# polli-labs/linnaeus

Measured on AMD Instinct MI355X. Metric: images/sec (train fwd+bwd) mFormerV1_sm 3x224x224, higher is better.
Workload: dtype bf16; 1 GPU; mFormerV1_sm train step (forward + 4-task CE loss + backward + AdamW (one HIP launch)), bf16 operands / fp32 accumulate+residual, batch 256/GPU, 3x224x224 synthetic, DropPath 0.2, gradient checkpointing off; per_gpu_batch=256, global_batch=256, parallelism=dp1, grad_mode=direct

## Files before the change

include/lnx.h:

```cpp
#ifndef LNX_H
#define LNX_H
#include <stdint.h>

#ifdef __cplusplus
extern "C" {
#endif

#define LNX_F32 0
#define LNX_BF16 1

const char* lnx_last_error(void);
int lnx_version(void);
int lnx_device_cus(void);
int lnx_set_cu_margin(int cus);

typedef struct lnx_rowmap {
    int group, pad, off;
} lnx_rowmap;

enum { LNX_ACT_NONE = 0, LNX_ACT_GELU = 1, LNX_ACT_RELU = 2, LNX_ACT_GELU_BWD = 3, LNX_ACT_RELU_BWD = 4,
       LNX_ACT_GELU_D = 5, LNX_ACT_MUL_AUX = 6 };
enum { LNX_ADDR_PLAIN = 0, LNX_ADDR_PATCH2 = 1 };

typedef struct lnx_gemm_args {
// ... 461 lines not shown
} lnx_metrics_task;
typedef struct lnx_metrics_args {
    int dtype;
    int B, n_tasks;
    lnx_metrics_task task[LNX_SOFTCE_MAX_TASKS];
    const int64_t* subset_ids[2];
    int n_bins[2];
    int64_t* counts;
    double* sums;
} lnx_metrics_args;
int lnx_metrics_table_sizes(int n_tasks, int n_bins0, int n_bins1, int64_t* n_counts, int64_t* n_sums);
int lnx_metrics_update(const lnx_metrics_args* args, void* stream);

#define LNX_PREDICT_MAX_K 16
typedef struct lnx_predict_task {
    const void* logits;
    int64_t ld;
    int C;
    const int32_t* parent;
    int null_index;
    const int64_t* id_map;
} lnx_predict_task;
typedef struct lnx_predict_args {
    int dtype;
    int B, n_tasks;
    int K;
    int consistency;
    const int32_t* k_per_sample;
    lnx_predict_task task[LNX_SOFTCE_MAX_TASKS];
    int64_t* ids;
    float* probs;
    int32_t* count;
    int32_t* flags;
} lnx_predict_args;
int lnx_predict(const lnx_predict_args* args, void* stream);

#define LNX_RESIZE_NEAREST 0
#define LNX_RESIZE_BILINEAR 1
#define LNX_RESIZE_BICUBIC 2
#define LNX_PREPROCESS_MAX_SIDE 16384
int lnx_resize_taps(int in_size, int out_size, int filter);
int lnx_resize_coeffs(int in_size, int out_size, int filter, int32_t* k, int32_t* bounds);
typedef struct lnx_preprocess_image {
    int64_t src;
    int64_t hk, hb;
    int64_t vk, vb;
    int64_t scratch;
    int32_t h, w;
    int32_t htaps, vtaps;
    int32_t y0, rows;
} lnx_preprocess_image;
typedef struct lnx_preprocess_args {
    int n, H, W;
    int filter;
    const lnx_preprocess_image* images;
    const void* blob;
    int64_t blob_bytes;
    int64_t images_off;
    void* scratch;
    int64_t scratch_bytes;
    float mean[3], std[3];
    float* out;
} lnx_preprocess_args;
int64_t lnx_preprocess_scratch_bytes(lnx_preprocess_image* images, int n, int H, int W, int filter);
int lnx_preprocess(const lnx_preprocess_args* args, void* stream);

enum { LNX_HL_WS_RAW = 0, LNX_HL_WS_LSE, LNX_HL_WS_SS, LNX_HL_WS_COEF, LNX_HL_WS_MASKED_CW, LNX_HL_WS_MASKED_W, LNX_HL_WS_FLAGS, LNX_HL_WS_ROWS };
enum { LNX_HL_OUT_RAW_MEAN = 0, LNX_HL_OUT_MASKED_MEAN, LNX_HL_OUT_WEIGHTED, LNX_HL_OUT_SCALE, LNX_HL_OUT_TOTAL = 32, LNX_HL_OUT_INCLUSION = 33,
       LNX_HL_OUT_FLOATS = 40 };
enum { LNX_HL_NULL_TOTAL = 8, LNX_HL_NULL_INCLUDED = 9, LNX_HL_COUNTS = 10 };
typedef struct lnx_hier_loss_task {
    const void* logits;
    int64_t ld;
    int C;
    const int64_t* target;
    const float* soft_target;
    int64_t ldt;
    const float* soft;
    float smoothing;
    const float* crit_weight;
    int64_t ignore_index;
    const float* class_weight;
    int n_cw;
    int p_cw, p_w;
    float* dlogits;
    int64_t ldd;
} lnx_hier_loss_task;
typedef struct lnx_hier_loss_args {
    int dtype;
    int B, n_tasks;
    float prob;
    int mask_mul;
    const float* draws;
    const float* weights;
    float* ws;
    float* out;
    int64_t* counts;
    lnx_hier_loss_task task[LNX_SOFTCE_MAX_TASKS];
} lnx_hier_loss_args;
int lnx_hier_loss_fwd(const lnx_hier_loss_args* args, void* stream);
int lnx_hier_loss_bwd(const lnx_hier_loss_args* args, const float* go_dev, void* stream);

int lnx_convmlp_supported(int dtype, int C);
typedef struct lnx_convmlp_args {
    int dtype, M, C;
    const void* ln;
    const void* w1;
    const float* b1;
    const void* w2;
    const float* b2;
    const float* gamma;
    const float* rowscale;
    int rows_per_sample;
    const float* x;
    float* out;
    void* z;
    const void* y;
    const float* ln_w;
    const float* ln_b;
    float ln_eps;
    void* ln_out;
    float* mean;
    float* rstd;
} lnx_convmlp_args;
int lnx_convmlp_fwd(const lnx_convmlp_args* args, void* stream);

typedef struct lnx_convmlp_bwd_args {
    int dtype, M, C;
    const float* g;
    const void* ln;
    const void* z;
    const void* w1;
    const float* b1;
    const void* w2t;
    const void* w1t;
    const float* gamma;
    const float* rowscale;
    int rows_per_sample;
    void* act;
    void* dh;
    void* dz;
    void* dln;
    float* dgamma;
    const void* y;
    const float* ln_w;
    const float* mean;
    const float* rstd;
    float* d_ln_w;
    float* d_ln_b;
    float* ws;
    int64_t ws_floats;
    int dz_plain;
    int ln_defer;
} lnx_convmlp_bwd_args;
int lnx_convmlp_bwd(const lnx_convmlp_bwd_args* args, void* stream);
int64_t lnx_convmlp_bwd_ws_floats(int C, int M);


#define LNX_MAX_META 8
#define LNX_MAX_TASKS 16
typedef struct lnx_mformer_cfg {
    int dtype;
    int batch, img_h, img_w, in_chans;
    int dims[4];
    int conv_depths[2];
    int rope_depths[2];
    int rope_heads[2];
    int mlp_hidden[2];
    int n_meta;
    int meta_dims[LNX_MAX_META];
    int only_last_cls;
    int n_tasks;
    int task_classes[LNX_MAX_TASKS];
    int inference;
    int recompute;
    int fp8;
    int rope_mode;
} lnx_mformer_cfg;

typedef struct lnx_plan lnx_plan;
int lnx_plan_create(const lnx_mformer_cfg* cfg, lnx_plan** out);
void lnx_plan_destroy(lnx_plan* p);
int64_t lnx_plan_workspace_bytes(const lnx_plan* p);
int lnx_plan_num_params(const lnx_plan* p);
const char* lnx_plan_param_name(const lnx_plan* p, int i);
int64_t lnx_plan_param_numel(const lnx_plan* p, int i);
int lnx_plan_num_drop_calls(const lnx_plan* p);
int64_t lnx_plan_logits_numel(const lnx_plan* p);
int64_t lnx_plan_logits_offset(const lnx_plan* p, int task);
int lnx_plan_logits_ld(const lnx_plan* p, int task);
int lnx_plan_bind(lnx_plan* p, const float* const* params, float* const* grads, void* workspace);
int lnx_plan_forward(lnx_plan* p, const float* x, const float* meta, const float* drop_scales, const unsigned char* drop_mask,
                     float* feats, float* logits, void* stream);
int64_t lnx_plan_dropout_bytes(const lnx_plan* p);
int lnx_plan_set_dropout(lnx_plan* p, const unsigned char* masks, float drop_rate);
int64_t lnx_plan_attn_dropout_bytes(const lnx_plan* p);
int lnx_plan_set_attn_dropout(lnx_plan* p, const unsigned char* masks, float drop_rate);
int lnx_plan_backward(lnx_plan* p, const float* dlogits, const float* dfeats, int segment, void* stream);
int lnx_plan_backward_into(lnx_plan* p, const float* dlogits, const float* dfeats, float* const* grads, void* stream);
#define LNX_PROFILE_CLASSES 8
int lnx_plan_profile_begin(lnx_plan* p);
int lnx_plan_profile_end(lnx_plan* p, double* ms, double* work, int* launches);
#define LNX_PROFILE_CLASSES_EX 10
int lnx_plan_profile_begin_spans(lnx_plan* p);
int lnx_plan_profile_end_ex(lnx_plan* p, double* ms, double* work, double* bytes, int* launches);
int lnx_plan_set_wgrad_stream(lnx_plan* p, int on);
int lnx_plan_set_meta_stream(lnx_plan* p, int mode);
int lnx_plan_segment_params(const lnx_plan* p, int segment, int* idx_out, int max_out);

#ifdef __cplusplus
}
#endif
#endif
```

linnaeus_amd/_lib.py:

```python
from __future__ import annotations

import ctypes as C
import os

_HERE = os.path.dirname(os.path.abspath(__file__))
LIB_PATH = os.environ.get("LNX_LIB_PATH") or os.path.join(_HERE, "liblnx_hip.so")

F32, BF16 = 0, 1
ACT_NONE, ACT_GELU, ACT_RELU, ACT_GELU_BWD, ACT_RELU_BWD, ACT_GELU_D, ACT_MUL_AUX = 0, 1, 2, 3, 4, 5, 6
TN_WS_FLOATS = 256 * (256 * 128 + 256)
ADDR_PLAIN, ADDR_PATCH2 = 0, 1


class LnxError(RuntimeError):
    pass


class RowMap(C.Structure):
    _fields_ = [("group", C.c_int), ("pad", C.c_int), ("off", C.c_int)]


class GemmArgs(C.Structure):
    _fields_ = [
        ("dtype", C.c_int), ("M", C.c_int), ("N", C.c_int), ("K", C.c_int),
        ("A", C.c_void_p), ("lda", C.c_int64),
        ("W", C.c_void_p), ("ldw", C.c_int64),
        ("C", C.c_void_p), ("ldc", C.c_int64),
        ("out_f32", C.c_int),
        ("a_mode", C.c_int), ("Hin", C.c_int), ("Win", C.c_int), ("Cin", C.c_int),
        ("c_mode", C.c_int), ("c_map", RowMap),
        ("bias", C.c_void_p),
        ("c2", C.c_void_p), ("ldc2", C.c_int64),
        ("act", C.c_int),
        ("aux", C.c_void_p), ("ldaux", C.c_int64),
        ("gamma", C.c_void_p), ("rowscale", C.c_void_p), ("rows_per_sample", C.c_int),
        ("res", C.c_void_p), ("ldres", C.c_int64),
        ("c8", C.c_void_p), ("ldc8", C.c_int64), ("c8_scales", C.c_void_p),
    ]


class WgradArgs(C.Structure):
    _fields_ = [
        ("dtype", C.c_int), ("M", C.c_int), ("N", C.c_int), ("K", C.c_int),
        ("dY", C.c_void_p), ("lddy", C.c_int64),
        ("A", C.c_void_p), ("lda", C.c_int64),
        ("a_mode", C.c_int), ("Hin", C.c_int), ("Win", C.c_int), ("Cin", C.c_int),
        ("dW", C.c_void_p), ("lddw", C.c_int64),
        ("k_perm_c", C.c_int),
        ("db", C.c_void_p),
        ("splits", C.c_int),
        ("k_store", C.c_int),
        ("ws", C.c_void_p), ("ws_floats", C.c_int64),
        ("defer", C.c_int),
    ]


class SoftCEArgs(C.Structure):
    _fields_ = [
        ("B", C.c_int), ("C", C.c_int),
        ("logits", C.c_void_p), ("ld", C.c_int64),
        ("target", C.c_void_p),
        ("soft", C.c_void_p), ("smoothing", C.c_float),
        ("class_weight", C.c_void_p),
        ("ignore_index", C.c_int64),
        ("row_scale", C.c_void_p), ("scale", C.c_float),
        ("loss", C.c_void_p), ("loss_sum", C.c_void_p),
        ("dlogits", C.c_void_p), ("ldd", C.c_int64),
    ]


ADAMW_MAX_GROUPS = 16


class AdamWDesc(C.Structure):
    _fields_ = [("p", C.c_void_p), ("m", C.c_void_p), ("v", C.c_void_p), ("g", C.c_void_p), ("n", C.c_int64), ("group", C.c_int), ("block_start", C.c_int)]


class AdamWHyper(C.Structure):
    _fields_ = [("ngroups", C.c_int)] + [(k, C.c_float * ADAMW_MAX_GROUPS) for k in ("lr", "beta1", "beta2", "eps", "weight_decay", "bias_c1", "bias_c2", "omb1", "omb2")]


class AdEMAMixHyper(C.Structure):
    _fields_ = [("ngroups", C.c_int)] + [(k, C.c_float * ADAMW_MAX_GROUPS) for k in ("lr", "beta1", "beta2", "eps", "weight_decay", "bias_c1", "bias_c2", "omb1", "omb2",
                                                                                  "alpha_t", "beta3_t", "omb3")]


class GradNormArgs(C.Structure):
    _fields_ = [("T", C.c_int), ("alpha", C.c_float), ("norm", C.c_void_p), ("loss_sum", C.c_void_p), ("count", C.c_void_p), ("init_loss", C.c_void_p),
                ("weights", C.c_void_p), ("initial_losses", C.c_void_p), ("initted", C.c_void_p), ("metrics", C.c_void_p)]


METRICS_MAX_TASKS = 8
METRICS_CHAIN_N, METRICS_CHAIN_CORRECT, METRICS_PARTIAL_N, METRICS_PARTIAL_CORRECT, METRICS_SUBSET_OOR = range(5)
METRICS_HEAD = 8
METRICS_N, METRICS_CORRECT1, METRICS_CORRECT3, METRICS_NULL_N, METRICS_NULL_CORRECT1, METRICS_NONNULL_N, METRICS_NONNULL_CORRECT1, METRICS_LOSS_N = range(8)
METRICS_TASK_STRIDE = 8
METRICS_SUM_LOSS, METRICS_SUM_NULL_LOSS, METRICS_SUM_NONNULL_LOSS = range(3)
METRICS_SUM_STRIDE = 4


def metrics_task(t: int) -> int:
    return METRICS_HEAD + METRICS_TASK_STRIDE * t


def metrics_subset(n_tasks: int, n_bins0: int, s: int) -> int:
    return metrics_task(n_tasks) + (2 * n_tasks * n_bins0 if s else 0)


class MetricsTask(C.Structure):
    _fields_ = [("logits", C.c_void_p), ("ld", C.c_int64), ("target", C.c_void_p), ("is_null", C.c_void_p), ("loss", C.c_void_p), ("C", C.c_int)]


class MetricsArgs(C.Structure):
    _fields_ = [("dtype", C.c_int), ("B", C.c_int), ("n_tasks", C.c_int), ("task", MetricsTask * METRICS_MAX_TASKS),
                ("subset_ids", C.c_void_p * 2), ("n_bins", C.c_int * 2), ("counts", C.c_void_p), ("sums", C.c_void_p)]


PREDICT_MAX_K = 16


class PredictTask(C.Structure):
    _fields_ = [("logits", C.c_void_p), ("ld", C.c_int64), ("C", C.c_int), ("parent", C.c_void_p), ("null_index", C.c_int), ("id_map", C.c_void_p)]


class PredictArgs(C.Structure):
    _fields_ = [("dtype", C.c_int), ("B", C.c_int), ("n_tasks", C.c_int), ("K", C.c_int), ("consistency", C.c_int), ("k_per_sample", C.c_void_p),
                ("task", PredictTask * METRICS_MAX_TASKS), ("ids", C.c_void_p), ("probs", C.c_void_p), ("count", C.c_void_p), ("flags", C.c_void_p)]


RESIZE_NEAREST, RESIZE_BILINEAR, RESIZE_BICUBIC = range(3)
PREPROCESS_MAX_SIDE = 16384


class PreprocessImage(C.Structure):
    _fields_ = [("src", C.c_int64), ("hk", C.c_int64), ("hb", C.c_int64), ("vk", C.c_int64), ("vb", C.c_int64), ("scratch", C.c_int64),
                ("h", C.c_int32), ("w", C.c_int32), ("htaps", C.c_int32), ("vtaps", C.c_int32), ("y0", C.c_int32), ("rows", C.c_int32)]


class PreprocessArgs(C.Structure):
    _fields_ = [("n", C.c_int), ("H", C.c_int), ("W", C.c_int), ("filter", C.c_int), ("images", C.POINTER(PreprocessImage)), ("blob", C.c_void_p),
                ("blob_bytes", C.c_int64), ("images_off", C.c_int64), ("scratch", C.c_void_p), ("scratch_bytes", C.c_int64),
                ("mean", C.c_float * 3), ("std", C.c_float * 3), ("out", C.c_void_p)]


HL_WS_RAW, HL_WS_LSE, HL_WS_SS, HL_WS_COEF, HL_WS_MASKED_CW, HL_WS_MASKED_W, HL_WS_FLAGS, HL_WS_ROWS = range(8)
HL_OUT_RAW_MEAN, HL_OUT_MASKED_MEAN, HL_OUT_WEIGHTED, HL_OUT_SCALE = range(4)
HL_OUT_TOTAL, HL_OUT_INCLUSION, HL_OUT_FLOATS = 32, 33, 40
HL_NULL_TOTAL, HL_NULL_INCLUDED, HL_COUNTS = 8, 9, 10


class HierLossTask(C.Structure):
    _fields_ = [("logits", C.c_void_p), ("ld", C.c_int64), ("C", C.c_int), ("target", C.c_void_p), ("soft_target", C.c_void_p), ("ldt", C.c_int64),
                ("soft", C.c_void_p), ("smoothing", C.c_float), ("crit_weight", C.c_void_p), ("ignore_index", C.c_int64), ("class_weight", C.c_void_p),
                ("n_cw", C.c_int), ("p_cw", C.c_int), ("p_w", C.c_int), ("dlogits", C.c_void_p), ("ldd", C.c_int64)]


class HierLossArgs(C.Structure):
    _fields_ = [("dtype", C.c_int), ("B", C.c_int), ("n_tasks", C.c_int), ("prob", C.c_float), ("mask_mul", C.c_int), ("draws", C.c_void_p),
                ("weights", C.c_void_p), ("ws", C.c_void_p), ("out", C.c_void_p), ("counts", C.c_void_p), ("task", HierLossTask * METRICS_MAX_TASKS)]


_lib = None


def lib() -> C.CDLL:
    global _lib
    if _lib is None:
        if not os.path.exists(LIB_PATH):
            raise LnxError(
                f"{LIB_PATH} is missing: build it with `python -c 'import __graft_entry__ as g; g.build()'` "
                "(or `make -C linnaeus_amd/csrc`). linnaeus_amd has no CPU fallback."
            )
        _lib = C.CDLL(LIB_PATH)
        _lib.lnx_last_error.restype = C.c_char_p
        _lib.lnx_nt_kernel_launches.restype = C.c_int64
        _lib.lnx_convmlp_bwd_ws_floats.restype = C.c_int64
        _lib.lnx_meta_heads_bwd_part_floats.restype = C.c_int64
        if hasattr(_lib, "lnx_ademamix_step"):
            _lib.lnx_ademamix_step.argtypes = [C.c_void_p, C.c_void_p, C.c_int, C.c_int, C.POINTER(AdEMAMixHyper), C.c_void_p, C.c_float, C.c_void_p]
        if hasattr(_lib, "lnx_gradnorm_sumsq"):
            _lib.lnx_gradnorm_sumsq.argtypes = [C.c_void_p, C.c_int, C.c_int, C.c_int, C.c_int64, C.c_void_p, C.c_void_p, C.c_void_p, C.c_void_p]
        if hasattr(_lib, "lnx_metrics_update"):
            _lib.lnx_metrics_update.argtypes = [C.POINTER(MetricsArgs), C.c_void_p]
            _lib.lnx_metrics_table_sizes.argtypes = [C.c_int, C.c_int, C.c_int, C.POINTER(C.c_int64), C.POINTER(C.c_int64)]
        if hasattr(_lib, "lnx_predict"):
            _lib.lnx_predict.argtypes = [C.POINTER(PredictArgs), C.c_void_p]
            _lib.lnx_predict.restype = C.c_int
        if hasattr(_lib, "lnx_hier_loss_fwd"):
            _lib.lnx_hier_loss_fwd.argtypes = [C.POINTER(HierLossArgs), C.c_void_p]
            _lib.lnx_hier_loss_bwd.argtypes = [C.POINTER(HierLossArgs), C.c_void_p, C.c_void_p]
        if hasattr(_lib, "lnx_preprocess"):
            _lib.lnx_resize_taps.argtypes = [C.c_int, C.c_int, C.c_int]
            _lib.lnx_resize_coeffs.argtypes = [C.c_int, C.c_int, C.c_int, C.c_void_p, C.c_void_p]
            _lib.lnx_preprocess_scratch_bytes.argtypes = [C.POINTER(PreprocessImage), C.c_int, C.c_int, C.c_int, C.c_int]
            _lib.lnx_preprocess_scratch_bytes.restype = C.c_int64
            _lib.lnx_preprocess.argtypes = [C.POINTER(PreprocessArgs), C.c_void_p]
            _lib.lnx_preprocess.restype = C.c_int
        if hasattr(_lib, "lnx_layernorm_fwd_query"):
            _lib.lnx_layernorm_fwd_query.argtypes = [C.POINTER(LnArgs), C.POINTER(LnLaunch)]
            _lib.lnx_layernorm_bwd_query.argtypes = [C.POINTER(LnBwdArgs), C.POINTER(LnLaunch)]
        older = bool(os.environ.get("LNX_LIB_PATH")) and os.environ.get("LNX_LIB_OLDER") == "1"
        for name in EXPORTS:
            if not hasattr(_lib, name) and not older:
                raise LnxError(f"{LIB_PATH} does not export {name}; rebuild it")
    return _lib


def check(rc: int, what: str) -> None:
    if rc != 0:
        raise LnxError(f"{what} failed (rc={rc}): {lib().lnx_last_error().decode()}")


AUG_CLAMP, AUG_POSTERIZE, AUG_SOLARIZE, AUG_SOLARIZE_ADD, AUG_INVERT, AUG_BRIGHTNESS, AUG_CONTRAST = range(7)

NT_KERNEL_NONE, NT_KERNEL_V1, NT_KERNEL_V2, NT_KERNEL_SKINNY, NT_KERNEL_V4, NT_KERNEL_FP8, NT_KERNEL_V7, NT_KERNEL_MX8, NT_KERNEL_V9, NT_KERNEL_EXPERIMENT = 0, 1, 2, 3, 4, 6, 7, 8, 9, 15

ROPE_COS, ROPE_ROTATE = 0, 1

ATTN_KERNEL_NONE, ATTN_KERNEL_RES4, ATTN_KERNEL_RES8, ATTN_KERNEL_TILED4, ATTN_KERNEL_TILED8 = range(5)

EXPORTS = [
    "lnx_last_error", "lnx_version", "lnx_device_cus", "lnx_set_cu_margin",
    "lnx_gemm_nt", "lnx_last_nt_kernel", "lnx_nt_kernel_launches", "lnx_nt_dispatch", "lnx_gemm_tn", "lnx_gemm_tn_flush", "lnx_gemm_tn_discard", "lnx_amax", "lnx_quantize_fp8", "lnx_gemm_nt_fp8", "lnx_quantize_mxfp8", "lnx_gemm_nt_mxfp8", "lnx_dropout_mul", "lnx_dropout_residual", "lnx_plan_dropout_bytes", "lnx_plan_set_dropout", "lnx_plan_attn_dropout_bytes", "lnx_plan_set_attn_dropout",
    "lnx_layernorm_fwd", "lnx_layernorm_bwd", "lnx_layernorm_bwd_flush", "lnx_layernorm_bwd_discard", "lnx_layernorm_fwd_query", "lnx_layernorm_bwd_query",
    "lnx_dwconv7_fwd", "lnx_dwconv7_wgrad",
    "lnx_gemm_nt_group_ok", "lnx_gemm_nt_group", "lnx_rope_cos_table", "lnx_rope_cos_table_hd", "lnx_rope_cossin_table_hd", "lnx_rope_cos_tables", "lnx_attn_bwd_ws_floats", "lnx_attn_bwd_ws_floats_hd", "lnx_attn_fwd", "lnx_attn_bwd", "lnx_attn_bwd_flush", "lnx_attn_bwd_discard", "lnx_attn_dispatch", "lnx_last_attn_kernel",
    "lnx_im2col_stem", "lnx_scale_cast", "lnx_layerscale_bwd", "lnx_layerscale_apply_wgrad", "lnx_fill_rows", "lnx_colsum_rows",
    "lnx_agg2_fwd", "lnx_agg2_bwd", "lnx_pack_meta", "lnx_meta_heads_supported", "lnx_meta_heads_fwd", "lnx_meta_heads_bwd", "lnx_meta_heads_bwd_part_floats", "lnx_prep_weights", "lnx_prep_blocks", "lnx_softce", "lnx_softce_multi", "lnx_stem_fwd", "lnx_stem_fwd_ok", "lnx_adamw_blocks", "lnx_grad_sumsq", "lnx_adamw_step", "lnx_ademamix_step", "lnx_gradnorm_sumsq", "lnx_gradnorm_update",
    "lnx_metrics_table_sizes", "lnx_metrics_update", "lnx_predict", "lnx_resize_taps", "lnx_resize_coeffs", "lnx_preprocess_scratch_bytes", "lnx_preprocess", "lnx_hier_loss_fwd", "lnx_hier_loss_bwd",
    "lnx_mix_rows", "lnx_mix_meta",
    "lnx_aug_pointwise", "lnx_aug_saturation", "lnx_aug_rowstat", "lnx_aug_rescale", "lnx_aug_affine", "lnx_aug_stencil", "lnx_erase_rects", "lnx_u8hwc_to_f32chw",
    "lnx_convmlp_supported", "lnx_convmlp_fwd", "lnx_convmlp_bwd", "lnx_convmlp_bwd_ws_floats",
    "lnx_plan_create", "lnx_plan_destroy", "lnx_plan_workspace_bytes", "lnx_plan_num_params", "lnx_plan_param_name",
    "lnx_plan_param_numel", "lnx_plan_num_drop_calls", "lnx_plan_logits_numel", "lnx_plan_logits_offset", "lnx_plan_logits_ld",
    "lnx_plan_bind", "lnx_plan_forward", "lnx_plan_backward", "lnx_plan_backward_into", "lnx_plan_segment_params", "lnx_plan_profile_begin", "lnx_plan_profile_end", "lnx_plan_profile_begin_spans", "lnx_plan_profile_end_ex", "lnx_plan_set_wgrad_stream", "lnx_plan_set_meta_stream",
]


class MetaHeadArgs(C.Structure):
    _fields_ = [
        ("B", C.c_int), ("C", C.c_int), ("dim", C.c_int), ("off", C.c_int),
        ("meta", C.c_void_p), ("meta_width", C.c_int), ("eps", C.c_float),
        ("w0", C.c_void_p), ("ldw0", C.c_int), ("b0", C.c_void_p), ("ln0_w", C.c_void_p), ("ln0_b", C.c_void_p),
        ("w1", C.c_void_p), ("ldw1", C.c_int), ("b1", C.c_void_p), ("ln1_w", C.c_void_p), ("ln1_b", C.c_void_p),
        ("w2", C.c_void_p), ("ldw2", C.c_int), ("b2", C.c_void_p), ("ln2_w", C.c_void_p), ("ln2_b", C.c_void_p),
        ("t0", C.c_void_p), ("h0", C.c_void_p), ("x", C.c_void_p), ("h1", C.c_void_p), ("n1", C.c_void_p), ("h2", C.c_void_p),
        ("m0", C.c_void_p), ("r0", C.c_void_p), ("m1", C.c_void_p), ("r1", C.c_void_p), ("m2", C.c_void_p), ("r2", C.c_void_p),
        ("tok", C.c_void_p), ("tok_row_stride", C.c_int64), ("tok_row_offset", C.c_int64),
    ]


class MetaHeadBwdArgs(C.Structure):
    _fields_ = [
        ("B", C.c_int), ("C", C.c_int), ("dim", C.c_int),
        ("g", C.c_void_p), ("g_row_stride", C.c_int64), ("g_row_offset", C.c_int64),
        ("w1t", C.c_void_p), ("ldw1t", C.c_int), ("w2t", C.c_void_p), ("ldw2t", C.c_int),
        ("ln0_w", C.c_void_p), ("ln1_w", C.c_void_p), ("ln2_w", C.c_void_p),
        ("t0", C.c_void_p), ("h0", C.c_void_p), ("x", C.c_void_p), ("h1", C.c_void_p), ("n1", C.c_void_p), ("h2", C.c_void_p),
        ("m0", C.c_void_p), ("r0", C.c_void_p), ("m1", C.c_void_p), ("r1", C.c_void_p), ("m2", C.c_void_p), ("r2", C.c_void_p),
        ("dp2", C.c_void_p), ("dp1", C.c_void_p), ("dp0", C.c_void_p), ("part", C.c_void_p),
        ("d_w0", C.c_void_p), ("d_b0", C.c_void_p), ("d_ln0_w", C.c_void_p), ("d_ln0_b", C.c_void_p),
        ("d_w1", C.c_void_p), ("d_b1", C.c_void_p), ("d_ln1_w", C.c_void_p), ("d_ln1_b", C.c_void_p),
        ("d_w2", C.c_void_p), ("d_b2", C.c_void_p), ("d_ln2_w", C.c_void_p), ("d_ln2_b", C.c_void_p),
    ]


class LnArgs(C.Structure):
    _fields_ = [
        ("M", C.c_int), ("C", C.c_int), ("eps", C.c_float),
        ("x", C.c_void_p), ("x_dtype", C.c_int), ("ldx", C.c_int64), ("x_map", RowMap),
        ("w", C.c_void_p), ("b", C.c_void_p),
        ("y", C.c_void_p), ("y_dtype", C.c_int), ("ldy", C.c_int64), ("y_map", RowMap),
        ("add", C.c_void_p), ("ldadd", C.c_int64),
        ("mean", C.c_void_p), ("rstd", C.c_void_p),
        ("y8", C.c_void_p), ("ldy8", C.c_int64), ("y8_scales", C.c_void_p),
    ]


class LnBwdArgs(C.Structure):
    _fields_ = [
        ("M", C.c_int), ("C", C.c_int),
        ("dy", C.c_void_p), ("dy_dtype", C.c_int), ("lddy", C.c_int64), ("dy_map", RowMap),
        ("x", C.c_void_p), ("x_dtype", C.c_int), ("ldx", C.c_int64), ("x_map", RowMap),
        ("w", C.c_void_p), ("mean", C.c_void_p), ("rstd", C.c_void_p),
        ("gin", C.c_void_p), ("ldgin", C.c_int64),
        ("dx", C.c_void_p), ("dx_dtype", C.c_int), ("lddx", C.c_int64),
        ("dw", C.c_void_p), ("db", C.c_void_p), ("relu_mask", C.c_int),
        ("ws", C.c_void_p), ("ws_floats", C.c_int64),
        ("dx2", C.c_void_p), ("dx2_dtype", C.c_int), ("lddx2", C.c_int64), ("dx2_rowscale", C.c_void_p), ("dx2_rows_per_sample", C.c_int),
        ("dx2_8", C.c_void_p), ("dx2_8_scales", C.c_void_p), ("lddx2_8", C.c_int64),
        ("defer", C.c_int),
    ]


LN_COLS_NONE, LN_COLS_ATOMICS, LN_COLS_WORKSPACE = range(3)


class LnLaunch(C.Structure):
    _fields_ = [("G", C.c_int), ("V", C.c_int), ("pair", C.c_int), ("full", C.c_int), ("mx", C.c_int), ("grid", C.c_int), ("cols", C.c_int), ("slices", C.c_int)]


class RopeTable(C.Structure):
    _fields_ = [
        ("freqs", C.c_void_p), ("cos_out", C.c_void_p), ("dsin_out", C.c_void_p),
        ("heads", C.c_int), ("H", C.c_int), ("W", C.c_int), ("head_dim", C.c_int),
        ("rope_mode", C.c_int), ("sin_out", C.c_void_p),
    ]


class DwconvArgs(C.Structure):
    _fields_ = [
        ("B", C.c_int), ("H", C.c_int), ("W", C.c_int), ("C", C.c_int),
        ("x", C.c_void_p), ("x_dtype", C.c_int), ("w49", C.c_void_p), ("bias", C.c_void_p),
        ("flip", C.c_int), ("res", C.c_void_p), ("y", C.c_void_p), ("y_dtype", C.c_int),
    ]


class DwconvWgradArgs(C.Structure):
    _fields_ = [
        ("B", C.c_int), ("H", C.c_int), ("W", C.c_int), ("C", C.c_int),
        ("x", C.c_void_p), ("x_dtype", C.c_int), ("dy", C.c_void_p), ("dy_dtype", C.c_int),
        ("dw", C.c_void_p), ("db", C.c_void_p),
    ]


class AttnArgs(C.Structure):
    _fields_ = [
        ("dtype", C.c_int), ("B", C.c_int), ("N", C.c_int), ("E", C.c_int), ("heads", C.c_int),
        ("qkv", C.c_void_p), ("cos_tab", C.c_void_p), ("o", C.c_void_p), ("lse", C.c_void_p),
        ("drop_mask", C.c_void_p), ("drop_inv_keep", C.c_float), ("head_dim", C.c_int),
        ("rope_mode", C.c_int), ("sin_tab", C.c_void_p),
    ]


class AttnBwdArgs(C.Structure):
    _fields_ = [
        ("dtype", C.c_int), ("B", C.c_int), ("N", C.c_int), ("E", C.c_int), ("heads", C.c_int),
        ("qkv", C.c_void_p), ("cos_tab", C.c_void_p), ("o", C.c_void_p), ("lse", C.c_void_p),
        ("d_o", C.c_void_p), ("dqkv", C.c_void_p), ("freq_ws", C.c_void_p), ("delta", C.c_void_p),
        ("drop_mask", C.c_void_p), ("drop_inv_keep", C.c_float),
        ("dsin_tab", C.c_void_p), ("dfreqs", C.c_void_p), ("defer_freqs", C.c_int), ("head_dim", C.c_int),
        ("rope_mode", C.c_int), ("sin_tab", C.c_void_p), ("grid_w", C.c_int),
    ]


class PrepDesc(C.Structure):
    _fields_ = [
        ("src", C.c_void_p), ("dst", C.c_void_p), ("dst_t", C.c_void_p),
        ("rows", C.c_int), ("cols", C.c_int), ("ld", C.c_int), ("ld_t", C.c_int),
        ("P", C.c_int), ("mode", C.c_int), ("block_start", C.c_int),
    ]


PREP_CAST, PREP_CONV_PERM, PREP_DW49 = 0, 1, 2


class ConvMlpArgs(C.Structure):
    _fields_ = [
        ("dtype", C.c_int), ("M", C.c_int), ("C", C.c_int),
        ("ln", C.c_void_p), ("w1", C.c_void_p), ("b1", C.c_void_p), ("w2", C.c_void_p), ("b2", C.c_void_p),
        ("gamma", C.c_void_p), ("rowscale", C.c_void_p), ("rows_per_sample", C.c_int),
        ("x", C.c_void_p), ("out", C.c_void_p), ("z", C.c_void_p),
        ("y", C.c_void_p), ("ln_w", C.c_void_p), ("ln_b", C.c_void_p), ("ln_eps", C.c_float), ("ln_out", C.c_void_p),
        ("mean", C.c_void_p), ("rstd", C.c_void_p),
    ]


class ConvMlpBwdArgs(C.Structure):
    _fields_ = [
        ("dtype", C.c_int), ("M", C.c_int), ("C", C.c_int),
        ("g", C.c_void_p), ("ln", C.c_void_p), ("z", C.c_void_p), ("w1", C.c_void_p), ("b1", C.c_void_p),
        ("w2t", C.c_void_p), ("w1t", C.c_void_p), ("gamma", C.c_void_p), ("rowscale", C.c_void_p), ("rows_per_sample", C.c_int),
        ("act", C.c_void_p), ("dh", C.c_void_p), ("dz", C.c_void_p), ("dln", C.c_void_p), ("dgamma", C.c_void_p),
        ("y", C.c_void_p), ("ln_w", C.c_void_p), ("mean", C.c_void_p), ("rstd", C.c_void_p), ("d_ln_w", C.c_void_p), ("d_ln_b", C.c_void_p),
        ("ws", C.c_void_p), ("ws_floats", C.c_int64),
        ("dz_plain", C.c_int), ("ln_defer", C.c_int),
    ]


class StemArgs(C.Structure):
    _fields_ = [("x", C.c_void_p), ("w", C.c_void_p), ("bias", C.c_void_p), ("ln_w", C.c_void_p), ("ln_b", C.c_void_p), ("patches", C.c_void_p),
                ("pre", C.c_void_p), ("y", C.c_void_p), ("mean", C.c_void_p), ("rstd", C.c_void_p), ("B", C.c_int), ("Cin", C.c_int), ("H", C.c_int),
                ("W", C.c_int), ("Cout", C.c_int), ("eps", C.c_float)]


class MixArgs(C.Structure):
    _fields_ = [
        ("x", C.c_void_p), ("perm", C.c_void_p), ("valid", C.c_void_p), ("out", C.c_void_p),
        ("B", C.c_int), ("row", C.c_int64), ("H", C.c_int), ("W", C.c_int), ("lam", C.c_float),
        ("h0", C.c_int), ("h1", C.c_int), ("w0", C.c_int), ("w1", C.c_int), ("mode", C.c_int),
    ]
```

linnaeus_amd/csrc/api.cpp:

```cpp
#include <hip/hip_runtime.h>
#include <stdarg.h>
#include <stdio.h>
#include <stdlib.h>
#include <string.h>

#include <atomic>
#include <mutex>

#include "../../include/lnx.h"

static thread_local char g_err[1024] = "";

void lnx_set_error(const char* fmt, ...) {
    va_list ap;
    va_start(ap, fmt);
    vsnprintf(g_err, sizeof(g_err), fmt, ap);
    va_end(ap);
}

extern "C" const char* lnx_last_error(void) { return g_err; }
extern "C" int lnx_version(void) { return 107; }
extern "C" int lnx_device_cus(void) {
    int dev = 0;
    if (hipGetDevice(&dev) != hipSuccess) return -1;
    hipDeviceProp_t prop;
    if (hipGetDeviceProperties(&prop, dev) != hipSuccess) return -1;
    return prop.multiProcessorCount;
}

static std::atomic<int> g_cu_margin{-1};
int persistent_cus(int cus) {
    int m = g_cu_margin.load(std::memory_order_relaxed);
    if (m < 0) {
        const char* e = getenv("LNX_CU_MARGIN");
        m = e ? atoi(e) : 0;
        if (m < 0) m = 0;
        g_cu_margin.store(m, std::memory_order_relaxed);
    }
    const int room = cus - m;
    return room < 8 ? 8 : room;
}
void set_cu_margin(int m) { g_cu_margin.store(m < 0 ? 0 : m, std::memory_order_relaxed); }
bool tile_sched_static() {
    const char* e = getenv("LNX_TILE_SCHED");
    return e && strcmp(e, "static") == 0;
}
int tile_slot_of(hipStream_t st) {
    static std::mutex mu;
    static hipStream_t known[64];
    static int n = 0;
    std::lock_guard<std::mutex> lock(mu);
    for (int i = 0; i < n; ++i)
        if (known[i] == st) return i;
    if (n < 64) {
        known[n] = st;
        return n++;
    }
    return -1;
}
int device_cus() {
    static std::atomic<int> cached{0};
    int c = cached.load(std::memory_order_relaxed);
    if (c == 0) {
        c = lnx_device_cus();
        if (c > 0) cached.store(c, std::memory_order_relaxed);
    }
    return c > 0 ? c : 0;
}
extern "C" int lnx_set_cu_margin(int cus) {
    if (cus < 0 || cus > 1024) {
        lnx_set_error("lnx_set_cu_margin: %d (0..1024 compute units)", cus);
        return 1;
    }
    set_cu_margin(cus);
    return 0;
}
```

linnaeus_amd/csrc/convmlp.hip:

```cpp
#include <stdlib.h>

#include "common.hpp"
#include "../../include/lnx.h"

namespace {

struct CmP {
    const unsigned char* ln;
    const unsigned char* w1;
    const unsigned char* w2;
    const unsigned char* w2t;
    const unsigned char* w1t;
    const unsigned char* zin;
    const float* b1;
    const float* b2;
    const float* gamma;
    const float* rowscale;
    const float* x;
    const float* g;
    float* out;
    unsigned char* z;
    unsigned char* act;
    unsigned char* dh;
    unsigned char* dz;
    unsigned char* dln;
    float* dgamma;
    int M, C, rps;
    const unsigned char* y;
    const float* lnw;
    const float* lnb;
    float eps;
    unsigned char* ln_out;
    float* mean;
    float* rstd;
    float* part;
    int64_t part_floats;
    int ln_defer;
    int tile_slot;
    int dz_plain;
    float* dlnw;
    float* dlnb;
};

__device__ __forceinline__ void mfma16(f32x4_t& acc, const uint4& a, const uint4& b) {
    acc = __builtin_amdgcn_mfma_f32_16x16x32_bf16(__builtin_bit_cast(bf16x8_t, a), __builtin_bit_cast(bf16x8_t, b), acc, 0, 0, 0);
}

__device__ __forceinline__ int key4(int a) { return (4 - (a & 3)) & 3; }

#define CM_DS_READ128(dst, addr, OFF) asm volatile("ds_read_b128 %0, %1 offset:" #OFF : "=v"(dst) : "v"(addr) : "memory")

template <int NK> struct Geo {
    static constexpr int C = 32 * NK;
    static constexpr int PART = NK * 4096;
    static constexpr int CT = C / 16;
};

template <int NK, int NW>
__device__ __forceinline__ void dma_nmajor(unsigned char* lds_part, const unsigned char* W, int n0, int wave, int lane) {
    constexpr int C = Geo<NK>::C;
    constexpr int NINS = 4 * NK;
    static_assert(NINS % NW == 0, "DMA pieces must divide evenly over the waves");
#pragma unroll
    for (int t = 0; t < NINS / NW; ++t) {
        const int i = wave + NW * t;
        const int ks = i >> 2, rb = i & 3;
        const int row = 16 * rb + (lane >> 2), u = lane & 3;
        const unsigned char* src = W + ((int64_t)(n0 + row) * C + ks * 32 + ((u ^ key4(row >> 3)) << 3)) * 2;
        __builtin_amdgcn_global_load_lds((const __attribute__((address_space(1))) void*)src,
                                         (__attribute__((address_space(3))) void*)(lds_part + i * 1024), 16, 0, 0);
    }
}

template <int NK, int NW>
__device__ __forceinline__ void dma_cmajor(unsigned char* lds_part, const unsigned char* W, int n0, int wave, int lane) {
    constexpr int C = Geo<NK>::C;
    constexpr int RB = C / 16;
    constexpr int NINS = 2 * RB;
#pragma unroll
    for (int t = 0; t < NINS / NW; ++t) {
        const int i = wave + NW * t;
        const int ks2 = i / RB, rb = i % RB;
        const int row = 16 * rb + (lane >> 2), u = lane & 3;
        const unsigned char* src = W + ((int64_t)row * (4 * C) + n0 + ks2 * 32 + ((u ^ key4(row >> 2)) << 3)) * 2;
        __builtin_amdgcn_global_load_lds((const __attribute__((address_space(1))) void*)src,
                                         (__attribute__((address_space(3))) void*)(lds_part + i * 1024), 16, 0, 0);
    }
}

template <int NK, int MT>
__device__ __forceinline__ void prod_nmajor(f32x4_t (&h)[4][MT], uint32_t part_addr, int s, int g, const uint4 (&xf)[MT][NK]) {
    const uint32_t unit = (uint32_t)((g ^ key4(s >> 2)) << 4);
    const uint32_t base = part_addr + (uint32_t)((8 * (s >> 2) + (s & 3)) * 64) + unit;
#pragma unroll
    for (int nt = 0; nt < 4; ++nt)
#pragma unroll
        for (int mt = 0; mt < MT; ++mt) h[nt][mt] = f32x4_t{0.f, 0.f, 0.f, 0.f};
#pragma unroll
    for (int ks = 0; ks < NK; ++ks) {
        uint4 wf[4];
        const uint32_t a = base + ks * 4096;
        CM_DS_READ128(wf[0], a, 0);
        CM_DS_READ128(wf[1], a, 256);
        CM_DS_READ128(wf[2], a, 2048);
        CM_DS_READ128(wf[3], a, 2304);
        asm volatile("s_waitcnt lgkmcnt(0)" ::: "memory");
        __builtin_amdgcn_sched_barrier(0);
#pragma unroll
        for (int nt = 0; nt < 4; ++nt)
#pragma unroll
            for (int mt = 0; mt < MT; ++mt) mfma16(h[nt][mt], wf[nt], xf[mt][ks]);
    }
}

template <int NK, int MT, int KB>
__device__ __forceinline__ void prod_nmajor_b(f32x4_t (&h)[4][MT], uint32_t part_addr, int s, int g, const uint4 (&xf)[MT][NK]) {
    const uint32_t unit = (uint32_t)((g ^ key4(s >> 2)) << 4);
    const uint32_t base = part_addr + (uint32_t)((8 * (s >> 2) + (s & 3)) * 64) + unit;
#pragma unroll
    for (int nt = 0; nt < 4; ++nt)
#pragma unroll
        for (int mt = 0; mt < MT; ++mt) h[nt][mt] = f32x4_t{0.f, 0.f, 0.f, 0.f};
#pragma unroll
    for (int k0 = 0; k0 < NK; k0 += KB) {
        uint4 wf[KB][4];
#pragma unroll
        for (int kb = 0; kb < KB; ++kb) {
            if (k0 + kb < NK) {
                const uint32_t a = base + (k0 + kb) * 4096;
                CM_DS_READ128(wf[kb][0], a, 0);
                CM_DS_READ128(wf[kb][1], a, 256);
                CM_DS_READ128(wf[kb][2], a, 2048);
                CM_DS_READ128(wf[kb][3], a, 2304);
            }
        }
        asm volatile("s_waitcnt lgkmcnt(0)" ::: "memory");
        __builtin_amdgcn_sched_barrier(0);
#pragma unroll
        for (int kb = 0; kb < KB; ++kb) {
            if (k0 + kb < NK) {
#pragma unroll
                for (int nt = 0; nt < 4; ++nt)
#pragma unroll
                    for (int mt = 0; mt < MT; ++mt) mfma16(h[nt][mt], wf[kb][nt], xf[mt][k0 + kb]);
            }
        }
    }
}

template <int NK, int MT>
__device__ __forceinline__ void prod_cmajor(f32x4_t (&o)[Geo<NK>::CT][MT], uint32_t part_addr, int s, int g, const uint4 (&pf)[MT][2]) {
    constexpr int C = Geo<NK>::C;
    constexpr int CT = Geo<NK>::CT;
    const uint32_t base = part_addr + (uint32_t)(s * 64) + (uint32_t)((g ^ key4(s >> 2)) << 4);
    constexpr int GB = CT % 6 == 0 ? 6 : (CT % 4 == 0 ? 4 : CT);
#pragma unroll
    for (int ks2 = 0; ks2 < 2; ++ks2) {
#pragma unroll
        for (int c0 = 0; c0 < CT; c0 += GB) {
            uint4 wf[GB];
#pragma unroll
            for (int b = 0; b < GB; ++b) {
                const uint32_t a = base + (uint32_t)(ks2 * C * 64 + (c0 + b) * 1024);
                CM_DS_READ128(wf[b], a, 0);
            }
            asm volatile("s_waitcnt lgkmcnt(0)" ::: "memory");
            __builtin_amdgcn_sched_barrier(0);
#pragma unroll
            for (int b = 0; b < GB; ++b)
#pragma unroll
                for (int mt = 0; mt < MT; ++mt) mfma16(o[c0 + b][mt], wf[b], pf[mt][ks2]);
        }
    }
}

template <int NK, int MT>
__device__ __forceinline__ void prod_nmajor_pipe(f32x4_t (&h)[4][MT], uint32_t part_addr, int s, int g, const uint4 (&xf)[MT][NK]) {
// ... 573 lines not shown
    float* gms = b2s + C;
    float* lws = gms + C;
    float* lbs = lws + C;
    const int lane = threadIdx.x & 63;
    const int wave = __builtin_amdgcn_readfirstlane(threadIdx.x >> 6);
    const int s = lane & 15, g = lane >> 4;
    const uint32_t lds0 = (uint32_t)(uintptr_t)(__attribute__((address_space(3))) unsigned char*)smem;

    for (int i = threadIdx.x; i < 4 * C; i += 512) b1s[i] = p.b1[i];
    for (int i = threadIdx.x; i < C; i += 512) {
        b2s[i] = p.b2[i];
        gms[i] = p.gamma[i];
        if constexpr (LNF) {
            lws[i] = p.lnw[i];
            lbs[i] = p.lnb[i];
        }
    }
    const bool dyn = p.tile_slot >= 0;
    const TileShare sh = tile_share((p.M + 31) / 32);
    unsigned* const ctr = &g_tile_ctr[dyn ? p.tile_slot : 0][sh.part][0];
    int drawn = dyn ? sched_draw_counted(ctr) : 0;
    dma_all_nmajor<NK>(w1img, p.w1, wave, lane);
    dma_all_cmajor<NK>(w2img, p.w2, wave, lane);
    asm volatile("s_waitcnt vmcnt(0)" ::: "memory");
    __syncthreads();

    const int ntile = (p.M + 31) / 32;
    auto load_x = [&](uint4 (&dst)[MT][NK], int tile) __attribute__((always_inline)) {
#pragma unroll
        for (int mt = 0; mt < MT; ++mt) {
            const int m = min(tile * 32 + mt * 16 + s, p.M - 1);
#pragma unroll
            for (int ks = 0; ks < NK; ++ks) dst[mt][ks] = ld16((LNF ? p.y : p.ln) + ((int64_t)m * C + ks * 32 + 8 * g) * 2);
        }
    };
    const int xbase = sh.base, xcnt = sh.cnt, xwaves = 8 * sh.workers;
    const int last_draw = xcnt + xwaves - 1;
    int pos = dyn ? __builtin_amdgcn_readfirstlane(drawn) : sh.index * 8 + wave;
    bool reset_ctr = dyn && pos == last_draw;
    uint4 xf[MT][NK];
    if (pos < xcnt) load_x(xf, xbase + pos);
    const float* rsp = p.rowscale ? p.rowscale : p.gamma;
    const float rsf = p.rowscale ? 1.0f : 0.0f;

    int next = 0;
    for (; pos < xcnt; pos = next) {
        const int tile = xbase + pos;
        const int m_base = tile * 32;
        if constexpr (LNF) {
#pragma unroll
            for (int mt = 0; mt < MT; ++mt) {
                float mu, rs;
                ln_row_frags<NK>(xf[mt], lws, lbs, g, p.eps, mu, rs);
                const int m = min(m_base + mt * 16 + s, p.M - 1);
                if constexpr (SAVE != 0) {
#pragma unroll
                    for (int ks = 0; ks < NK; ++ks) st16(p.ln_out + ((int64_t)m * C + ks * 32 + 8 * g) * 2, xf[mt][ks]);
                    if (g == 0) {
                        p.mean[m] = mu;
                        p.rstd[m] = rs;
                    }
                }
            }
        }
        if constexpr (LNF) __builtin_amdgcn_sched_barrier(0);
        if (dyn) drawn = sched_draw_counted(ctr);
        float4 xrv[MT][CT];
        float rsv[MT];
        f32x4_t o[CT][MT];
#pragma unroll
        for (int ct = 0; ct < CT; ++ct)
#pragma unroll
            for (int mt = 0; mt < MT; ++mt) o[ct][mt] = f32x4_t{0.f, 0.f, 0.f, 0.f};
        auto chunk = [&](const int j, auto lastc) __attribute__((always_inline)) {
            constexpr bool LAST = decltype(lastc)::value;
            if constexpr (LAST) {
                __builtin_amdgcn_sched_barrier(0);
                if (dyn) {
                    next = __builtin_amdgcn_readfirstlane(drawn);
                    reset_ctr = reset_ctr || next == last_draw;
                } else {
                    next = pos + xwaves;
                }
#pragma unroll
                for (int mt = 0; mt < MT; ++mt) {
                    const int m = min(m_base + mt * 16 + s, p.M - 1);
#pragma unroll
                    for (int ct = 0; ct < CT; ++ct) xrv[mt][ct] = *reinterpret_cast<const float4*>(p.x + (int64_t)m * C + ct * 16 + 4 * g);
                    rsv[mt] = rsp[p.rowscale ? m / p.rps : 0];
                }
            }
            f32x4_t h[4][MT];
            prod_nmajor_b<NK, MT, NK>(h, lds0 + j * PART, s, g, xf);
            if constexpr (LAST) {
                __builtin_amdgcn_sched_barrier(0);
                load_x(xf, next < xcnt ? xbase + next : tile);
            }
            f32x4_t bv[4];
            const uint32_t ba = lds0 + 2 * NCH * PART + (uint32_t)((64 * j + 8 * g) * 4);
            CM_DS_READ128(bv[0], ba, 0);
            CM_DS_READ128(bv[1], ba, 16);
            CM_DS_READ128(bv[2], ba, 128);
            CM_DS_READ128(bv[3], ba, 144);
            asm volatile("s_waitcnt lgkmcnt(0)" ::: "memory");
            __builtin_amdgcn_sched_barrier(0);
            constexpr int GK = NK == 3 ? 1 : 2;
#pragma unroll
            for (int mt = 0; mt < MT; ++mt)
#pragma unroll
                for (int n2 = 0; n2 < 4; n2 += GK) {
                    f32x4_t hv[GK];
#pragma unroll
                    for (int k = 0; k < GK; ++k) hv[k] = h[n2 + k][mt];
                    gelu4_bias_n<GK>(hv, &bv[n2]);
#pragma unroll
                    for (int k = 0; k < GK; ++k) h[n2 + k][mt] = hv[k];
                }
            uint4 pf[MT][2];
#pragma unroll
            for (int mt = 0; mt < MT; ++mt) {
                pf[mt][0] = pack8(h[0][mt], h[1][mt]);
                pf[mt][1] = pack8(h[2][mt], h[3][mt]);
            }
            prod_cmajor<NK, MT>(o, lds0 + NCH * PART + j * PART, s, g, pf);
        };
#pragma unroll 1
        for (int j = 0; j < NCH - 1; ++j) chunk(j, BoolC<false>{});
        chunk(NCH - 1, BoolC<true>{});
#pragma unroll
        for (int mt = 0; mt < MT; ++mt) {
            const int m = min(m_base + mt * 16 + s, p.M - 1);
            const float rs = fmaf(rsv[mt] - 1.0f, rsf, 1.0f);
#pragma unroll
            for (int ct = 0; ct < CT; ++ct) {
                const int c = ct * 16 + 4 * g;
                const float4 b2 = *reinterpret_cast<const float4*>(b2s + c);
                const float4 gm = *reinterpret_cast<const float4*>(gms + c);
                const float4 xr = xrv[mt][ct];
                const float z0 = o[ct][mt][0] + b2.x, z1 = o[ct][mt][1] + b2.y, z2 = o[ct][mt][2] + b2.z, z3 = o[ct][mt][3] + b2.w;
                if constexpr (SAVE == 1) {
                    uint2 zz;
                    bf16_t* zh = reinterpret_cast<bf16_t*>(&zz);
                    zh[0] = (bf16_t)z0; zh[1] = (bf16_t)z1; zh[2] = (bf16_t)z2; zh[3] = (bf16_t)z3;
                    *reinterpret_cast<uint2*>(p.z + ((int64_t)m * C + c) * 2) = zz;
                }
                *reinterpret_cast<float4*>(p.out + (int64_t)m * C + c) =
                    make_float4(xr.x + rs * gm.x * z0, xr.y + rs * gm.y * z1, xr.z + rs * gm.z * z2, xr.w + rs * gm.w * z3);
            }
        }
    }
    if (reset_ctr && lane == 0) sched_reset(ctr);
}

template <int NK, int MT, bool ST, bool LNB, bool DG>
__global__ __launch_bounds__(512) void convmlp_bwd_res_kernel(const CmP p) {
    constexpr int C = Geo<NK>::C;
    constexpr int CT = Geo<NK>::CT;
    constexpr int PART = Geo<NK>::PART;
    constexpr int NCH = 4 * C / 64;
    extern __shared__ __attribute__((aligned(16))) unsigned char smem[];
    unsigned char* w1img = smem;
    unsigned char* w2timg = smem + NCH * PART;
    float* b1s = reinterpret_cast<float*>(smem + 2 * NCH * PART);
    float* dgs = b1s + 4 * C;
    float* lws = dgs + C;
    float* dls = lws + C;
    float* gms = dls + 2 * C;
    const int lane = threadIdx.x & 63;
    const int wave = __builtin_amdgcn_readfirstlane(threadIdx.x >> 6);
    const int s = lane & 15, g = lane >> 4;
    const uint32_t lds0 = (uint32_t)(uintptr_t)(__attribute__((address_space(3))) unsigned char*)smem;

    for (int i = threadIdx.x; i < 4 * C; i += 512) b1s[i] = p.b1[i];
    for (int i = threadIdx.x; i < C; i += 512) {
        dgs[i] = 0.f;
        gms[i] = p.gamma[i];
        if constexpr (LNB) {
            lws[i] = p.lnw[i];
            dls[i] = dls[C + i] = 0.f;
        }
    }
    const bool dyn = p.tile_slot >= 0;
    const TileShare sh = tile_share((p.M + 16 * MT - 1) / (16 * MT));
    unsigned* const ctr = &g_tile_ctr[dyn ? p.tile_slot : 0][sh.part][0];
    int drawn = dyn ? sched_draw_counted(ctr) : 0;
    dma_all_nmajor<NK>(w1img, p.w1, wave, lane);
    dma_all_nmajor<NK>(w2timg, p.w2t, wave, lane);
    asm volatile("s_waitcnt vmcnt(0)" ::: "memory");
    __syncthreads();

    float dgp[NK][8];
#pragma unroll
    for (int ks = 0; ks < NK; ++ks)
#pragma unroll
        for (int j = 0; j < 8; ++j) dgp[ks][j] = 0.f;

    const int ntile = (p.M + 16 * MT - 1) / (16 * MT);
    const float* rsp = p.rowscale ? p.rowscale : p.gamma;
    const float rsf = p.rowscale ? 1.0f : 0.0f;
    struct TileIn {
        uint4 x[MT][NK], z[MT][NK];
        float4 g0[MT][NK], g1[MT][NK];
        float rs[MT];
        LnRow<NK> lr[MT];
    };
    auto fetch_tile = [&](TileIn& t, int tile) __attribute__((always_inline)) {
#pragma unroll
        for (int mt = 0; mt < MT; ++mt) {
            const int m = min(tile * (16 * MT) + mt * 16 + s, p.M - 1);
#pragma unroll
            for (int ks = 0; ks < NK; ++ks) {
                const int c = ks * 32 + 8 * g;
                t.x[mt][ks] = ld16(p.ln + ((int64_t)m * C + c) * 2);
                t.g0[mt][ks] = *reinterpret_cast<const float4*>(p.g + (int64_t)m * C + c);
                t.g1[mt][ks] = *reinterpret_cast<const float4*>(p.g + (int64_t)m * C + c + 4);
                if constexpr (DG) t.z[mt][ks] = ld16(p.zin + ((int64_t)m * C + c) * 2);
            }
            t.rs[mt] = rsp[p.rowscale ? m / p.rps : 0];
            if constexpr (LNB) ln_bwd_fetch<NK>(t.lr[mt], p, m, g);
        }
    };
    const int xbase = sh.base, xcnt = sh.cnt, xwaves = 8 * sh.workers;
    const int last_draw = xcnt + xwaves - 1;
    int pos = dyn ? __builtin_amdgcn_readfirstlane(drawn) : sh.index * 8 + wave;
    bool reset_ctr = dyn && pos == last_draw;
    TileIn cur;
    if (pos < xcnt) fetch_tile(cur, xbase + pos);
    int next = 0;
    for (; pos < xcnt; pos = next) {
        const int tile = xbase + pos;
        const int m_base = tile * (16 * MT);
        uint4 xf[MT][NK], zf[MT][NK];
        LnRow<NK> lrow[MT];
#pragma unroll
        for (int mt = 0; mt < MT; ++mt) {
            int m = m_base + mt * 16 + s;
            const bool mv = m < p.M;
            if (!mv) m = p.M - 1;
            const float rs = fmaf(cur.rs[mt] - 1.0f, rsf, 1.0f);
            lrow[mt] = cur.lr[mt];
#pragma unroll
            for (int ks = 0; ks < NK; ++ks) {
                const int c = ks * 32 + 8 * g;
                xf[mt][ks] = cur.x[mt][ks];
                const float4 g0 = cur.g0[mt][ks], g1 = cur.g1[mt][ks];
                const float4 a0 = *reinterpret_cast<const float4*>(gms + c), a1 = *reinterpret_cast<const float4*>(gms + c + 4);
                Vec16<bf16_t> zin, dzv, dzs;
                if constexpr (DG) zin.raw = cur.z[mt][ks];
                const float gv[8] = {g0.x, g0.y, g0.z, g0.w, g1.x, g1.y, g1.z, g1.w};
                const float av[8] = {a0.x, a0.y, a0.z, a0.w, a1.x, a1.y, a1.z, a1.w};
#pragma unroll
                for (int j = 0; j < 8; ++j) {
                    const float sg = rs * gv[j];
                    dzv.set(j, sg * av[j]);
                    dzs.set(j, p.dz_plain ? sg : sg * av[j]);
                    if constexpr (DG) dgp[ks][j] = fmaf(mv ? sg : 0.f, zin.get(j), dgp[ks][j]);
                }
                zf[mt][ks] = dzv.raw;
                st16(p.dz + ((int64_t)m * C + c) * 2, dzs.raw);
            }
        }
        if (dyn) drawn = sched_draw_counted(ctr);
        f32x4_t dl[CT][MT];
#pragma unroll
        for (int ct = 0; ct < CT; ++ct)
#pragma unroll
            for (int mt = 0; mt < MT; ++mt) dl[ct][mt] = f32x4_t{0.f, 0.f, 0.f, 0.f};
#pragma unroll 1
        for (int j = 0; j < NCH; ++j) {
            f32x4_t h[4][MT], da[4][MT];
            prod_nmajor_b<NK, MT, NK>(h, lds0 + j * PART, s, g, xf);
            prod_nmajor_b<NK, MT, NK>(da, lds0 + NCH * PART + j * PART, s, g, zf);
            f32x4_t bv[4];
            const uint32_t ba = lds0 + 2 * NCH * PART + (uint32_t)((64 * j + 8 * g) * 4);
            CM_DS_READ128(bv[0], ba, 0);
            CM_DS_READ128(bv[1], ba, 16);
            CM_DS_READ128(bv[2], ba, 128);
            CM_DS_READ128(bv[3], ba, 144);
            asm volatile("s_waitcnt lgkmcnt(0)" ::: "memory");
            __builtin_amdgcn_sched_barrier(0);
#pragma unroll
            for (int mt = 0; mt < MT; ++mt)
#pragma unroll
                for (int n2 = 0; n2 < 4; n2 += 2) {
                    f32x4_t hv[2] = {h[n2][mt], h[n2 + 1][mt]}, dv[2] = {da[n2][mt], da[n2 + 1][mt]};
                    gelu4_bias_grad_n<2>(hv, &bv[n2], dv);
                    h[n2][mt] = hv[0];
                    h[n2 + 1][mt] = hv[1];
                    da[n2][mt] = dv[0];
                    da[n2 + 1][mt] = dv[1];
                }
            uint4 pd[MT][2];
#pragma unroll
            for (int mt = 0; mt < MT; ++mt) {
                const uint4 pa0 = pack8(h[0][mt], h[1][mt]), pa1 = pack8(h[2][mt], h[3][mt]);
                pd[mt][0] = pack8(da[0][mt], da[1][mt]);
                pd[mt][1] = pack8(da[2][mt], da[3][mt]);
                const int m = min(m_base + mt * 16 + s, p.M - 1);
                if constexpr (ST) {
                    const int64_t off = ((int64_t)m * (4 * C) + 64 * j + 8 * g) * 2;
                    st16(p.act + off, pa0);
                    st16(p.act + off + 64, pa1);
                    st16(p.dh + off, pd[mt][0]);
                    st16(p.dh + off + 64, pd[mt][1]);
                }
            }
            prod_tr_nmajor<NK, MT>(dl, lds0 + j * PART, s, g, pd);
        }
        __builtin_amdgcn_sched_barrier(0);
        if (dyn) {
            next = __builtin_amdgcn_readfirstlane(drawn);
            reset_ctr = reset_ctr || next == last_draw;
        } else {
            next = pos + xwaves;
        }
        fetch_tile(cur, next < xcnt ? xbase + next : tile);
        if constexpr (LNB) {
            ln_bwd_rows<NK, MT, 0>(p, dl, lrow[0], m_base + s, s, g, lws, dls);
            if constexpr (MT == 2) ln_bwd_rows<NK, MT, 1>(p, dl, lrow[MT - 1], m_base + 16 + s, s, g, lws, dls);
        } else {
#pragma unroll
            for (int mt = 0; mt < MT; ++mt) {
                const int m = min(m_base + mt * 16 + s, p.M - 1);
#pragma unroll
                for (int ct = 0; ct < CT; ++ct) {
                    const int c = ct * 16 + 4 * g;
                    uint2 v;
                    bf16_t* vh = reinterpret_cast<bf16_t*>(&v);
                    vh[0] = (bf16_t)dl[ct][mt][0]; vh[1] = (bf16_t)dl[ct][mt][1]; vh[2] = (bf16_t)dl[ct][mt][2]; vh[3] = (bf16_t)dl[ct][mt][3];
                    *reinterpret_cast<uint2*>(p.dln + ((int64_t)m * C + c) * 2) = v;
                }
            }
        }
    }
    if constexpr (DG) {
#pragma unroll
        for (int ks = 0; ks < NK; ++ks)
#pragma unroll
            for (int j = 0; j < 8; ++j) {
                float t = dgp[ks][j];
                t += __shfl_xor(t, 1, 64);
                t += __shfl_xor(t, 2, 64);
                t += __shfl_xor(t, 4, 64);
                t += __shfl_xor(t, 8, 64);
                if (s == 0) atomicAdd(&dgs[ks * 32 + 8 * g + j], t);
            }
    }
    __syncthreads();
    if constexpr (DG)
        for (int i = threadIdx.x; i < C; i += 512) atomicAdd(p.dgamma + i, dgs[i]);
    if constexpr (LNB)
        for (int i = threadIdx.x; i < 2 * C; i += 512) p.part[(int64_t)blockIdx.x * (2 * C) + i] = dls[i];
    if (reset_ctr && lane == 0) sched_reset(ctr);
}

__global__ __launch_bounds__(256) void ln_partials_reduce_kernel(const float* __restrict__ part, int nwg, int C, float* __restrict__ dw, float* __restrict__ db) {
    const int e = blockIdx.x * 256 + threadIdx.x;
    if (e >= 2 * C) return;
    const int per = (nwg + gridDim.y - 1) / gridDim.y;
    const int w0 = blockIdx.y * per, w1 = min(nwg, w0 + per);
    float t0 = 0.f, t1 = 0.f, t2 = 0.f, t3 = 0.f;
    int w = w0;
    for (; w + 4 <= w1; w += 4) {
        t0 += part[(int64_t)w * 2 * C + e];
        t1 += part[(int64_t)(w + 1) * 2 * C + e];
        t2 += part[(int64_t)(w + 2) * 2 * C + e];
        t3 += part[(int64_t)(w + 3) * 2 * C + e];
    }
    for (; w < w1; ++w) t0 += part[(int64_t)w * 2 * C + e];
    const float t = (t0 + t1) + (t2 + t3);
    if (w0 < w1) atomicAdd((e < C ? dw : db) + (e < C ? e : e - C), t);
}

static const bool nw8 = !(getenv("LNX_CM_NW") && atoi(getenv("LNX_CM_NW")) == 4);

static int bwd_grid(int C, int M) {
    if (C <= 96) {
        const int rows = C == 32 ? 32 : 16;
        const int grid = cdiv(cdiv(M, rows), 8);
        return grid > 256 ? 256 : grid;
    }
    return cdiv(M, 16 * (nw8 ? 8 : 4));
}

static int res_room() {
    const int cus = device_cus();
    const int room = persistent_cus(cus > 0 ? cus : 256);
    return room > 256 ? 256 : room;
}

template <int NK, bool LNF, int SAVE>
int launch_fwd_res_t(const CmP& p, hipStream_t st) {
    const size_t lds = 2 * (4 * Geo<NK>::C / 64) * Geo<NK>::PART + 8 * Geo<NK>::C * sizeof(float);
    static bool attr = false;
    if (!attr) {
        (void)hipFuncSetAttribute(reinterpret_cast<const void*>(&convmlp_fwd_res_kernel<NK, LNF, SAVE>), hipFuncAttributeMaxDynamicSharedMemorySize, (int)lds);
        attr = true;
    }
    int grid = cdiv(cdiv(p.M, 32), 8);
    const int room = res_room();
    if (grid > room) grid = room;
    CmP q = p;
    q.tile_slot = tile_sched_static() ? -1 : tile_slot_of(st);
    hipLaunchKernelGGL((convmlp_fwd_res_kernel<NK, LNF, SAVE>), dim3(grid), dim3(512), lds, st, q);
    return 0;
}
template <int NK>
int launch_fwd_res(const CmP& p, hipStream_t st) {
    if (p.y) return p.z ? launch_fwd_res_t<NK, true, 1>(p, st) : (p.ln_out ? launch_fwd_res_t<NK, true, 2>(p, st) : launch_fwd_res_t<NK, true, 0>(p, st));
    return p.z ? launch_fwd_res_t<NK, false, 1>(p, st) : launch_fwd_res_t<NK, false, 0>(p, st);
}
inline int reduce_ln_partials(const CmP& p, int nwg, hipStream_t st) {
    if (p.ln_defer) {
        ln_postpone_reduce(p.part, nwg, p.C, p.dlnw, p.dlnb, nwg >= 64 ? 64 : 1, st);
        return 0;
    }
    hipLaunchKernelGGL(ln_partials_reduce_kernel, dim3(cdiv(2 * p.C, 256), nwg >= 64 ? 64 : 1), dim3(256), 0, st, p.part, nwg, p.C, p.dlnw, p.dlnb);
    return 0;
}
template <int NK, int MT, bool ST, bool LNB, bool DG>
int launch_bwd_res_t(const CmP& p, hipStream_t st) {
    const size_t lds = 2 * (4 * Geo<NK>::C / 64) * Geo<NK>::PART + 9 * Geo<NK>::C * sizeof(float);
    static bool attr = false;
    if (!attr) {
        (void)hipFuncSetAttribute(reinterpret_cast<const void*>(&convmlp_bwd_res_kernel<NK, MT, ST, LNB, DG>), hipFuncAttributeMaxDynamicSharedMemorySize, (int)lds);
        attr = true;
    }
    int grid = bwd_grid(p.C, p.M);
    if (LNB && (int64_t)grid * 2 * p.C > p.part_floats) return -1;
    const int room = res_room();
    if (grid > room) grid = room;
    CmP q = p;
    q.tile_slot = tile_sched_static() ? -1 : tile_slot_of(st);
    hipLaunchKernelGGL((convmlp_bwd_res_kernel<NK, MT, ST, LNB, DG>), dim3(grid), dim3(512), lds, st, q);
    return LNB ? reduce_ln_partials(p, grid, st) : 0;
}
template <int NK, int MT>
int launch_bwd_res(const CmP& p, hipStream_t st) {
    if (p.zin == nullptr) {
        if (p.y) return p.act ? launch_bwd_res_t<NK, MT, true, true, false>(p, st) : launch_bwd_res_t<NK, MT, false, true, false>(p, st);
        return p.act ? launch_bwd_res_t<NK, MT, true, false, false>(p, st) : launch_bwd_res_t<NK, MT, false, false, false>(p, st);
    }
    if (p.y) return p.act ? launch_bwd_res_t<NK, MT, true, true, true>(p, st) : launch_bwd_res_t<NK, MT, false, true, true>(p, st);
    return p.act ? launch_bwd_res_t<NK, MT, true, false, true>(p, st) : launch_bwd_res_t<NK, MT, false, false, true>(p, st);
}

template <int NK, int MT, int NW, bool LNF>
int launch_fwd_t(const CmP& p, hipStream_t st) {
    const size_t lds = 3 * 2 * Geo<NK>::PART + 4 * Geo<NK>::C * sizeof(float);
    static bool attr = false;
    if (!attr) {
        (void)hipFuncSetAttribute(reinterpret_cast<const void*>(&convmlp_fwd_kernel<NK, MT, NW, LNF>), hipFuncAttributeMaxDynamicSharedMemorySize, (int)lds);
        attr = true;
    }
    hipLaunchKernelGGL((convmlp_fwd_kernel<NK, MT, NW, LNF>), dim3(cdiv(p.M, 16 * NW * MT)), dim3(64 * NW), lds, st, p);
    return 0;
}
template <int NK, int MT, int NW>
int launch_fwd(const CmP& p, hipStream_t st) {
    return p.y ? launch_fwd_t<NK, MT, NW, true>(p, st) : launch_fwd_t<NK, MT, NW, false>(p, st);
}

template <int NK, int MT, int NW, bool ST, bool LNB, bool DG>
int launch_bwd_t(const CmP& p, hipStream_t st) {
    const size_t lds = 2 * 3 * Geo<NK>::PART + 8 * Geo<NK>::C * sizeof(float);
    static bool attr = false;
    if (!attr) {
        (void)hipFuncSetAttribute(reinterpret_cast<const void*>(&convmlp_bwd_kernel<NK, MT, NW, ST, LNB, DG>), hipFuncAttributeMaxDynamicSharedMemorySize, (int)lds);
        attr = true;
    }
    static_assert(MT == 1, "bwd_grid() assumes 16-row wave tiles in the streamed-weight backward");
    const int grid = bwd_grid(p.C, p.M);
    if (LNB && (int64_t)grid * 2 * p.C > p.part_floats) return -1;
    hipLaunchKernelGGL((convmlp_bwd_kernel<NK, MT, NW, ST, LNB, DG>), dim3(grid), dim3(64 * NW), lds, st, p);
    return LNB ? reduce_ln_partials(p, grid, st) : 0;
}
template <int NK, int MT, int NW>
int launch_bwd(const CmP& p, hipStream_t st) {
    if (p.zin == nullptr) {
        if (p.y) return p.act ? launch_bwd_t<NK, MT, NW, true, true, false>(p, st) : launch_bwd_t<NK, MT, NW, false, true, false>(p, st);
        return p.act ? launch_bwd_t<NK, MT, NW, true, false, false>(p, st) : launch_bwd_t<NK, MT, NW, false, false, false>(p, st);
    }
    if (p.y) return p.act ? launch_bwd_t<NK, MT, NW, true, true, true>(p, st) : launch_bwd_t<NK, MT, NW, false, true, true>(p, st);
    return p.act ? launch_bwd_t<NK, MT, NW, true, false, true>(p, st) : launch_bwd_t<NK, MT, NW, false, false, true>(p, st);
}

}

extern "C" int64_t lnx_convmlp_bwd_ws_floats(int C, int M) {
    if (!lnx_convmlp_supported(LNX_BF16, C) || M <= 0) return 0;
    return (int64_t)bwd_grid(C, M) * 2 * C;
}

extern "C" int lnx_convmlp_supported(int dtype, int C) { return dtype == LNX_BF16 && (C == 32 || C == 64 || C == 96 || C == 128 || C == 192); }

extern "C" int lnx_convmlp_fwd(const lnx_convmlp_args* a, void* stream) {
    LNX_CHECK(a && (a->ln || a->y) && a->w1 && a->w2 && a->b1 && a->b2 && a->gamma && a->x && a->out, "lnx_convmlp_fwd: null operand");
    if (a->y) {
        LNX_CHECK(a->ln_w && a->ln_b && a->ln == nullptr, "lnx_convmlp_fwd: the fused LayerNorm form takes y, ln_w, ln_b and no ln");
        LNX_CHECK((a->mean == nullptr) == (a->ln_out == nullptr) && (a->rstd == nullptr) == (a->ln_out == nullptr) && (a->z == nullptr || a->ln_out != nullptr),
                  "lnx_convmlp_fwd: with y, the outputs ln_out, mean and rstd are written together (what a backward needs) or not at all; z only with them");
    }
    LNX_CHECK(lnx_convmlp_supported(a->dtype, a->C), "lnx_convmlp_fwd: unsupported dtype %d / C %d (bf16, C in {32,64,96,128,192})", a->dtype, a->C);
    LNX_CHECK(a->M > 0, "lnx_convmlp_fwd: empty");
    if (a->rowscale) LNX_CHECK(a->rows_per_sample > 0, "lnx_convmlp_fwd: rowscale needs rows_per_sample");
    CmP p{};
    p.ln = (const unsigned char*)a->ln; p.w1 = (const unsigned char*)a->w1; p.w2 = (const unsigned char*)a->w2;
    p.b1 = a->b1; p.b2 = a->b2; p.gamma = a->gamma; p.rowscale = a->rowscale; p.x = a->x; p.out = a->out; p.z = (unsigned char*)a->z;
    p.M = a->M; p.C = a->C; p.rps = a->rows_per_sample > 0 ? a->rows_per_sample : 1;
    p.y = (const unsigned char*)a->y; p.lnw = a->ln_w; p.lnb = a->ln_b; p.eps = a->ln_eps; p.ln_out = (unsigned char*)a->ln_out; p.mean = a->mean; p.rstd = a->rstd;
    hipStream_t st = (hipStream_t)stream;
    switch (a->C) {
        case 32: launch_fwd_res<1>(p, st); break;
        case 64: launch_fwd_res<2>(p, st); break;
        case 96: launch_fwd_res<3>(p, st); break;
        case 128: if (nw8) launch_fwd<4, 1, 8>(p, st); else launch_fwd<4, 1, 4>(p, st); break;
        case 192: if (nw8) launch_fwd<6, 1, 8>(p, st); else launch_fwd<6, 1, 4>(p, st); break;
    }
    LNX_LAUNCH_CHECK();
    return 0;
}

extern "C" int lnx_convmlp_bwd(const lnx_convmlp_bwd_args* a, void* stream) {
    LNX_CHECK(a && a->g && a->ln && a->w1 && a->w2t && a->w1t && a->b1 && a->gamma && a->dz && a->dln && (a->dgamma || !a->z),
              "lnx_convmlp_bwd: null operand (z may be NULL: dgamma is then not produced here; with z, dgamma is required)");
    LNX_CHECK((a->act == nullptr) == (a->dh == nullptr), "lnx_convmlp_bwd: act and dh must both be given or both be NULL");
    LNX_CHECK(lnx_convmlp_supported(a->dtype, a->C), "lnx_convmlp_bwd: unsupported dtype %d / C %d", a->dtype, a->C);
    LNX_CHECK(a->M > 0, "lnx_convmlp_bwd: empty");
    if (a->rowscale) LNX_CHECK(a->rows_per_sample > 0, "lnx_convmlp_bwd: rowscale needs rows_per_sample");
    if (a->y) LNX_CHECK(a->ln_w && a->mean && a->rstd && a->d_ln_w && a->d_ln_b && a->ws, "lnx_convmlp_bwd: the fused LayerNorm form needs ln_w, mean, rstd, d_ln_w, d_ln_b and ws");
    CmP p{};
    p.y = (const unsigned char*)a->y; p.lnw = a->ln_w; p.mean = const_cast<float*>(a->mean); p.rstd = const_cast<float*>(a->rstd);
    p.part = a->ws; p.part_floats = a->ws_floats; p.dlnw = a->d_ln_w; p.dlnb = a->d_ln_b; p.ln_defer = a->ln_defer;
    p.g = a->g; p.ln = (const unsigned char*)a->ln; p.zin = (const unsigned char*)a->z; p.w1 = (const unsigned char*)a->w1;
    p.w2t = (const unsigned char*)a->w2t; p.w1t = (const unsigned char*)a->w1t; p.b1 = a->b1; p.gamma = a->gamma; p.rowscale = a->rowscale;
    p.act = (unsigned char*)a->act; p.dh = (unsigned char*)a->dh; p.dz = (unsigned char*)a->dz; p.dln = (unsigned char*)a->dln; p.dgamma = a->dgamma;
    p.M = a->M; p.C = a->C; p.rps = a->rows_per_sample > 0 ? a->rows_per_sample : 1;
    p.dz_plain = a->dz_plain != 0;
    hipStream_t st = (hipStream_t)stream;
    int rc = 0;
    switch (a->C) {
        case 32: rc = launch_bwd_res<1, 2>(p, st); break;
        case 64: rc = launch_bwd_res<2, 1>(p, st); break;
        case 96: rc = launch_bwd_res<3, 1>(p, st); break;
        case 128: rc = nw8 ? launch_bwd<4, 1, 8>(p, st) : launch_bwd<4, 1, 4>(p, st); break;
        case 192: rc = nw8 ? launch_bwd<6, 1, 8>(p, st) : launch_bwd<6, 1, 4>(p, st); break;
    }
    LNX_CHECK(rc == 0, "lnx_convmlp_bwd: ws too small for the LayerNorm partial sums (M=%d C=%d ws_floats=%lld)", a->M, a->C, (long long)a->ws_floats);
    LNX_LAUNCH_CHECK();
    return 0;
}
```

linnaeus_amd/csrc/plan.cpp:

```cpp
#include <hip/hip_runtime.h>
#include <stdlib.h>
#include <string.h>

#include <mutex>
#include <atomic>
#include <string>
#include <vector>

#include "../../include/lnx.h"

void lnx_set_error(const char* fmt, ...);

#define RUN(expr)                  \
    do {                           \
        const int rc_ = (expr);    \
        if (rc_ != 0) return rc_;  \
    } while (0)
#define FAIL(...)                   \
    do {                            \
        lnx_set_error(__VA_ARGS__); \
        return 1;                   \
    } while (0)
#define HIPRUN(expr)                                                         \
    do {                                                                     \
        const hipError_t e_ = (expr);                                        \
        if (e_ != hipSuccess) FAIL("%s: %s", #expr, hipGetErrorString(e_)); \
    } while (0)

namespace {

constexpr int LN_DEFER_SLOTS = 16;
constexpr int FREQ_DEFER_SLOTS = 8;

inline int64_t align_up(int64_t v, int64_t a) { return (v + a - 1) / a * a; }

struct OpW {
    int param = -1;
    int N = 0, K = 0;
    int ld = 0;
    int ld_t = 0;
    int mode = LNX_PREP_CAST, P = 0;
    bool f32 = false;
    int64_t off = 0, off_t = 0;
    int64_t off8 = 0, off8s = 0;
    int64_t off8t = 0, off8ts = 0;
};

struct ConvBlk {
    bool fused = false;
    bool fused_ln = false;
    bool keep_z = true;
    int gamma, dww, dwb, lnw, lnb, b1, b2;
    OpW w1, w2;
    int64_t w49;
    int64_t xin, y, ln, mean, rstd, hpre, act, z;
};
struct RopeBlk {
    int n1w, n1b, n2w, n2b, freqs, qkvb, projb, fc1b, fc2b;
    OpW qkv, proj, fc1, fc2;
    int64_t xin, n1, mean1, rstd1, qkvbuf, cos, dsin, o, lse, xmid, n2, mean2, rstd2, hpre, act;
    int64_t dm_proj = 0, dm_hid = 0, dm_fc2 = 0;
    int64_t dm_attn = 0;
};
struct MetaHead {
    int b0, lnw0, lnb0, nf1w, nf1b, nf2w, nf2b, b1, b2;
    OpW w0, w1, w2;
    int dim, off;
    int64_t t0, h0, x, m0, r0, h1, n1, m1, r1, h2, m2, r2;
    int64_t dp2 = 0, dp1 = 0, dp0 = 0, part = 0;
};
struct Down {
    int lnw, lnb, cb;
    OpW w;
    int64_t ln, mean, rstd;
};

}

constexpr int TN_WS_SLOTS = 4;

struct lnx_plan {
    lnx_mformer_cfg c;
    int esz;
    int E;
    int H[4], W[4], HW[4];
    int N2, N3;
    std::vector<std::string> names;
    std::vector<int64_t> numel;
    std::vector<const float*> P;
    std::vector<float*> G;
    bool bound = false, has_grads = false, fwd_done = false;
    unsigned char* ws = nullptr;
    int64_t ws_bytes = 0;

    int stem_b, stem_lnw, stem_lnb, cls[2], norm_w[2], norm_b[2], fin_w, fin_b, agg_w, agg_b, cl_b1, cl_b2, cl_lnw, cl_lnb;
    OpW stem_w, cl_w1, cl_w2;
    std::vector<int> head_b;
    std::vector<OpW> head_w;
    std::vector<int> logit_ld;
    std::vector<int64_t> logit_off;
    int64_t logits_numel = 0;
    Down down[3];
    std::vector<ConvBlk> conv[2];
    std::vector<RopeBlk> rope[2];
    std::vector<MetaHead> meta[2];
    std::vector<OpW*> all_w;
    std::vector<int> drop_conv[2], drop_attn[2], drop_mlp[2];
    int n_drop = 0;

    int64_t o_descs = 0, n_descs = 0, prep_blocks = 0;
    int64_t n_descs_t = 0, n_descs_f = 0, prep_blocks_f = 0;
    int64_t o_patches, o_stem_pre, o_stem_mean, o_stem_rstd;
    int64_t o_stage_out[4];
    int64_t o_tok[2];
    int64_t o_t1, o_t1_mean, o_t1_rstd;
    int64_t o_cl_hpre, o_cl_act, o_cl_u, o_cl_mean, o_cl_rstd, o_c1n;
    int64_t o_c2n, o_n2_mean, o_n2_rstd, o_agg, o_fin_mean, o_fin_rstd, o_feats, o_featsT;
    int64_t o_g[4];
    int64_t o_sA, o_sB = 0, o_sC, o_sD;
    int64_t o_lnws = 0, lnws_floats = 0, o_lnws_side = 0, lnws_side_floats = 0;
    int64_t lnws_defer_floats = 0;
    int64_t o_lnws_defer = 0;
    int ln_pending = 0;
    int64_t gcos_floats = 0;
    int freq_pending = 0;
    bool freq_defer = true;
    bool ln_defer = true;
    int64_t o_tnws = 0;
    int64_t o_lsws = 0, lsws_floats = 0;
    int64_t o_gcos , o_delta, o_dt1, o_tail[6], o_mtmp[4], o_dlT;
    int64_t o_a8 = 0, o_a8s = 0, o_h8 = 0, o_h8s = 0;
    const float* last_drop = nullptr;
    const unsigned char* last_mask = nullptr;
    std::vector<unsigned char> mask_host;
    const float* last_meta = nullptr;
    int resident[4] = {-1, -1, -1, -1};
    const unsigned char* dmask = nullptr;
    float inv_keep = 1.0f;
    int64_t dmask_bytes = 0;
    const unsigned char* amask = nullptr;
    float a_inv_keep = 1.0f;
    int64_t amask_bytes = 0;
    hipStream_t side = nullptr;
    hipEvent_t ev_fork = nullptr, ev_meta = nullptr, ev_bfork[2] = {nullptr, nullptr}, ev_bjoin[2] = {nullptr, nullptr};
    hipStream_t wgs = nullptr;
    bool wgs_on = true;
    bool meta_forked[2] = {false, false};
    int meta_mode = 1;
    bool meta_chain = true;
    bool chain_ok[2] = {false, false};
    bool dy8_ready = false;
    hipEvent_t ev_wf[4] = {nullptr, nullptr, nullptr, nullptr}, ev_wj[4] = {nullptr, nullptr, nullptr, nullptr};
    bool profile = false;
    bool profile_spans = false;
    struct Span { hipEvent_t e0, e1; int cls; double work, bytes; };
    std::vector<Span> spans;
    std::vector<hipEvent_t> ev_pool;
    size_t ev_used = 0;

    template <typename U> U* at(int64_t off) const { return reinterpret_cast<U*>(ws + off); }
    const float* drop_ptr(int call) const {
        if (last_drop == nullptr || call < 0 || !mask_host[call]) return nullptr;
        return last_drop + (int64_t)call * c.batch;
    }
};

namespace {

int find_param(const lnx_plan* p, const std::string& n) {
    for (size_t i = 0; i < p->names.size(); ++i)
        if (p->names[i] == n) return (int)i;
    return -1;
}

void add_param(lnx_plan* p, const std::string& n, int64_t numel) {
    p->names.push_back(n);
    p->numel.push_back(numel);
}

void build_inventory(lnx_plan* p) {
    const lnx_mformer_cfg& c = p->c;
    const int* D = c.dims;
    char b[128];
    add_param(p, "cls_token_1", D[2]);
    add_param(p, "cls_token_2", D[3]);
    add_param(p, "stem.0.weight", (int64_t)D[0] * c.in_chans * 16);
    add_param(p, "stem.0.bias", D[0]);
    add_param(p, "stem.1.weight", D[0]);
    add_param(p, "stem.1.bias", D[0]);
    for (int i = 0; i < 3; ++i) {
        snprintf(b, sizeof b, "downsample_layers.%d.", i);
        const std::string pre(b);
        add_param(p, pre + "norm.weight", D[i]);
        add_param(p, pre + "norm.bias", D[i]);
        add_param(p, pre + "conv.weight", (int64_t)D[i + 1] * D[i] * 4);
        add_param(p, pre + "conv.bias", D[i + 1]);
    }
    for (int s = 0; s < 2; ++s)
        for (int i = 0; i < c.conv_depths[s]; ++i) {
            snprintf(b, sizeof b, "stages.%d.%d.", s, i);
            const std::string pre(b);
            const int64_t C = D[s];
            add_param(p, pre + "gamma", C);
            add_param(p, pre + "dwconv.weight", C * 49);
// ... 164 lines not shown
            ConvBlk& k = p->conv[s][i];
            const int C = D[s];
            k.gamma = find_param(p, pre + "gamma");
            k.dww = find_param(p, pre + "dwconv.weight");
            k.dwb = find_param(p, pre + "dwconv.bias");
            k.lnw = find_param(p, pre + "norm.weight");
            k.lnb = find_param(p, pre + "norm.bias");
            k.b1 = find_param(p, pre + "pwconv1.bias");
            k.b2 = find_param(p, pre + "pwconv2.bias");
            k.w1 = make_w(p, pre + "pwconv1.weight", 4 * C, C, true);
            k.w2 = make_w(p, pre + "pwconv2.weight", C, 4 * C, true);
            p->drop_conv[s].push_back(call++);
        }
    }
    for (int s = 0; s < 2; ++s) {
        p->rope[s].resize(c.rope_depths[s]);
        for (int i = 0; i < c.rope_depths[s]; ++i) {
            snprintf(b, sizeof b, "stages.%d.%d.", s + 2, i);
            const std::string pre(b);
            RopeBlk& k = p->rope[s][i];
            const int C = D[2 + s], hid = c.mlp_hidden[s];
            k.n1w = find_param(p, pre + "norm1.weight");
            k.n1b = find_param(p, pre + "norm1.bias");
            k.n2w = find_param(p, pre + "norm2.weight");
            k.n2b = find_param(p, pre + "norm2.bias");
            k.freqs = find_param(p, pre + "attn.freqs");
            k.qkvb = find_param(p, pre + "attn.qkv.bias");
            k.projb = find_param(p, pre + "attn.proj.bias");
            k.fc1b = find_param(p, pre + "mlp.fc1.bias");
            k.fc2b = find_param(p, pre + "mlp.fc2.bias");
            k.qkv = make_w(p, pre + "attn.qkv.weight", 3 * C, C, true);
            k.proj = make_w(p, pre + "attn.proj.weight", C, C, true);
            k.fc1 = make_w(p, pre + "mlp.fc1.weight", hid, C, true);
            k.fc2 = make_w(p, pre + "mlp.fc2.weight", C, hid, true);
            p->drop_attn[s].push_back(call++);
            p->drop_mlp[s].push_back(call++);
        }
    }
    p->n_drop = call;
    for (int s = 0; s < 2; ++s) {
        snprintf(b, sizeof b, "norm_%d.", s + 1);
        p->norm_w[s] = find_param(p, std::string(b) + "weight");
        p->norm_b[s] = find_param(p, std::string(b) + "bias");
        p->meta[s].resize(c.n_meta);
        int off = 0;
        for (int m = 0; m < c.n_meta; ++m) {
            snprintf(b, sizeof b, "meta.%d.head_%d.", m, s + 1);
            const std::string pre(b);
            MetaHead& k = p->meta[s][m];
            const int C = D[2 + s];
            k.dim = c.meta_dims[m];
            k.off = off;
            off += k.dim;
            k.w0 = make_w(p, pre + "0.weight", C, k.dim, false, LNX_PREP_CAST, 0, true);
            k.b0 = find_param(p, pre + "0.bias");
            k.lnw0 = find_param(p, pre + "2.weight");
            k.lnb0 = find_param(p, pre + "2.bias");
            k.nf1w = find_param(p, pre + "3.norm_fn1.weight");
            k.nf1b = find_param(p, pre + "3.norm_fn1.bias");
            k.nf2w = find_param(p, pre + "3.norm_fn2.weight");
            k.nf2b = find_param(p, pre + "3.norm_fn2.bias");
            k.w1 = make_w(p, pre + "3.w1.weight", C, C, true, LNX_PREP_CAST, 0, true);
            k.b1 = find_param(p, pre + "3.w1.bias");
            k.w2 = make_w(p, pre + "3.w2.weight", C, C, true, LNX_PREP_CAST, 0, true);
            k.b2 = find_param(p, pre + "3.w2.bias");
        }
    }
    if (!c.only_last_cls) {
        p->cl_w1 = make_w(p, "cl_1_fc.0.fc1.weight", D[2], D[2], true);
        p->cl_w2 = make_w(p, "cl_1_fc.0.fc2.weight", D[3], D[2], true);
        p->cl_b1 = find_param(p, "cl_1_fc.0.fc1.bias");
        p->cl_b2 = find_param(p, "cl_1_fc.0.fc2.bias");
        p->cl_lnw = find_param(p, "cl_1_fc.1.weight");
        p->cl_lnb = find_param(p, "cl_1_fc.1.bias");
        p->agg_w = find_param(p, "aggregate.weight");
        p->agg_b = find_param(p, "aggregate.bias");
    }
    p->fin_w = find_param(p, "final_norm.weight");
    p->fin_b = find_param(p, "final_norm.bias");
    p->head_w.resize(c.n_tasks);
    p->head_b.resize(c.n_tasks);
    p->logit_ld.resize(c.n_tasks);
    p->logit_off.resize(c.n_tasks);
    for (int t = 0; t < c.n_tasks; ++t) {
        snprintf(b, sizeof b, "head.%d.", t);
        p->head_w[t] = make_w(p, std::string(b) + "weight", c.task_classes[t], D[3], true);
        p->head_b[t] = find_param(p, std::string(b) + "bias");
        p->logit_ld[t] = (int)align_up(c.task_classes[t], 8);
        p->head_w[t].ld_t = p->logit_ld[t];
        p->logit_off[t] = p->logits_numel;
        p->logits_numel += (int64_t)B * p->logit_ld[t];
    }

    auto reg = [&](OpW& w) { p->all_w.push_back(&w); };
    reg(p->stem_w);
    for (int i = 0; i < 3; ++i) reg(p->down[i].w);
    for (int s = 0; s < 2; ++s)
        for (auto& k : p->conv[s]) {
            reg(k.w1);
            reg(k.w2);
        }
    for (int s = 0; s < 2; ++s)
        for (auto& k : p->rope[s]) {
            reg(k.qkv);
            reg(k.proj);
            reg(k.fc1);
            reg(k.fc2);
        }
    for (int s = 0; s < 2; ++s)
        for (auto& k : p->meta[s]) {
            reg(k.w0);
            reg(k.w1);
            reg(k.w2);
        }
    if (!c.only_last_cls) {
        reg(p->cl_w1);
        reg(p->cl_w2);
    }
    for (auto& w : p->head_w) reg(w);

    Carver cv;
    int ndw = 0;
    for (int s = 0; s < 2; ++s) ndw += c.conv_depths[s];
    p->n_descs = (int64_t)p->all_w.size() + ndw;
    p->o_descs = cv.take(p->n_descs * sizeof(lnx_prep_desc));
    for (OpW* w : p->all_w) {
        const int wes = w->f32 ? 4 : 2;
        w->off = cv.take((int64_t)w->N * w->ld * wes);
        if (w->ld_t) w->off_t = cv.take((int64_t)w->K * w->ld_t * wes);
    }
    for (int s = 0; s < 2; ++s)
        for (auto& k : p->conv[s]) k.w49 = cv.take((int64_t)49 * D[s] * 4);
    if (c.fp8)
        for (int s = 0; s < 2; ++s)
            for (auto& k : p->rope[s]) {
                for (OpW* w : {&k.qkv, &k.fc1, &k.fc2}) {
                    w->off8 = cv.take((int64_t)w->N * w->K);
                    w->off8s = cv.take((int64_t)(w->K / 128) * w->N * 4);
                }
                if (!c.inference && !(getenv("LNX_FP8_DGRAD") && atoi(getenv("LNX_FP8_DGRAD")) == 0))
                    for (OpW* w : {&k.proj, &k.fc1, &k.fc2}) {
                        w->off8t = cv.take((int64_t)w->K * w->N);
                        w->off8ts = cv.take((int64_t)(w->N / 128) * w->K * 4);
                    }
            }
    const int64_t arena_end = cv.cur;
    (void)arena_end;

    const int64_t M0 = (int64_t)B * p->HW[0];
    p->o_patches = cv.take(M0 * 64 * esz);
    p->o_stem_pre = cv.take(M0 * D[0] * esz);
    p->o_stem_mean = cv.take(M0 * 4);
    p->o_stem_rstd = cv.take(M0 * 4);
    int64_t maxMC = 0, maxM4C = 0;
    bool any_fused = false;
    const bool inf = c.inference != 0;
    const bool ck = !inf && c.recompute != 0;
    for (int s = 0; s < 2; ++s) {
        const int64_t M = (int64_t)B * p->HW[s], C = D[s];
        if (M * C > maxMC) maxMC = M * C;
        if (M * 4 * C > maxM4C) maxM4C = M * 4 * C;
        int64_t pp[2] = {0, 0};
        if (inf) {
            pp[0] = cv.take(M * C * 4);
            pp[1] = cv.take(M * C * 4);
        }
        const size_t nb = p->conv[s].size();
        for (size_t i = 0; i < nb; ++i) {
            ConvBlk& k = p->conv[s][i];
            const bool share = (inf || ck) && i > 0;
            const ConvBlk& f = p->conv[s][0];
            k.xin = inf ? pp[i & 1] : cv.take(M * C * 4);
            k.y = share ? f.y : cv.take(M * C * esz);
            k.ln = share ? f.ln : cv.take(M * C * esz);
            k.mean = share ? f.mean : cv.take(M * 4);
            k.rstd = share ? f.rstd : cv.take(M * 4);
            k.fused = lnx_convmlp_supported(c.dtype, (int)C) != 0 && getenv("LNX_NO_FUSED_MLP") == nullptr &&
                      (getenv("LNX_FUSED_MLP_MAXC") == nullptr || C <= atoi(getenv("LNX_FUSED_MLP_MAXC")));
            any_fused = any_fused || k.fused;
            {
                const int64_t lnws = (int64_t)2048 * 2 * (D[3] > D[0] ? D[3] : D[0]);
                k.fused_ln = k.fused && getenv("LNX_NO_FUSED_LN") == nullptr && lnx_convmlp_bwd_ws_floats((int)C, (int)M) <= lnws;
            }
            if (!k.fused) {
                k.hpre = share ? f.hpre : cv.take(M * 4 * C * esz);
                k.act = share ? f.act : cv.take(M * 4 * C * esz);
            }
            k.keep_z = !k.fused || getenv("LNX_CONV_Z") != nullptr;
            k.z = !k.keep_z ? 0 : (share ? f.z : cv.take(M * C * esz));
        }
        p->o_stage_out[s] = inf ? pp[nb & 1] : cv.take(M * C * 4);
        p->down[s].ln = cv.take(M * C * esz);
        p->down[s].mean = cv.take(M * 4);
        p->down[s].rstd = cv.take(M * 4);
        p->o_g[s] = inf ? 0 : cv.take(M * C * 4);
    }
    for (int s = 0; s < 2; ++s) {
        const int N = s == 0 ? p->N2 : p->N3;
        const int64_t M = (int64_t)B * N, C = D[2 + s], hid = c.mlp_hidden[s];
        const int heads = c.rope_heads[s];
        if (M * C > maxMC) maxMC = M * C;
        const int64_t wide = hid > 3 * C ? hid : 3 * C;
        if (M * wide > maxM4C) maxM4C = M * wide;
        p->o_tok[s] = cv.take(M * C * 4);
        int64_t pp[2] = {0, 0};
        if (inf) {
            pp[0] = cv.take(M * C * 4);
            pp[1] = cv.take(M * C * 4);
        }
        for (size_t i = 0; i < p->rope[s].size(); ++i) {
            RopeBlk& k = p->rope[s][i];
            const bool share = (inf || ck) && i > 0;
            const RopeBlk& f = p->rope[s][0];
            if (i == 0) k.xin = p->o_tok[s];
            k.n1 = share ? f.n1 : cv.take(M * C * esz);
            k.mean1 = share ? f.mean1 : cv.take(M * 4);
            k.rstd1 = share ? f.rstd1 : cv.take(M * 4);
            k.qkvbuf = share ? f.qkvbuf : cv.take(M * 3 * C * esz);
            k.cos = cv.take((int64_t)p->HW[2 + s] * C / 2 * 4);
            if (c.rope_mode == LNX_ROPE_ROTATE) k.dsin = cv.take((int64_t)p->HW[2 + s] * C / 2 * 4);
            else k.dsin = inf ? 0 : cv.take((int64_t)2 * p->HW[2 + s] * C / 2 * 4);
            k.o = share ? f.o : cv.take(M * C * esz);
            k.lse = share ? f.lse : cv.take((int64_t)B * heads * N * 4);
            k.xmid = share ? f.xmid : cv.take(M * C * 4);
            k.n2 = share ? f.n2 : cv.take(M * C * esz);
            k.mean2 = share ? f.mean2 : cv.take(M * 4);
            k.rstd2 = share ? f.rstd2 : cv.take(M * 4);
            k.hpre = share ? f.hpre : cv.take(M * hid * esz);
            k.act = share ? f.act : cv.take(M * hid * esz);
            const int64_t outb = inf ? pp[i & 1] : cv.take(M * C * 4);
            if (i + 1 < p->rope[s].size()) p->rope[s][i + 1].xin = outb;
            else p->o_stage_out[2 + s] = outb;
        }
        p->o_g[2 + s] = inf ? 0 : cv.take(M * C * 4);
        for (auto& k : p->meta[s]) {
            k.t0 = cv.take((int64_t)B * 16 * 4);
            k.h0 = cv.take((int64_t)B * C * 4);
            k.x = cv.take((int64_t)B * C * 4);
            k.m0 = cv.take(B * 4);
            k.r0 = cv.take(B * 4);
            k.h1 = cv.take((int64_t)B * C * 4);
            k.n1 = cv.take((int64_t)B * C * 4);
            k.m1 = cv.take(B * 4);
            k.r1 = cv.take(B * 4);
            k.h2 = cv.take((int64_t)B * C * 4);
            k.m2 = cv.take(B * 4);
            k.r2 = cv.take(B * 4);
            if (!inf && p->chain_ok[s]) {
                k.dp2 = cv.take((int64_t)B * C * 4);
                k.dp1 = cv.take((int64_t)B * C * 4);
                k.dp0 = cv.take((int64_t)B * C * 4);
                k.part = cv.take(lnx_meta_heads_bwd_part_floats(B, (int)C) * 4);
            }
        }
    }
    {
        const int64_t M2 = (int64_t)B * p->N2;
        p->o_t1 = cv.take(M2 * D[2] * esz);
        p->o_t1_mean = cv.take(M2 * 4);
        p->o_t1_rstd = cv.take(M2 * 4);
        p->o_dt1 = inf ? 0 : cv.take(M2 * D[2] * esz);
        p->down[2].ln = cv.take((int64_t)B * p->HW[2] * D[2] * esz);
        p->down[2].mean = cv.take((int64_t)B * p->HW[2] * 4);
        p->down[2].rstd = cv.take((int64_t)B * p->HW[2] * 4);
        p->o_cl_hpre = cv.take((int64_t)B * D[2] * esz);
        p->o_cl_act = cv.take((int64_t)B * D[2] * esz);
        p->o_cl_u = cv.take((int64_t)B * D[3] * 4);
        p->o_cl_mean = cv.take(B * 4);
        p->o_cl_rstd = cv.take(B * 4);
        p->o_c1n = cv.take((int64_t)B * D[3] * 4);
        p->o_c2n = cv.take((int64_t)B * D[3] * 4);
        p->o_n2_mean = cv.take(B * 4);
        p->o_n2_rstd = cv.take(B * 4);
        p->o_agg = cv.take((int64_t)B * D[3] * 4);
        p->o_fin_mean = cv.take(B * 4);
        p->o_fin_rstd = cv.take(B * 4);
        p->o_feats = cv.take((int64_t)B * D[3] * 4);
        p->o_featsT = cv.take((int64_t)B * D[3] * esz);
        for (int i = 0; i < 6; ++i) p->o_tail[i] = cv.take((int64_t)B * D[3] * 4);
        for (int i = 0; i < 4; ++i) p->o_mtmp[i] = cv.take((int64_t)B * (D[3] > D[2] ? D[3] : D[2]) * 4);
        p->o_dlT = cv.take((p->logits_numel > 8 ? p->logits_numel : 8) * esz);
    }
    if (c.fp8) {
        int64_t mc = 0, mh = 0;
        for (int s = 0; s < 2; ++s) {
            const int64_t M = (int64_t)B * (s == 0 ? p->N2 : p->N3);
            if (M * D[2 + s] > mc) mc = M * D[2 + s];
            if (M * c.mlp_hidden[s] > mh) mh = M * c.mlp_hidden[s];
        }
        p->o_a8 = cv.take(mc);
        p->o_a8s = cv.take(mc / 32);
        p->o_h8 = cv.take(mh);
        p->o_h8s = cv.take(mh / 32);
    }
    p->lnws_floats = (int64_t)2048 * 2 * (D[3] > D[0] ? D[3] : D[0]);
    p->lnws_side_floats = (int64_t)256 * 2 * D[3];
    if (!inf) {
        p->o_lnws = cv.take(p->lnws_floats * 4);
        {
            const int64_t rows[5] = {(int64_t)B * p->HW[0], (int64_t)B * p->HW[1], (int64_t)B * p->N2, (int64_t)B * p->N3, (int64_t)B};
            const int64_t wide[5] = {D[0], D[1], D[2], D[3], D[3]};
            int64_t need = 0;
            for (int i = 0; i < 5; ++i) {
                int64_t wgs = (rows[i] + 7) / 8;
                if (wgs > 2048) wgs = 2048;
                if (wgs * 2 * wide[i] > need) need = wgs * 2 * wide[i];
            }
            p->lnws_defer_floats = need;
            p->o_lnws_defer = cv.take(need * 4 * LN_DEFER_SLOTS);
        }
        p->o_lnws_side = cv.take(p->lnws_side_floats * 4);
        p->o_tnws = cv.take((int64_t)LNX_TN_WS_FLOATS * 4 * TN_WS_SLOTS);
        {
            const int64_t cmax = D[0] > D[1] ? D[0] : D[1];
            p->lsws_floats = cmax * 4 * cmax + cmax;
            p->o_lsws = cv.take(p->lsws_floats * 4);
        }
        p->o_sA = cv.take(maxM4C * esz);
        if (any_fused) p->o_sB = cv.take(maxM4C * esz);
        p->o_sC = cv.take(maxMC * esz);
        p->o_sD = cv.take(maxMC * esz);
    }
    if (!inf) {
        int64_t gmax = 0, dmax = 0;
        for (int s = 0; s < 2; ++s) {
            const int N = s == 0 ? p->N2 : p->N3;
            const int64_t gsz = lnx_attn_bwd_ws_floats_hd(B, N, c.rope_heads[s], D[2 + s] / c.rope_heads[s]) * 4;
            const int64_t dsz = (int64_t)B * c.rope_heads[s] * N * 4;
            if (gsz > gmax) gmax = gsz;
            if (dsz > dmax) dmax = dsz;
        }
        p->gcos_floats = gmax / 4;
        p->o_gcos = cv.take(gmax * FREQ_DEFER_SLOTS);
        p->o_delta = cv.take(dmax);
    }
    for (int s = 0; s < 2; ++s) {
        const int64_t M = (int64_t)B * (s == 0 ? p->N2 : p->N3), C = D[2 + s], hid = c.mlp_hidden[s];
        for (auto& k : p->rope[s]) {
            k.dm_proj = p->dmask_bytes;
            k.dm_hid = k.dm_proj + M * C;
            k.dm_fc2 = k.dm_hid + M * hid;
            p->dmask_bytes = k.dm_fc2 + M * C;
            const int64_t N = s == 0 ? p->N2 : p->N3;
            k.dm_attn = p->amask_bytes;
            p->amask_bytes += (int64_t)B * c.rope_heads[s] * N * ((N + 63) / 64 * 64);
        }
    }
    p->ws_bytes = cv.cur;
    *out = p;
    return 0;
}

extern "C" int64_t lnx_plan_dropout_bytes(const lnx_plan* p) { return p ? p->dmask_bytes : 0; }
extern "C" int64_t lnx_plan_attn_dropout_bytes(const lnx_plan* p) { return p ? p->amask_bytes : 0; }

extern "C" int lnx_plan_set_attn_dropout(lnx_plan* p, const unsigned char* masks, float drop_rate) {
    if (!p) FAIL("lnx_plan_set_attn_dropout: null plan");
    if (masks == nullptr || drop_rate == 0.0f) {
        p->amask = nullptr;
        p->a_inv_keep = 1.0f;
        return 0;
    }
    if (!(drop_rate > 0.0f && drop_rate < 1.0f)) FAIL("lnx_plan_set_attn_dropout: drop_rate %g must be in [0, 1)", (double)drop_rate);
    if (p->c.inference) FAIL("lnx_plan_set_attn_dropout: dropout is a training-time operation; this is an inference plan");
    if ((((uintptr_t)masks) & 3) != 0) FAIL("lnx_plan_set_attn_dropout: the mask buffer must be 4-byte aligned");
    p->amask = masks;
    p->a_inv_keep = 1.0f / (1.0f - drop_rate);
    return 0;
}

extern "C" int lnx_plan_set_dropout(lnx_plan* p, const unsigned char* masks, float drop_rate) {
    if (!p) FAIL("lnx_plan_set_dropout: null plan");
    if (masks == nullptr || drop_rate == 0.0f) {
        p->dmask = nullptr;
        p->inv_keep = 1.0f;
        return 0;
    }
    if (!(drop_rate > 0.0f && drop_rate < 1.0f)) FAIL("lnx_plan_set_dropout: drop_rate %g must be in [0, 1)", (double)drop_rate);
    if (p->c.inference) FAIL("lnx_plan_set_dropout: dropout is a training-time operation; this is an inference plan");
    if (p->c.fp8) FAIL("lnx_plan_set_dropout: dropout is not available on fp8 plans");
    if ((((uintptr_t)masks) & 7) != 0) FAIL("lnx_plan_set_dropout: the mask buffer must be 8-byte aligned");
    p->dmask = masks;
    p->inv_keep = 1.0f / (1.0f - drop_rate);
    return 0;
}

static hipStream_t shared_stream(int which) {
    static std::mutex mu;
    static hipStream_t tab[2][64] = {};
    int dev = 0;
    if (hipGetDevice(&dev) != hipSuccess || dev < 0 || dev >= 64) return nullptr;
    std::lock_guard<std::mutex> lock(mu);
    if (!tab[which][dev] && hipStreamCreateWithFlags(&tab[which][dev], hipStreamNonBlocking) != hipSuccess) tab[which][dev] = nullptr;
    return tab[which][dev];
}

extern "C" void lnx_plan_destroy(lnx_plan* p) {
    if (!p) return;
    (void)lnx_gemm_tn_discard();
    (void)lnx_layernorm_bwd_discard();
    if (p->side) {
        (void)hipStreamSynchronize(p->side);
        (void)hipEventDestroy(p->ev_fork);
        (void)hipEventDestroy(p->ev_meta);
        for (int i = 0; i < 2; ++i) {
            (void)hipEventDestroy(p->ev_bfork[i]);
            (void)hipEventDestroy(p->ev_bjoin[i]);
        }
    }
    if (p->wgs) {
        (void)hipStreamSynchronize(p->wgs);
        for (int i = 0; i < 4; ++i) {
            (void)hipEventDestroy(p->ev_wf[i]);
            (void)hipEventDestroy(p->ev_wj[i]);
        }
    }
    for (hipEvent_t e : p->ev_pool) (void)hipEventDestroy(e);
    delete p;
}
extern "C" int64_t lnx_plan_workspace_bytes(const lnx_plan* p) { return p ? p->ws_bytes : 0; }
extern "C" int lnx_plan_num_params(const lnx_plan* p) { return p ? (int)p->names.size() : 0; }
extern "C" const char* lnx_plan_param_name(const lnx_plan* p, int i) {
    return (p && i >= 0 && i < (int)p->names.size()) ? p->names[i].c_str() : nullptr;
}
extern "C" int64_t lnx_plan_param_numel(const lnx_plan* p, int i) { return (p && i >= 0 && i < (int)p->numel.size()) ? p->numel[i] : -1; }
extern "C" int lnx_plan_num_drop_calls(const lnx_plan* p) { return p ? p->n_drop : 0; }
extern "C" int64_t lnx_plan_logits_numel(const lnx_plan* p) { return p ? p->logits_numel : 0; }
extern "C" int64_t lnx_plan_logits_offset(const lnx_plan* p, int t) { return (p && t >= 0 && t < p->c.n_tasks) ? p->logit_off[t] : -1; }
extern "C" int lnx_plan_logits_ld(const lnx_plan* p, int t) { return (p && t >= 0 && t < p->c.n_tasks) ? p->logit_ld[t] : -1; }

extern "C" int lnx_plan_bind(lnx_plan* p, const float* const* params, float* const* grads, void* workspace) {
    if (!p || !params || !workspace) FAIL("lnx_plan_bind: null argument");
    {
        static std::atomic<int> bound_dev{-1};
        int dev = -1;
        HIPRUN(hipGetDevice(&dev));
        int expect = -1;
        if (!bound_dev.compare_exchange_strong(expect, dev) && expect != dev)
            FAIL("lnx_plan_bind: this process already runs plans on device %d, now device %d is current: the library is one-process-per-GPU", expect, dev);
    }
    const int n = (int)p->names.size();
    p->P.assign(params, params + n);
    for (int i = 0; i < n; ++i)
        if (p->P[i] == nullptr || (((uintptr_t)p->P[i]) & 3) != 0) FAIL("lnx_plan_bind: parameter %s is null or misaligned", p->names[i].c_str());
    p->has_grads = grads != nullptr;
    if (grads) {
        p->G.assign(grads, grads + n);
        for (int i = 0; i < n; ++i)
            if (p->G[i] == nullptr) FAIL("lnx_plan_bind: gradient of %s is null", p->names[i].c_str());
    } else {
        p->G.assign(n, nullptr);
    }
    p->ws = reinterpret_cast<unsigned char*>(workspace);
    if ((((uintptr_t)p->ws) & 255) != 0) FAIL("lnx_plan_bind: workspace must be 256-byte aligned");
    int64_t arena_end = 0;
    for (OpW* w : p->all_w) {
        const int wes = w->f32 ? 4 : 2;
        const int64_t e1 = w->off + (int64_t)w->N * w->ld * wes;
        const int64_t e2 = w->ld_t ? w->off_t + (int64_t)w->K * w->ld_t * wes : 0;
        if (e1 > arena_end) arena_end = e1;
        if (e2 > arena_end) arena_end = e2;
    }
    HIPRUN(hipMemset(p->ws, 0, (size_t)arena_end));
    std::vector<lnx_prep_desc> d;
    int blk = 0;
    auto push_w = [&](OpW* w) {
        lnx_prep_desc e;
        memset(&e, 0, sizeof e);
        e.src = p->P[w->param];
        e.dst = p->ws + w->off;
        e.dst_t = w->ld_t ? p->ws + w->off_t : nullptr;
        e.rows = w->N;
// ... 624 lines not shown
        RUN(ln_fwd(c, B, C, 1e-5f, c.at<float>(p->o_stage_out[3]), LNX_F32, C, clsrow, p->norm_w[1], p->norm_b[1], c.at<float>(p->o_c2n), LNX_F32, C, IDM, nullptr,
                   0, c.at<float>(p->o_n2_mean), c.at<float>(p->o_n2_rstd)));
        const float* fin_in = c.at<float>(p->o_c2n);
        if (!cf.only_last_cls) {
            RUN(lnx_agg2_fwd(c.at<float>(p->o_c1n), c.at<float>(p->o_c2n), p->P[p->agg_w], p->P[p->agg_b], c.at<float>(p->o_agg), B, C, stream));
            fin_in = c.at<float>(p->o_agg);
        }
        RUN(ln_fwd(c, B, C, 1e-5f, fin_in, LNX_F32, C, IDM, p->fin_w, p->fin_b, c.at<float>(p->o_feats), LNX_F32, C, IDM, nullptr, 0, c.at<float>(p->o_fin_mean),
                   c.at<float>(p->o_fin_rstd)));
        if (feats) HIPRUN(hipMemcpyAsync(feats, c.at<float>(p->o_feats), (size_t)B * C * 4, hipMemcpyDeviceToDevice, (hipStream_t)stream));
        if (cf.n_tasks > 0) {
            RUN(lnx_scale_cast(c.at<float>(p->o_feats), C, IDM, nullptr, 0, c.at<void>(p->o_featsT), cf.dtype, C, B, C, stream));
            lnx_gemm_args hg[LNX_MAX_TASKS];
            for (int t = 0; t < cf.n_tasks; ++t) {
                hg[t] = gemm_base(c, B, cf.task_classes[t], C, c.at<void>(p->o_featsT), C, c.wptr(p->head_w[t]), p->head_w[t].ld, logits + p->logit_off[t],
                                  p->logit_ld[t], true);
                hg[t].bias = p->P[p->head_b[t]];
            }
            RUN(heads_nt(c, hg, cf.n_tasks, false));
        }
    }
    p->fwd_done = true;
    return 0;
}

namespace {

static inline bool wg_on(const lnx_plan* p) { return p->wgs != nullptr && p->wgs_on; }
Ctx wg_ctx(const Ctx& c) { return Ctx{c.p, wg_on(c.p) ? (void*)c.p->wgs : c.st, c.dt}; }
int wg_fork(const Ctx& c, int j) {
    if (!wg_on(c.p)) return 0;
    HIPRUN(hipEventRecord(c.p->ev_wf[j], (hipStream_t)c.st));
    HIPRUN(hipStreamWaitEvent(c.p->wgs, c.p->ev_wf[j], 0));
    return 0;
}
int wg_done(const Ctx& c, int j) {
    if (!wg_on(c.p)) return 0;
    HIPRUN(hipEventRecord(c.p->ev_wj[j], c.p->wgs));
    return 0;
}
int wg_join(const Ctx& c, int j) {
    if (!wg_on(c.p)) return 0;
    HIPRUN(hipStreamWaitEvent((hipStream_t)c.st, c.p->ev_wj[j], 0));
    return 0;
}

int rope_block_bwd(const Ctx& c, int s, int i, float* g, bool have_dy) {
    lnx_plan* p = c.p;
    RopeBlk& k = p->rope[s][i];
    const int B = p->c.batch, C = p->c.dims[2 + s], heads = p->c.rope_heads[s], hid = p->c.mlp_hidden[s];
    const int N = s == 0 ? p->N2 : p->N3, M = B * N, E = p->E;
    void* sA = c.at<void>(p->o_sA);
    void* sC = c.at<void>(p->o_sC);
    void* sD = c.at<void>(p->o_sD);
    Timed span(c, 8, 2.0 * rope_block_flops(B, N, C, hid));
    const Ctx cw = wg_ctx(c);
    auto wfork = [&](int j) { return wg_fork(c, j); };
    auto wdone = [&](int j) { return wg_done(c, j); };
    auto wjoin = [&](int j) { return wg_join(c, j); };
    if (!have_dy) RUN(lnx_scale_cast(g, C, IDM, p->drop_ptr(p->drop_mlp[s][i]), N, sC, c.dt, C, M, C, c.st));
    if (p->dmask) RUN(lnx_dropout_mul(sC, c.dt, p->dmask + k.dm_fc2, p->inv_keep, M, C, c.st));
    RUN(wfork(0));
    RUN(wgrad(cw, M, C, hid, sC, C, c.at<void>(k.act), hid, k.fc2.param, k.fc2b, hid, 0, 0));
    RUN(wdone(0));
    lnx_gemm_args a = gemm_base(c, M, hid, C, sC, C, c.wtptr(k.fc2), k.fc2.ld_t, sA, hid, false);
    a.act = fp8_rows(p, M, C) ? LNX_ACT_GELU_BWD : LNX_ACT_MUL_AUX; a.aux = c.at<void>(k.hpre); a.ldaux = hid;
    const bool qpass = getenv("LNX_FP8_DGRAD_QPASS") != nullptr;
    const bool mx_dgrad = c.dt == LNX_BF16 && fp8_rows(p, M, C) && k.fc2.off8ts != 0 && k.proj.off8ts != 0 && !p->dmask && C % 128 == 0 && !qpass;
    RUN(linear_dgrad(c, a, k.fc2, !(have_dy && p->dy8_ready), p->o_a8, p->o_a8s, p->o_h8, p->o_h8s));
    p->dy8_ready = false;
    if (p->dmask) RUN(lnx_dropout_mul(sA, c.dt, p->dmask + k.dm_hid, p->inv_keep, M, hid, c.st));
    RUN(wfork(1));
    RUN(wgrad(cw, M, hid, C, sA, hid, c.at<void>(k.n2), C, k.fc1.param, k.fc1b, C, 0, 1));
    RUN(wdone(1));
    a = gemm_base(c, M, C, hid, sA, hid, c.wtptr(k.fc1), k.fc1.ld_t, sD, C, false);
    RUN(linear_dgrad(c, a, k.fc1, false, p->o_h8, p->o_h8s));
    RUN(wjoin(0));
    Dx2 d2;
    d2.p = sC; d2.rowscale = p->drop_ptr(p->drop_attn[s][i]); d2.rps = N;
    if (mx_dgrad) {
        d2.p8 = c.at<void>(p->o_a8); d2.p8s = c.at<void>(p->o_a8s);
    }
    RUN(ln_bwd(c, M, C, sD, c.dt, C, IDM, c.at<float>(k.xmid), LNX_F32, C, IDM, k.n2w, k.n2b, c.at<float>(k.mean2), c.at<float>(k.rstd2), g, g, LNX_F32, C, false, d2));
    if (p->dmask) RUN(lnx_dropout_mul(sC, c.dt, p->dmask + k.dm_proj, p->inv_keep, M, C, c.st));
    RUN(wfork(2));
    RUN(wgrad(cw, M, C, C, sC, C, c.at<void>(k.o), C, k.proj.param, k.projb, C, 0, 2));
    RUN(wdone(2));
    a = gemm_base(c, M, C, C, sC, C, c.wtptr(k.proj), k.proj.ld_t, sD, C, false);
    RUN(linear_dgrad(c, a, k.proj, !mx_dgrad, p->o_a8, p->o_a8s));
    RUN(wjoin(1));
    lnx_attn_bwd_args ab;
    memset(&ab, 0, sizeof ab);
    ab.dtype = c.dt; ab.B = B; ab.N = N; ab.E = E; ab.heads = heads; ab.head_dim = C / heads;
    ab.qkv = c.at<void>(k.qkvbuf); ab.cos_tab = c.at<float>(k.cos); ab.o = c.at<void>(k.o); ab.lse = c.at<float>(k.lse);
    ab.d_o = sD; ab.dqkv = sA; ab.freq_ws = c.at<float>(p->o_gcos); ab.delta = c.at<float>(p->o_delta);
    if (p->freq_defer && E < N) {
        if (p->freq_pending == FREQ_DEFER_SLOTS) {
            RUN(lnx_attn_bwd_flush(c.st));
            p->freq_pending = 0;
        }
        ab.freq_ws = c.at<float>(p->o_gcos) + (int64_t)p->freq_pending * p->gcos_floats;
        ab.defer_freqs = 1;
        ++p->freq_pending;
    }
    ab.dsin_tab = c.at<float>(k.dsin); ab.dfreqs = p->G[k.freqs];
    if (p->c.rope_mode == LNX_ROPE_ROTATE) {
        ab.rope_mode = LNX_ROPE_ROTATE; ab.sin_tab = c.at<float>(k.dsin); ab.dsin_tab = nullptr; ab.grid_w = p->W[2 + s];
    }
    if (p->amask) {
        ab.drop_mask = p->amask + k.dm_attn; ab.drop_inv_keep = p->a_inv_keep;
    }
    {
        Timed t(c, 3, 14.0 * B * (double)N * N * C);
        RUN(lnx_attn_bwd(&ab, c.st));
    }
    RUN(wfork(3));
    RUN(wgrad(cw, M, 3 * C, C, sA, 3 * C, c.at<void>(k.n1), C, k.qkv.param, k.qkvb, C, 0, 3));
    RUN(lnx_gemm_tn_flush(cw.st));
    RUN(wdone(3));
    RUN(wjoin(2));
    a = gemm_base(c, M, C, 3 * C, sA, 3 * C, c.wtptr(k.qkv), k.qkv.ld_t, sC, C, false);
    RUN(gemm_nt_t(c, &a));
    Dx2 d1;
    if (i > 0) {
        d1.p = sC; d1.rowscale = p->drop_ptr(p->drop_mlp[s][i - 1]); d1.rps = N;
        if (mx_dgrad) {
            d1.p8 = c.at<void>(p->o_a8); d1.p8s = c.at<void>(p->o_a8s);
            p->dy8_ready = true;
        }
    }
    RUN(ln_bwd(c, M, C, sC, c.dt, C, IDM, c.at<float>(k.xin), LNX_F32, C, IDM, k.n1w, k.n1b, c.at<float>(k.mean1), c.at<float>(k.rstd1), g, g, LNX_F32, C, false, d1));
    RUN(wjoin(3));
    return 0;
}

int conv_block_bwd(const Ctx& c, int s, int i, float* g) {
    lnx_plan* p = c.p;
    ConvBlk& k = p->conv[s][i];
    const int B = p->c.batch, H = p->H[s], W = p->W[s], C = p->c.dims[s];
    const int M = B * H * W;
    void* sA = c.at<void>(p->o_sA);
    void* sC = c.at<void>(p->o_sC);
    void* sD = c.at<void>(p->o_sD);
    Timed span(c, 9, 4.0 * M * C * (8.0 * C + 49.0));
    bool forked = false, joined = false;
    if (k.fused) {
        void* sB = c.at<void>(p->o_sB);
        lnx_convmlp_bwd_args f;
        memset(&f, 0, sizeof f);
        f.dtype = c.dt; f.M = M; f.C = C;
        f.g = g; f.ln = c.at<void>(k.ln); f.z = k.keep_z ? c.at<void>(k.z) : nullptr; f.w1 = c.wptr(k.w1); f.b1 = p->P[k.b1];
        f.w2t = c.wtptr(k.w2); f.w1t = c.wtptr(k.w1); f.gamma = p->P[k.gamma];
        f.rowscale = p->drop_ptr(p->drop_conv[s][i]); f.rows_per_sample = H * W;
        f.act = sB; f.dh = sA; f.dz = sC; f.dln = sD; f.dgamma = p->G[k.gamma];
        f.dz_plain = k.keep_z ? 0 : 1;
        if (k.fused_ln) {
            f.y = c.at<void>(k.y); f.ln_w = p->P[k.lnw]; f.mean = c.at<float>(k.mean); f.rstd = c.at<float>(k.rstd);
            f.d_ln_w = p->G[k.lnw]; f.d_ln_b = p->G[k.lnb];
            f.ws = c.at<float>(p->o_lnws); f.ws_floats = p->lnws_floats;
            if (p->ln_defer && p->o_lnws_defer != 0 && lnx_convmlp_bwd_ws_floats(C, M) <= p->lnws_defer_floats) {
                if (p->ln_pending == LN_DEFER_SLOTS) {
                    RUN(lnx_layernorm_bwd_flush(c.st));
                    p->ln_pending = 0;
                }
                f.ws = c.at<float>(p->o_lnws_defer) + (int64_t)p->ln_pending * p->lnws_defer_floats;
                f.ws_floats = p->lnws_defer_floats;
                f.ln_defer = 1;
                ++p->ln_pending;
            }
        }
        {
            Timed t(c, 7, 2.0 * M * C * 4 * C * 3);
            RUN(lnx_convmlp_bwd(&f, c.st));
        }
        const Ctx cw = wg_ctx(c);
        RUN(wg_fork(c, 0));
        forked = true;
        if (k.keep_z) {
            RUN(wgrad(cw, M, C, 4 * C, sC, C, sB, 4 * C, k.w2.param, k.b2, 4 * C, 0, 0));
            RUN(wgrad(cw, M, 4 * C, C, sA, 4 * C, c.at<void>(k.ln), C, k.w1.param, k.b1, C, 0, 1));
            RUN(lnx_gemm_tn_flush(cw.st));
        } else {
            float* S = c.at<float>(p->o_lsws);
            float* T = S + (int64_t)C * 4 * C;
            HIPRUN(hipMemsetAsync(S, 0, ((size_t)C * 4 * C + C) * 4, (hipStream_t)cw.st));
            RUN(wgrad_into(cw, M, C, 4 * C, sC, C, sB, 4 * C, S, T, 4 * C, 0));
            RUN(wgrad(cw, M, 4 * C, C, sA, 4 * C, c.at<void>(k.ln), C, k.w1.param, k.b1, C, 0, 1));
            RUN(lnx_gemm_tn_flush(cw.st));
            RUN(lnx_layerscale_apply_wgrad(S, T, 4 * C, p->P[k.w2.param], p->P[k.b2], 4 * C, p->P[k.gamma], p->G[k.w2.param], p->G[k.b2], 4 * C, p->G[k.gamma], C, 4 * C, cw.st));
        }
        RUN(wg_done(c, 0));
        if (!k.fused_ln) {
            RUN(wg_join(c, 0));
            joined = true;
        }
    } else {
        RUN(lnx_layerscale_bwd(g, c.at<void>(k.z), c.dt, p->P[k.gamma], p->drop_ptr(p->drop_conv[s][i]), H * W, sC, p->G[k.gamma], M, C, c.st));
        RUN(wgrad(c, M, C, 4 * C, sC, C, c.at<void>(k.act), 4 * C, k.w2.param, k.b2, 4 * C));
        lnx_gemm_args a = gemm_base(c, M, 4 * C, C, sC, C, c.wtptr(k.w2), k.w2.ld_t, sA, 4 * C, false);
        static const bool keep_h = getenv("LNX_CONV_HPRE") != nullptr;
        a.act = keep_h ? LNX_ACT_GELU_BWD : LNX_ACT_MUL_AUX; a.aux = c.at<void>(k.hpre); a.ldaux = 4 * C;
        RUN(gemm_nt_t(c, &a));
        RUN(wgrad(c, M, 4 * C, C, sA, 4 * C, c.at<void>(k.ln), C, k.w1.param, k.b1, C));
        a = gemm_base(c, M, C, 4 * C, sA, 4 * C, c.wtptr(k.w1), k.w1.ld_t, sD, C, false);
        RUN(gemm_nt_t(c, &a));
    }
    void* dy = sD;
    if (!k.fused_ln) {
        RUN(ln_bwd(c, M, C, sD, c.dt, C, IDM, c.at<void>(k.y), c.dt, C, IDM, k.lnw, k.lnb, c.at<float>(k.mean), c.at<float>(k.rstd), nullptr, sC, c.dt, C, false));
        dy = sC;
    }
    lnx_dwconv_wgrad_args w;
    memset(&w, 0, sizeof w);
    w.B = B; w.H = H; w.W = W; w.C = C;
    w.x = c.at<float>(k.xin); w.x_dtype = LNX_F32; w.dy = dy; w.dy_dtype = c.dt;
    w.dw = p->G[k.dww]; w.db = p->G[k.dwb];
    {
        Timed t(c, 5, (double)M * C * (4 + p->esz));
        RUN(lnx_dwconv7_wgrad(&w, c.st));
    }
    lnx_dwconv_args d;
    memset(&d, 0, sizeof d);
    d.B = B; d.H = H; d.W = W; d.C = C;
    d.x = dy; d.x_dtype = c.dt; d.w49 = c.at<float>(k.w49); d.bias = nullptr; d.flip = 1; d.res = g; d.y = g; d.y_dtype = LNX_F32;
    {
        Timed t(c, 4, (double)M * C * (8 + p->esz));
        RUN(lnx_dwconv7_fwd(&d, c.st));
    }
    if (forked && !joined) RUN(wg_join(c, 0));
    return 0;
}

int downsample_bwd(const Ctx& c, int i, const float* gout, int64_t ldg, lnx_rowmap gmap, const void* x, int xdt, int64_t ldx, lnx_rowmap xm, void* dx, int dxdt,
                   int64_t lddx) {
    lnx_plan* p = c.p;
    Down& d = p->down[i];
    const int B = p->c.batch, Hin = p->H[i], Win = p->W[i], Cin = p->c.dims[i], Cout = p->c.dims[i + 1];
    const int Min = B * Hin * Win, Mout = Min / 4;
    void* sA = c.at<void>(p->o_sA);
    void* sC = c.at<void>(p->o_sC);
    RUN(lnx_scale_cast(gout, ldg, gmap, nullptr, 0, sC, c.dt, Cout, Mout, Cout, c.st));
    lnx_wgrad_args w;
    memset(&w, 0, sizeof w);
    w.dtype = c.dt; w.M = Mout; w.N = Cout; w.K = 4 * Cin;
    w.dY = sC; w.lddy = Cout; w.A = c.at<void>(d.ln); w.a_mode = LNX_ADDR_PATCH2; w.Hin = Hin; w.Win = Win; w.Cin = Cin;
    w.dW = p->G[d.w.param]; w.lddw = 4 * Cin; w.k_perm_c = Cin; w.db = p->G[d.cb];
    w.ws = c.at<float>(p->o_tnws); w.ws_floats = LNX_TN_WS_FLOATS;
    {
        Timed t(c, 1, 2.0 * Mout * Cout * 4 * Cin);
        RUN(lnx_gemm_tn(&w, c.st));
    }
    lnx_gemm_args a = gemm_base(c, Mout, 4 * Cin, Cout, sC, Cout, c.wtptr(d.w), d.w.ld_t, sA, 0, false);
    a.c_mode = LNX_ADDR_PATCH2; a.Hin = Hin; a.Win = Win; a.Cin = Cin;
    RUN(gemm_nt_t(c, &a));
    RUN(ln_bwd(c, Min, Cin, sA, c.dt, Cin, IDM, x, xdt, ldx, xm, d.lnw, d.lnb, c.at<float>(d.mean), c.at<float>(d.rstd), nullptr, dx, dxdt, lddx, false));
    return 0;
}

int meta_head_bwd(const Ctx& cc, int s, int m, const float* g, int N) {
    const Ctx c{cc.p, cc.st, LNX_F32};
    lnx_plan* p = c.p;
    MetaHead& k = p->meta[s][m];
    const int B = p->c.batch, C = p->c.dims[2 + s];
    float* dtok = c.at<float>(p->o_mtmp[0]);
    void* t1 = c.at<void>(p->o_mtmp[1]);
    void* t2 = c.at<void>(p->o_mtmp[2]);
    float* dxf = c.at<float>(p->o_mtmp[3]);
    const lnx_rowmap rm = {1, N - 1, 1 + m};
    RUN(lnx_scale_cast(g, C, rm, nullptr, 0, dtok, LNX_F32, C, B, C, c.st));
    RUN(ln_bwd(c, B, C, dtok, LNX_F32, C, IDM, c.at<void>(k.h2), c.dt, C, IDM, k.nf2w, k.nf2b, c.at<float>(k.m2), c.at<float>(k.r2), nullptr, t1, c.dt, C, true));
    RUN(wgrad(c, B, C, C, t1, C, c.at<void>(k.n1), C, k.w2.param, k.b2, C));
    lnx_gemm_args a = gemm_base(c, B, C, C, t1, C, c.wtptr(k.w2), k.w2.ld_t, t2, C, false);
    RUN(gemm_nt_t(c, &a));
    RUN(ln_bwd(c, B, C, t2, c.dt, C, IDM, c.at<void>(k.h1), c.dt, C, IDM, k.nf1w, k.nf1b, c.at<float>(k.m1), c.at<float>(k.r1), nullptr, t1, c.dt, C, true));
    RUN(wgrad(c, B, C, C, t1, C, c.at<void>(k.x), C, k.w1.param, k.b1, C));
    a = gemm_base(c, B, C, C, t1, C, c.wtptr(k.w1), k.w1.ld_t, dxf, C, true);
    a.res = dtok; a.ldres = C;
    RUN(gemm_nt_t(c, &a));
    RUN(ln_bwd(c, B, C, dxf, LNX_F32, C, IDM, c.at<void>(k.h0), c.dt, C, IDM, k.lnw0, k.lnb0, c.at<float>(k.m0), c.at<float>(k.r0), nullptr, t1, c.dt, C, true));
    RUN(wgrad(c, B, C, 16, t1, C, c.at<void>(k.t0), 16, k.w0.param, k.b0, k.dim, k.dim));
    return 0;
}

int tokens_bwd(const Ctx& c, int s, const float* g) {
    lnx_plan* p = c.p;
    const int B = p->c.batch, C = p->c.dims[2 + s], N = s == 0 ? p->N2 : p->N3;
    const lnx_rowmap clsmap = {1, N - 1, 0};
    RUN(lnx_colsum_rows(g, C, clsmap, p->G[p->cls[s]], B, C, c.st));
    hipStream_t const mst = meta_stream(p);
    p->meta_forked[s] = mst != nullptr;
    if (mst) {
        HIPRUN(hipEventRecord(p->ev_bfork[s], (hipStream_t)c.st));
        HIPRUN(hipStreamWaitEvent(mst, p->ev_bfork[s], 0));
        const Ctx cs{p, (void*)mst, c.dt};
        if (p->chain_ok[s]) RUN(meta_chain_bwd(cs, s, g));
        else
            for (int m = 0; m < p->c.n_meta; ++m) RUN(meta_head_bwd(cs, s, m, g, N));
        HIPRUN(hipEventRecord(p->ev_bjoin[s], mst));
    } else if (p->chain_ok[s]) {
        RUN(meta_chain_bwd(c, s, g));
    } else {
        for (int m = 0; m < p->c.n_meta; ++m) RUN(meta_head_bwd(c, s, m, g, N));
    }
    return 0;
}

int conv_block_restore(const Ctx& c, int s, int i) {
    lnx_plan* p = c.p;
    if (!p->c.recompute || p->resident[s] == i) return 0;
    const int nb = p->c.conv_depths[s];
    float* xout = i + 1 < nb ? c.at<float>(p->conv[s][i + 1].xin) : c.at<float>(p->o_stage_out[s]);
    return conv_block_fwd(c, s, i, nullptr, xout);
}
int rope_block_restore(const Ctx& c, int s, int i) {
    lnx_plan* p = c.p;
    if (!p->c.recompute || p->resident[2 + s] == i) return 0;
    const int nb = p->c.rope_depths[s];
    float* xout = i + 1 < nb ? c.at<float>(p->rope[s][i + 1].xin) : c.at<float>(p->o_stage_out[2 + s]);
    p->dy8_ready = false;
    return rope_block_fwd(c, s, i, xout);
}

int ln_flush(const Ctx& c) {
    lnx_plan* p = c.p;
    if (p->ln_pending > 0) {
        RUN(lnx_layernorm_bwd_flush(c.st));
        p->ln_pending = 0;
    }
    if (p->freq_pending > 0) {
        RUN(lnx_attn_bwd_flush(c.st));
        p->freq_pending = 0;
// ... 270 lines not shown
```

linnaeus_amd/ops.py:

```python
from __future__ import annotations

import ctypes as C
from typing import Optional, Tuple

import torch

from . import _lib as L
from ._lib import F32, BF16

_TORCH_DT = {F32: torch.float32, BF16: torch.bfloat16}


def code_of(t: torch.Tensor) -> int:
    if t.dtype == torch.float32:
        return F32
    if t.dtype == torch.bfloat16:
        return BF16
    raise L.LnxError(f"unsupported tensor dtype {t.dtype}")


def torch_dtype(code: int) -> torch.dtype:
    return _TORCH_DT[code]


# ... 206 lines not shown
    B, H, W, Cc = x.shape
    a = L.DwconvArgs()
    a.B, a.H, a.W, a.C = B, H, W, Cc
    a.x, a.x_dtype, a.w49, a.bias = _p(x), code_of(x), _p(w49), _p(bias)
    a.flip, a.res, a.y, a.y_dtype = int(flip), _p(res), _p(y), code_of(y)
    L.check(L.lib().lnx_dwconv7_fwd(C.byref(a), _stream()), "lnx_dwconv7_fwd")
    return y


def dwconv7_wgrad(x, dy, dw, db):
    B, H, W, Cc = x.shape
    a = L.DwconvWgradArgs()
    a.B, a.H, a.W, a.C = B, H, W, Cc
    a.x, a.x_dtype, a.dy, a.dy_dtype, a.dw, a.db = _p(x), code_of(x), _p(dy), code_of(dy), _p(dw), _p(db)
    L.check(L.lib().lnx_dwconv7_wgrad(C.byref(a), _stream()), "lnx_dwconv7_wgrad")


def rope_cos_table(freqs, H, W, out=None, dsin=None):
    heads, half = freqs.shape[1], freqs.shape[2]
    if out is None:
        out = torch.empty(H * W, heads, half, device=freqs.device, dtype=torch.float32)
    L.check(L.lib().lnx_rope_cos_table_hd(_p(freqs), heads, 2 * half, H, W, _p(out), _p(dsin) if dsin is not None else None, _stream()),
            "lnx_rope_cos_table_hd")
    return out


def rope_cossin_table(freqs, H, W):
    heads, half = freqs.shape[1], freqs.shape[2]
    cos = torch.empty(H * W, heads, half, device=freqs.device, dtype=torch.float32)
    sin = torch.empty_like(cos)
    L.check(L.lib().lnx_rope_cossin_table_hd(_p(freqs), heads, 2 * half, H, W, _p(cos), _p(sin), None, _stream()), "lnx_rope_cossin_table_hd")
    return cos, sin


def rope_cos_tables(entries):
    arr = (L.RopeTable * len(entries))()
    for t, (freqs, H, W, out, dsin, *rest) in zip(arr, entries):
        t.freqs, t.cos_out, t.dsin_out = _p(freqs), _p(out), _p(dsin) if dsin is not None else None
        t.heads, t.H, t.W, t.head_dim = freqs.shape[1], H, W, 2 * freqs.shape[2]
        if rest and rest[0] is not None:
            t.rope_mode, t.sin_out = L.ROPE_ROTATE, _p(rest[0])
    L.check(L.lib().lnx_rope_cos_tables(arr, len(entries), _stream()), "lnx_rope_cos_tables")


def attn_bwd_ws_floats(B, N, heads, head_dim=64):
    fn = L.lib().lnx_attn_bwd_ws_floats_hd
    fn.restype = C.c_int64
    return int(fn(B, N, heads, head_dim))


def _head_dim(qkv, heads, head_dim):
    if head_dim is not None:
        return int(head_dim)
    return qkv.shape[-1] // (3 * heads) if qkv.dim() >= 2 and qkv.shape[-1] % (3 * heads) == 0 else 64


def attn_fwd(qkv, cos_tab, o, lse, B, N, E, heads, *, drop_mask=None, drop_rate=0.0, head_dim=None, sin_tab=None):
    a = L.AttnArgs()
    if sin_tab is not None:
        a.rope_mode, a.sin_tab = L.ROPE_ROTATE, _p(sin_tab)
    a.dtype, a.B, a.N, a.E, a.heads = code_of(qkv), B, N, E, heads
    a.head_dim = _head_dim(qkv, heads, head_dim)
    a.qkv, a.cos_tab, a.o, a.lse = _p(qkv), _p(cos_tab), _p(o), _p(lse)
    if drop_mask is not None:
        a.drop_mask, a.drop_inv_keep = _p(drop_mask), 1.0 / (1.0 - drop_rate)
    L.check(L.lib().lnx_attn_fwd(C.byref(a), _stream()), "lnx_attn_fwd")


def attn_bwd(qkv, cos_tab, o, lse, d_o, dqkv, delta, B, N, E, heads, *, dsin=None, dfreqs=None, drop_mask=None, drop_rate=0.0, defer_freqs=False,
             head_dim=None, sin_tab=None, grid_w=0):
    a = L.AttnBwdArgs()
    if sin_tab is not None:
        a.rope_mode, a.sin_tab, a.grid_w, a.dfreqs = L.ROPE_ROTATE, _p(sin_tab), int(grid_w), _p(dfreqs) if dfreqs is not None else None
    a.dtype, a.B, a.N, a.E, a.heads = code_of(qkv), B, N, E, heads
    a.head_dim = _head_dim(qkv, heads, head_dim)
    a.qkv, a.cos_tab, a.o, a.lse = _p(qkv), _p(cos_tab), _p(o), _p(lse)
    ws = torch.empty(max(attn_bwd_ws_floats(B, N, heads, a.head_dim), 1), device=qkv.device, dtype=torch.float32)
    a.d_o, a.dqkv, a.freq_ws, a.delta = _p(d_o), _p(dqkv), _p(ws), _p(delta)
    if dsin is not None:
        a.dsin_tab, a.dfreqs = _p(dsin), _p(dfreqs)
    if drop_mask is not None:
        a.drop_mask, a.drop_inv_keep = _p(drop_mask), 1.0 / (1.0 - drop_rate)
    a.defer_freqs = int(bool(defer_freqs))
    L.check(L.lib().lnx_attn_bwd(C.byref(a), _stream()), "lnx_attn_bwd")
    return ws


def attn_bwd_flush():
    L.check(L.lib().lnx_attn_bwd_flush(_stream()), "lnx_attn_bwd_flush")


def im2col_stem(x, patches):
    B, Cin, H, W = x.shape
    L.check(L.lib().lnx_im2col_stem(_p(x), B, Cin, H, W, _p(patches), code_of(patches), patches.stride(0), _stream()), "lnx_im2col_stem")


def stem_fwd(x, w, bias, ln_w, ln_b, y, *, patches=None, pre=None, mean=None, rstd=None, eps=1e-6):
    a = L.StemArgs()
    a.x, a.w, a.bias, a.ln_w, a.ln_b = _p(x), _p(w), _p(bias), _p(ln_w), _p(ln_b)
    a.patches, a.pre, a.y, a.mean, a.rstd = _p(patches), _p(pre), _p(y), _p(mean), _p(rstd)
    a.B, a.Cin, a.H, a.W = x.shape
    a.Cout, a.eps = w.shape[0], eps
    L.check(L.lib().lnx_stem_fwd(C.byref(a), _stream()), "lnx_stem_fwd")


def scale_cast(inp, out, M, Cc, *, ldin=None, in_map=None, rowscale=None, rows_per_sample=0, ldout=None):
    L.check(L.lib().lnx_scale_cast(_p(inp), C.c_int64(ldin if ldin is not None else inp.stride(-2)), _map(in_map), _p(rowscale), rows_per_sample,
                                   _p(out), code_of(out), C.c_int64(ldout if ldout is not None else out.stride(-2)), M, Cc, _stream()), "lnx_scale_cast")


def layerscale_bwd(g, z, gamma, rowscale, rows_per_sample, dz, dgamma, M, Cc):
    L.check(L.lib().lnx_layerscale_bwd(_p(g), _p(z), code_of(z), _p(gamma), _p(rowscale), rows_per_sample, _p(dz), _p(dgamma), M, Cc, _stream()),
            "lnx_layerscale_bwd")


def fill_rows(vec, out, ldout, row_map, M, Cc):
    L.check(L.lib().lnx_fill_rows(_p(vec), _p(out), C.c_int64(ldout), _map(row_map), M, Cc, _stream()), "lnx_fill_rows")


def colsum_rows(inp, ldin, row_map, out, M, Cc):
    L.check(L.lib().lnx_colsum_rows(_p(inp), C.c_int64(ldin), _map(row_map), _p(out), M, Cc, _stream()), "lnx_colsum_rows")


def agg2_fwd(a, b, w2, bias1, out, M, Cc):
    L.check(L.lib().lnx_agg2_fwd(_p(a), _p(b), _p(w2), _p(bias1), _p(out), M, Cc, _stream()), "lnx_agg2_fwd")


def agg2_bwd(dout, a, b, w2, da, db, dw2, dbias1, M, Cc):
    L.check(L.lib().lnx_agg2_bwd(_p(dout), _p(a), _p(b), _p(w2), _p(da), _p(db), _p(dw2), _p(dbias1), M, Cc, _stream()), "lnx_agg2_bwd")


def pack_meta(meta, off, dim, out):
    L.check(L.lib().lnx_pack_meta(_p(meta), meta.shape[1], off, dim, _p(out), code_of(out), meta.shape[0], _stream()), "lnx_pack_meta")


def convmlp_fwd(ln, w1, b1, w2, b2, gamma, x, out, *, rowscale=None, rows_per_sample=0, z=None, y=None, ln_w=None, ln_b=None, ln_eps=1e-6,
                ln_out=None, mean=None, rstd=None):
    a = L.ConvMlpArgs()
    src = ln if y is None else y
    a.dtype, a.M, a.C = code_of(src), src.shape[0], src.shape[1]
    a.ln, a.w1, a.b1, a.w2, a.b2, a.gamma = _p(ln), _p(w1), _p(b1), _p(w2), _p(b2), _p(gamma)
    a.rowscale, a.rows_per_sample, a.x, a.out, a.z = _p(rowscale), rows_per_sample, _p(x), _p(out), _p(z)
    a.y, a.ln_w, a.ln_b, a.ln_eps, a.ln_out, a.mean, a.rstd = _p(y), _p(ln_w), _p(ln_b), ln_eps, _p(ln_out), _p(mean), _p(rstd)
    L.check(L.lib().lnx_convmlp_fwd(C.byref(a), _stream()), "lnx_convmlp_fwd")
    return out


def layerscale_apply_wgrad(s, t, w, b, gamma, dw, db, dgamma):
    L.check(L.lib().lnx_layerscale_apply_wgrad(_p(s), _p(t), C.c_int64(s.stride(0)), _p(w), _p(b), C.c_int64(w.stride(0)), _p(gamma), _p(dw), _p(db),
                                               C.c_int64(dw.stride(0)), _p(dgamma), w.shape[0], w.shape[1], _stream()), "lnx_layerscale_apply_wgrad")


def convmlp_bwd(g, ln, z, w1, b1, w2t, w1t, gamma, act, dh, dz, dln, dgamma, *, rowscale=None, rows_per_sample=0, y=None, ln_w=None, mean=None,
                rstd=None, d_ln_w=None, d_ln_b=None, ws=None, dz_plain=False):
    a = L.ConvMlpBwdArgs()
    a.dtype, a.M, a.C = code_of(ln), ln.shape[0], ln.shape[1]
    a.g, a.ln, a.z, a.w1, a.b1, a.w2t, a.w1t, a.gamma = _p(g), _p(ln), _p(z), _p(w1), _p(b1), _p(w2t), _p(w1t), _p(gamma)
    a.rowscale, a.rows_per_sample = _p(rowscale), rows_per_sample
    a.act, a.dh, a.dz, a.dln, a.dgamma = _p(act), _p(dh), _p(dz), _p(dln), _p(dgamma)
    a.y, a.ln_w, a.mean, a.rstd, a.d_ln_w, a.d_ln_b = _p(y), _p(ln_w), _p(mean), _p(rstd), _p(d_ln_w), _p(d_ln_b)
    a.ws, a.ws_floats = _p(ws), (ws.numel() if ws is not None else 0)
    a.dz_plain = int(dz_plain)
    L.check(L.lib().lnx_convmlp_bwd(C.byref(a), _stream()), "lnx_convmlp_bwd")


def _meta_head_buffers(B, C_, dev):
    f = lambda *shape: torch.empty(*shape, device=dev, dtype=torch.float32)
    return {"t0": f(B, 16), "h0": f(B, C_), "x": f(B, C_), "h1": f(B, C_), "n1": f(B, C_), "h2": f(B, C_),
            "m0": f(B), "r0": f(B), "m1": f(B), "r1": f(B), "m2": f(B), "r2": f(B)}


def meta_heads_fwd(meta, heads, tok, eps=1e-5):
    B = meta.shape[0]
    arr = (L.MetaHeadArgs * len(heads))()
    keep, saved = [], []
    for i, h in enumerate(heads):
        C_ = h["w1"].shape[0]
        w0p = torch.zeros(C_, 16, device=meta.device)
        w0p[:, :h["dim"]] = h["w0"]
        bufs = _meta_head_buffers(B, C_, meta.device)
        t = tok[i] if isinstance(tok, (list, tuple)) else tok
        a = arr[i]
        a.B, a.C, a.dim, a.off, a.meta, a.meta_width, a.eps = B, C_, h["dim"], h["off"], _p(meta), meta.shape[1], eps
        a.w0, a.ldw0, a.b0, a.ln0_w, a.ln0_b = _p(w0p), 16, _p(h["b0"]), _p(h["ln0_w"]), _p(h["ln0_b"])
        a.w1, a.ldw1, a.b1, a.ln1_w, a.ln1_b = _p(h["w1"]), C_, _p(h["b1"]), _p(h["ln1_w"]), _p(h["ln1_b"])
        a.w2, a.ldw2, a.b2, a.ln2_w, a.ln2_b = _p(h["w2"]), C_, _p(h["b2"]), _p(h["ln2_w"]), _p(h["ln2_b"])
        for k_, v in bufs.items():
            setattr(a, k_, _p(v))
        a.tok, a.tok_row_stride, a.tok_row_offset = _p(t), t.shape[1] * C_, h["slot"] * C_
        keep.append(w0p)
        saved.append(bufs)
    L.check(L.lib().lnx_meta_heads_fwd(arr, len(heads), _stream()), "lnx_meta_heads_fwd")
    return saved


def meta_heads_bwd(g, heads, saved, grads):
    arr = (L.MetaHeadBwdArgs * len(heads))()
    keep = []
    for i, (h, sv, gr) in enumerate(zip(heads, saved, grads)):
        C_ = h["w1"].shape[0]
        gi = g[i] if isinstance(g, (list, tuple)) else g
        B = gi.shape[0]
        w1t, w2t = h["w1"].t().contiguous(), h["w2"].t().contiguous()
        dp = [torch.empty(B, C_, device=gi.device) for _ in range(3)]
        part = torch.empty(L.lib().lnx_meta_heads_bwd_part_floats(B, C_), device=gi.device)
        a = arr[i]
        a.B, a.C, a.dim = B, C_, h["dim"]
        a.g, a.g_row_stride, a.g_row_offset = _p(gi), gi.shape[1] * C_, h["slot"] * C_
        a.w1t, a.ldw1t, a.w2t, a.ldw2t = _p(w1t), C_, _p(w2t), C_
        a.ln0_w, a.ln1_w, a.ln2_w = _p(h["ln0_w"]), _p(h["ln1_w"]), _p(h["ln2_w"])
        for k_, v in sv.items():
            setattr(a, k_, _p(v))
        a.dp2, a.dp1, a.dp0, a.part = _p(dp[0]), _p(dp[1]), _p(dp[2]), _p(part)
        for k_ in ("w0", "b0", "ln0_w", "ln0_b", "w1", "b1", "ln1_w", "ln1_b", "w2", "b2", "ln2_w", "ln2_b"):
            setattr(a, "d_" + k_, _p(gr[k_]))
        keep += [w1t, w2t, part] + dp
    L.check(L.lib().lnx_meta_heads_bwd(arr, len(heads), _stream()), "lnx_meta_heads_bwd")
    torch.cuda.current_stream().synchronize()


def metrics_table_sizes(n_tasks: int, n_bins0: int = 0, n_bins1: int = 0) -> Tuple[int, int]:
    nc, ns = C.c_int64(), C.c_int64()
    L.check(L.lib().lnx_metrics_table_sizes(n_tasks, n_bins0, n_bins1, C.byref(nc), C.byref(ns)), "lnx_metrics_table_sizes")
    return nc.value, ns.value


def metrics_update(logits, targets, counts, sums, *, num_classes=None, is_null=None, losses=None, subset_ids=(), n_bins=()):
    T = len(logits)
    if not 1 <= T <= L.METRICS_MAX_TASKS or len(targets) != T:
        raise L.LnxError(f"metrics_update: {T} tasks (1..{L.METRICS_MAX_TASKS}), {len(targets)} targets")
    a = L.MetricsArgs()
    a.dtype, a.B, a.n_tasks = code_of(logits[0]), logits[0].shape[0], T
    for t in range(T):
        x, tg = logits[t], targets[t]
        nul = is_null[t] if is_null is not None else None
        ls = losses[t] if losses is not None else None
        if x.dim() != 2 or x.shape[0] != a.B or code_of(x) != a.dtype or (x.shape[1] > 1 and x.stride(1) != 1):
            raise L.LnxError(f"metrics_update: task {t} logits must be [B, C] rows of one dtype with unit column stride, got {tuple(x.shape)} {x.dtype} strides {x.stride()}")
        if tg.dtype != torch.int64 or tg.shape != (a.B,) or not tg.is_contiguous():
            raise L.LnxError(f"metrics_update: task {t} target must be contiguous int64 [B]")
        if nul is not None and (nul.dtype not in (torch.uint8, torch.bool) or nul.shape != (a.B,) or not nul.is_contiguous()):
            raise L.LnxError(f"metrics_update: task {t} is_null must be contiguous uint8 / bool [B]")
        if ls is not None and (ls.dtype != torch.float32 or ls.shape != (a.B,) or not ls.is_contiguous()):
            raise L.LnxError(f"metrics_update: task {t} loss must be contiguous fp32 [B]")
        k = a.task[t]
        k.logits, k.ld, k.C = _p(x), (x.stride(0) if a.B > 1 else x.shape[1]), (num_classes[t] if num_classes is not None else x.shape[1])
        k.target, k.is_null, k.loss = _p(tg), _p(nul), _p(ls)
    for s, (ids, nb) in enumerate(zip(subset_ids, n_bins)):
        if ids is None:
            continue
        if ids.dtype != torch.int64 or ids.shape != (a.B,) or not ids.is_contiguous():
            raise L.LnxError(f"metrics_update: subset ids {s} must be contiguous int64 [B]")
        a.subset_ids[s], a.n_bins[s] = ids.data_ptr(), nb
    nc, ns = metrics_table_sizes(T, a.n_bins[0], a.n_bins[1])
    if counts.dtype != torch.int64 or sums.dtype != torch.float64 or counts.numel() < nc or sums.numel() < ns or not (counts.is_contiguous() and sums.is_contiguous()):
        raise L.LnxError(f"metrics_update: tables must be contiguous int64 [>= {nc}] / float64 [>= {ns}]")
    a.counts, a.sums = _p(counts), _p(sums)
    L.check(L.lib().lnx_metrics_update(C.byref(a), _stream()), "lnx_metrics_update")


def predict_topk(logits, parents, *, K, null_index=0, id_maps=None, k_per_sample=None, consistency=True, num_classes=None, out=None):
    T = len(logits)
    if not 1 <= T <= L.METRICS_MAX_TASKS or len(parents) != T:
        raise L.LnxError(f"predict_topk: {T} tasks (1..{L.METRICS_MAX_TASKS}), {len(parents)} parent tables")
    nulls = list(null_index) if isinstance(null_index, (list, tuple)) else [null_index] * T
    if len(nulls) != T or (id_maps is not None and len(id_maps) != T):
        raise L.LnxError(f"predict_topk: {T} tasks need {T} null indices / id maps")
    a = L.PredictArgs()
    a.dtype, a.B, a.n_tasks, a.K, a.consistency = code_of(logits[0]), logits[0].shape[0], T, int(K), int(bool(consistency))
    dev = logits[0].device
    for t in range(T):
        x, par = logits[t], parents[t]
        ids = id_maps[t] if id_maps is not None else None
        if x.dim() != 2 or x.shape[0] != a.B or code_of(x) != a.dtype or (x.shape[1] > 1 and x.stride(1) != 1):
            raise L.LnxError(f"predict_topk: task {t} logits must be [B, C] rows of one dtype with unit column stride, got {tuple(x.shape)} {x.dtype} strides {x.stride()}")
        Ct = int(num_classes[t]) if num_classes is not None else x.shape[1]
        if Ct > x.shape[1]:
            raise L.LnxError(f"predict_topk: task {t} has {x.shape[1]} logit columns, {Ct} classes")
        if par is not None and (par.dtype != torch.int32 or par.shape != (Ct,) or not par.is_contiguous()):
            raise L.LnxError(f"predict_topk: task {t} parent table must be contiguous int32 [{Ct}]")
        if ids is not None and (ids.dtype != torch.int64 or ids.shape != (Ct,) or not ids.is_contiguous()):
            raise L.LnxError(f"predict_topk: task {t} id map must be contiguous int64 [{Ct}]")
        k = a.task[t]
        k.logits, k.ld, k.C = _p(x), (x.stride(0) if a.B > 1 else x.shape[1]), Ct
        k.parent, k.id_map, k.null_index = _p(par), _p(ids), (-1 if nulls[t] is None else int(nulls[t]))
    if k_per_sample is not None:
        if k_per_sample.dtype != torch.int32 or k_per_sample.shape != (a.B,) or not k_per_sample.is_contiguous():
            raise L.LnxError("predict_topk: k_per_sample must be contiguous int32 [B]")
        a.k_per_sample = _p(k_per_sample)
    if out is None:
        out = (torch.empty(a.B, T, a.K, dtype=torch.int64, device=dev), torch.empty(a.B, T, a.K, dtype=torch.float32, device=dev),
               torch.empty(a.B, T, dtype=torch.int32, device=dev), torch.empty(a.B, T, dtype=torch.int32, device=dev))
    for o, dt, shape in zip(out, (torch.int64, torch.float32, torch.int32, torch.int32), ((a.B, T, a.K), (a.B, T, a.K), (a.B, T), (a.B, T))):
        if o.dtype != dt or tuple(o.shape) != shape or not o.is_contiguous():
            raise L.LnxError(f"predict_topk: outputs must be contiguous int64 / fp32 [B, T, K] and int32 [B, T] x 2, got {tuple(o.shape)} {o.dtype}")
    a.ids, a.probs, a.count, a.flags = (_p(o) for o in out)
    L.check(L.lib().lnx_predict(C.byref(a), _stream()), "lnx_predict")
    return tuple(out)


def preprocess_images(blob, blob_bytes, images, images_off, n, H, W, filter_code, mean, std, scratch, out):
    if out.dtype != torch.float32 or tuple(out.shape) != (n, 3, H, W) or not out.is_contiguous():
        raise L.LnxError(f"preprocess_images: out must be contiguous fp32 [{n}, 3, {H}, {W}], got {tuple(out.shape)} {out.dtype}")
    if blob.dtype != torch.uint8 or (scratch is not None and scratch.dtype != torch.uint8):
        raise L.LnxError("preprocess_images: blob and scratch are uint8 buffers")
    a = L.PreprocessArgs()
    a.n, a.H, a.W, a.filter = int(n), int(H), int(W), int(filter_code)
    a.images = C.cast(images, C.POINTER(L.PreprocessImage))
    a.blob, a.blob_bytes, a.images_off = _p(blob), int(blob_bytes), int(images_off)
    a.scratch, a.scratch_bytes = _p(scratch), (0 if scratch is None else scratch.numel())
    a.mean[:] = [float(v) for v in mean]
    a.std[:] = [float(v) for v in std]
    a.out = _p(out)
    L.check(L.lib().lnx_preprocess(C.byref(a), _stream()), "lnx_preprocess")
    return out
```

Baseline: 13270 images/sec.

## Recompute ConvMLP hidden activations inside a fused weight-gradient kernel for C=96

Adds a fused ConvMLP weight-gradient kernel for C=96. It recomputes the hidden GELU activation and its gradient from the saved LayerNorm output and dz tiles, then accumulates dW1, dW2, db1 and db2 with MFMA, using transposed LDS reads and per-block slabs followed by a reduce kernel. The backward kernel no longer writes the 4C-wide activation and hidden-gradient tensors to global memory; when gamma is folded in, it writes an extra dz copy instead. This removes large memory traffic and two split-K GEMMs and shrinks scratch buffers, at the cost of redoing the first-layer matmuls in the weight-gradient pass. The path is on by default behind an environment flag.

```diff
diff --git a/include/lnx.h b/include/lnx.h
--- a/include/lnx.h
+++ b/include/lnx.h
@@ -637,10 +637,36 @@
     int64_t ws_floats;
     int dz_plain;
     int ln_defer;
+    void* dz_gamma;
 } lnx_convmlp_bwd_args;
 int lnx_convmlp_bwd(const lnx_convmlp_bwd_args* args, void* stream);
 int64_t lnx_convmlp_bwd_ws_floats(int C, int M);
 
+typedef struct lnx_convmlp_wgrad_args {
+    int dtype, M, C;
+    const void* ln;
+    const void* dz;
+    const void* dz_w;
+    const void* w1;
+    const float* b1;
+    const void* w2t;
+    float* dw1;
+    int64_t lddw1;
+    float* db1;
+    float* dw2;
+    int64_t lddw2;
+    float* db2;
+    float* ws;
+    int64_t ws_floats;
+} lnx_convmlp_wgrad_args;
+#define LNX_CONVMLP_WGRAD_WS_FLOATS (256 * (2 * 192 * 96 + 192 + 96))
+int lnx_convmlp_wgrad_supported(int dtype, int C);
+int lnx_convmlp_wgrad(const lnx_convmlp_wgrad_args* args, void* stream);
+typedef struct lnx_convmlp_wgrad_launch {
+    int grid, pairs, rows_per_tile;
+    int64_t ws_floats;
+} lnx_convmlp_wgrad_launch;
+int lnx_convmlp_wgrad_query(int C, int M, lnx_convmlp_wgrad_launch* out);
 
 #define LNX_MAX_META 8
 #define LNX_MAX_TASKS 16
diff --git a/linnaeus_amd/_lib.py b/linnaeus_amd/_lib.py
--- a/linnaeus_amd/_lib.py
+++ b/linnaeus_amd/_lib.py
@@ -175,6 +175,7 @@
         _lib.lnx_last_error.restype = C.c_char_p
         _lib.lnx_nt_kernel_launches.restype = C.c_int64
         _lib.lnx_convmlp_bwd_ws_floats.restype = C.c_int64
+        _lib.lnx_plan_workspace_bytes.restype = C.c_int64
         _lib.lnx_meta_heads_bwd_part_floats.restype = C.c_int64
         if hasattr(_lib, "lnx_ademamix_step"):
             _lib.lnx_ademamix_step.argtypes = [C.c_void_p, C.c_void_p, C.c_int, C.c_int, C.POINTER(AdEMAMixHyper), C.c_void_p, C.c_float, C.c_void_p]
@@ -196,6 +197,9 @@
             _lib.lnx_preprocess_scratch_bytes.restype = C.c_int64
             _lib.lnx_preprocess.argtypes = [C.POINTER(PreprocessArgs), C.c_void_p]
             _lib.lnx_preprocess.restype = C.c_int
+        if hasattr(_lib, "lnx_convmlp_wgrad"):
+            _lib.lnx_convmlp_wgrad.argtypes = [C.POINTER(ConvMlpWgradArgs), C.c_void_p]
+            _lib.lnx_convmlp_wgrad_query.argtypes = [C.c_int, C.c_int, C.POINTER(ConvMlpWgradLaunch)]
         if hasattr(_lib, "lnx_layernorm_fwd_query"):
             _lib.lnx_layernorm_fwd_query.argtypes = [C.POINTER(LnArgs), C.POINTER(LnLaunch)]
             _lib.lnx_layernorm_bwd_query.argtypes = [C.POINTER(LnBwdArgs), C.POINTER(LnLaunch)]
@@ -231,6 +235,7 @@
     "lnx_mix_rows", "lnx_mix_meta",
     "lnx_aug_pointwise", "lnx_aug_saturation", "lnx_aug_rowstat", "lnx_aug_rescale", "lnx_aug_affine", "lnx_aug_stencil", "lnx_erase_rects", "lnx_u8hwc_to_f32chw",
     "lnx_convmlp_supported", "lnx_convmlp_fwd", "lnx_convmlp_bwd", "lnx_convmlp_bwd_ws_floats",
+    "lnx_convmlp_wgrad_supported", "lnx_convmlp_wgrad", "lnx_convmlp_wgrad_query",
     "lnx_plan_create", "lnx_plan_destroy", "lnx_plan_workspace_bytes", "lnx_plan_num_params", "lnx_plan_param_name",
     "lnx_plan_param_numel", "lnx_plan_num_drop_calls", "lnx_plan_logits_numel", "lnx_plan_logits_offset", "lnx_plan_logits_ld",
     "lnx_plan_bind", "lnx_plan_forward", "lnx_plan_backward", "lnx_plan_backward_into", "lnx_plan_segment_params", "lnx_plan_profile_begin", "lnx_plan_profile_end", "lnx_plan_profile_begin_spans", "lnx_plan_profile_end_ex", "lnx_plan_set_wgrad_stream", "lnx_plan_set_meta_stream",
@@ -374,8 +379,21 @@
         ("act", C.c_void_p), ("dh", C.c_void_p), ("dz", C.c_void_p), ("dln", C.c_void_p), ("dgamma", C.c_void_p),
         ("y", C.c_void_p), ("ln_w", C.c_void_p), ("mean", C.c_void_p), ("rstd", C.c_void_p), ("d_ln_w", C.c_void_p), ("d_ln_b", C.c_void_p),
         ("ws", C.c_void_p), ("ws_floats", C.c_int64),
-        ("dz_plain", C.c_int), ("ln_defer", C.c_int),
-    ]
+        ("dz_plain", C.c_int), ("ln_defer", C.c_int), ("dz_gamma", C.c_void_p),
+    ]
+
+
+class ConvMlpWgradArgs(C.Structure):
+    _fields_ = [
+        ("dtype", C.c_int), ("M", C.c_int), ("C", C.c_int),
+        ("ln", C.c_void_p), ("dz", C.c_void_p), ("dz_w", C.c_void_p), ("w1", C.c_void_p), ("b1", C.c_void_p), ("w2t", C.c_void_p),
+        ("dw1", C.c_void_p), ("lddw1", C.c_int64), ("db1", C.c_void_p), ("dw2", C.c_void_p), ("lddw2", C.c_int64), ("db2", C.c_void_p),
+        ("ws", C.c_void_p), ("ws_floats", C.c_int64),
+    ]
+
+
+class ConvMlpWgradLaunch(C.Structure):
+    _fields_ = [("grid", C.c_int), ("pairs", C.c_int), ("rows_per_tile", C.c_int), ("ws_floats", C.c_int64)]
 
 
 class StemArgs(C.Structure):
diff --git a/linnaeus_amd/csrc/api.cpp b/linnaeus_amd/csrc/api.cpp
--- a/linnaeus_amd/csrc/api.cpp
+++ b/linnaeus_amd/csrc/api.cpp
@@ -19,7 +19,7 @@
 }
 
 extern "C" const char* lnx_last_error(void) { return g_err; }
-extern "C" int lnx_version(void) { return 107; }
+extern "C" int lnx_version(void) { return 108; }
 extern "C" int lnx_device_cus(void) {
     int dev = 0;
     if (hipGetDevice(&dev) != hipSuccess) return -1;
diff --git a/linnaeus_amd/csrc/convmlp.hip b/linnaeus_amd/csrc/convmlp.hip
--- a/linnaeus_amd/csrc/convmlp.hip
+++ b/linnaeus_amd/csrc/convmlp.hip
@@ -23,6 +23,7 @@
     unsigned char* act;
     unsigned char* dh;
     unsigned char* dz;
+    unsigned char* dzg;
     unsigned char* dln;
     float* dgamma;
     int M, C, rps;
@@ -902,7 +903,7 @@
     if (reset_ctr && lane == 0) sched_reset(ctr);
 }
 
-template <int NK, int MT, bool ST, bool LNB, bool DG>
+template <int NK, int MT, int ST, bool LNB, bool DG>
 __global__ __launch_bounds__(512) void convmlp_bwd_res_kernel(const CmP p) {
     constexpr int C = Geo<NK>::C;
     constexpr int CT = Geo<NK>::CT;
@@ -1008,6 +1009,7 @@
                 }
                 zf[mt][ks] = dzv.raw;
                 st16(p.dz + ((int64_t)m * C + c) * 2, dzs.raw);
+                if constexpr (ST == 2) st16(p.dzg + ((int64_t)m * C + c) * 2, dzv.raw);
             }
         }
         if (dyn) drawn = sched_draw_counted(ctr);
@@ -1047,7 +1049,7 @@
                 pd[mt][0] = pack8(da[0][mt], da[1][mt]);
                 pd[mt][1] = pack8(da[2][mt], da[3][mt]);
                 const int m = min(m_base + mt * 16 + s, p.M - 1);
-                if constexpr (ST) {
+                if constexpr (ST == 1) {
                     const int64_t off = ((int64_t)m * (4 * C) + 64 * j + 8 * g) * 2;
                     st16(p.act + off, pa0);
                     st16(p.act + off + 64, pa1);
@@ -1168,7 +1170,7 @@
     hipLaunchKernelGGL(ln_partials_reduce_kernel, dim3(cdiv(2 * p.C, 256), nwg >= 64 ? 64 : 1), dim3(256), 0, st, p.part, nwg, p.C, p.dlnw, p.dlnb);
     return 0;
 }
-template <int NK, int MT, bool ST, bool LNB, bool DG>
+template <int NK, int MT, int ST, bool LNB, bool DG>
 int launch_bwd_res_t(const CmP& p, hipStream_t st) {
     const size_t lds = 2 * (4 * Geo<NK>::C / 64) * Geo<NK>::PART + 9 * Geo<NK>::C * sizeof(float);
     static bool attr = false;
@@ -1188,11 +1190,14 @@
 template <int NK, int MT>
 int launch_bwd_res(const CmP& p, hipStream_t st) {
     if (p.zin == nullptr) {
-        if (p.y) return p.act ? launch_bwd_res_t<NK, MT, true, true, false>(p, st) : launch_bwd_res_t<NK, MT, false, true, false>(p, st);
-        return p.act ? launch_bwd_res_t<NK, MT, true, false, false>(p, st) : launch_bwd_res_t<NK, MT, false, false, false>(p, st);
-    }
-    if (p.y) return p.act ? launch_bwd_res_t<NK, MT, true, true, true>(p, st) : launch_bwd_res_t<NK, MT, false, true, true>(p, st);
-    return p.act ? launch_bwd_res_t<NK, MT, true, false, true>(p, st) : launch_bwd_res_t<NK, MT, false, false, true>(p, st);
+        if constexpr (NK == 3) {
+            if (p.dzg) return p.y ? launch_bwd_res_t<NK, MT, 2, true, false>(p, st) : launch_bwd_res_t<NK, MT, 2, false, false>(p, st);
+        }
+        if (p.y) return p.act ? launch_bwd_res_t<NK, MT, 1, true, false>(p, st) : launch_bwd_res_t<NK, MT, 0, true, false>(p, st);
+        return p.act ? launch_bwd_res_t<NK, MT, 1, false, false>(p, st) : launch_bwd_res_t<NK, MT, 0, false, false>(p, st);
+    }
+    if (p.y) return p.act ? launch_bwd_res_t<NK, MT, 1, true, true>(p, st) : launch_bwd_res_t<NK, MT, 0, true, true>(p, st);
+    return p.act ? launch_bwd_res_t<NK, MT, 1, false, true>(p, st) : launch_bwd_res_t<NK, MT, 0, false, true>(p, st);
 }
 
 template <int NK, int MT, int NW, bool LNF>
@@ -1276,6 +1281,9 @@
               "lnx_convmlp_bwd: null operand (z may be NULL: dgamma is then not produced here; with z, dgamma is required)");
     LNX_CHECK((a->act == nullptr) == (a->dh == nullptr), "lnx_convmlp_bwd: act and dh must both be given or both be NULL");
     LNX_CHECK(lnx_convmlp_supported(a->dtype, a->C), "lnx_convmlp_bwd: unsupported dtype %d / C %d", a->dtype, a->C);
+    if (a->dz_gamma)
+        LNX_CHECK(a->dz_plain != 0 && a->z == nullptr && a->act == nullptr && a->C == 96,
+                  "lnx_convmlp_bwd: dz_gamma goes with dz_plain, without z, act and dh, at C = 96 (the operands of lnx_convmlp_wgrad)");
     LNX_CHECK(a->M > 0, "lnx_convmlp_bwd: empty");
     if (a->rowscale) LNX_CHECK(a->rows_per_sample > 0, "lnx_convmlp_bwd: rowscale needs rows_per_sample");
     if (a->y) LNX_CHECK(a->ln_w && a->mean && a->rstd && a->d_ln_w && a->d_ln_b && a->ws, "lnx_convmlp_bwd: the fused LayerNorm form needs ln_w, mean, rstd, d_ln_w, d_ln_b and ws");
@@ -1287,6 +1295,7 @@
     p.act = (unsigned char*)a->act; p.dh = (unsigned char*)a->dh; p.dz = (unsigned char*)a->dz; p.dln = (unsigned char*)a->dln; p.dgamma = a->dgamma;
     p.M = a->M; p.C = a->C; p.rps = a->rows_per_sample > 0 ? a->rows_per_sample : 1;
     p.dz_plain = a->dz_plain != 0;
+    p.dzg = (unsigned char*)a->dz_gamma;
     hipStream_t st = (hipStream_t)stream;
     int rc = 0;
     switch (a->C) {
diff --git a/linnaeus_amd/csrc/convmlp_wgrad.hip b/linnaeus_amd/csrc/convmlp_wgrad.hip
--- /dev/null
+++ b/linnaeus_amd/csrc/convmlp_wgrad.hip
@@ -0,0 +1,269 @@
+#include "common.hpp"
+#include "../../include/lnx.h"
+
+namespace {
+
+constexpr int WG_NW = 12;
+constexpr int WG_HID = 16 * WG_NW;
+constexpr int WG_ROWS = 64;
+constexpr int WG_PITCH = 208;
+constexpr int WG_TENSOR = WG_ROWS * WG_PITCH;
+constexpr int WG_BUF = 3 * WG_TENSOR;
+constexpr int WG_C = 96;
+constexpr int WG_SLAB = 2 * WG_HID * WG_C + WG_HID + WG_C;
+
+typedef short wg_s16x4 __attribute__((ext_vector_type(4)));
+
+struct WgP {
+    const unsigned char* ln;
+    const unsigned char* dz;
+    const unsigned char* dzw;
+    const unsigned char* w1;
+    const unsigned char* w2t;
+    const float* b1;
+    float* ws;
+    int M, pairs;
+};
+
+__device__ __forceinline__ uint4 wg_pack8(const f32x4_t& lo, const f32x4_t& hi) {
+    Vec16<bf16_t> v;
+#pragma unroll
+    for (int j = 0; j < 4; ++j) {
+        v.set(j, lo[j]);
+        v.set(4 + j, hi[j]);
+    }
+    return v.raw;
+}
+__device__ __forceinline__ f32x4_t wg_mfma(const uint4& a, const uint4& b, const f32x4_t& acc) {
+    return __builtin_amdgcn_mfma_f32_16x16x32_bf16(__builtin_bit_cast(bf16x8_t, a), __builtin_bit_cast(bf16x8_t, b), acc, 0, 0, 0);
+}
+__device__ __forceinline__ float wg_sum8(const uint4& v) {
+    Vec16<bf16_t> t;
+    t.raw = v;
+    return ((t.get(0) + t.get(1)) + (t.get(2) + t.get(3))) + ((t.get(4) + t.get(5)) + (t.get(6) + t.get(7)));
+}
+
+__device__ __forceinline__ void wg_role(int& pair, int& half) {
+    const int b = (int)blockIdx.x;
+    if ((gridDim.x & 15) == 0) {
+        half = (b >> 3) & 1;
+        pair = (b >> 4) * 8 + (b & 7);
+    } else {
+        half = b & 1;
+        pair = b >> 1;
+    }
+}
+
+template <int NK, bool DUAL>
+__global__ __launch_bounds__(64 * WG_NW) void convmlp_wgrad_kernel(const WgP p) {
+    constexpr int ZW = DUAL ? 2 : 1;
+    constexpr int C = 32 * NK;
+    constexpr int CT = C / 16;
+    static_assert(C == WG_C, "tile staging and slab layout are written for C = 96");
+    extern __shared__ __attribute__((aligned(16))) unsigned char smem[];
+    const int lane = threadIdx.x & 63;
+    const int wave = __builtin_amdgcn_readfirstlane(threadIdx.x >> 6);
+    const int s = lane & 15, g = lane >> 4;
+    int pair, half;
+    wg_role(pair, half);
+    const int nl0 = wave * 16;
+    const int n0 = half * WG_HID + nl0;
+
+    uint4 w1f[NK], w2f[NK];
+#pragma unroll
+    for (int ks = 0; ks < NK; ++ks) {
+        w1f[ks] = ld16(p.w1 + ((int64_t)(n0 + s) * C + ks * 32 + 8 * g) * 2);
+        w2f[ks] = ld16(p.w2t + ((int64_t)(n0 + s) * C + ks * 32 + 8 * g) * 2);
+    }
+    const float bias = p.b1[n0 + s];
+    const f32x4_t bv[2] = {f32x4_t{bias, bias, bias, bias}, f32x4_t{bias, bias, bias, bias}};
+
+    const int srow = (int)threadIdx.x / 12, spiece = (int)threadIdx.x % 12;
+    const int ntile = (p.M + WG_ROWS - 1) / WG_ROWS;
+    auto fetch = [&](uint4 (&r)[3], int tile) __attribute__((always_inline)) {
+        const int m = tile * WG_ROWS + srow;
+        const int64_t off = (int64_t)(m < p.M ? m : p.M - 1) * (C * 2) + spiece * 16;
+        r[0] = ld16(p.ln + off);
+        r[1] = ld16(p.dz + off);
+        if constexpr (DUAL) r[2] = ld16(p.dzw + off);
+        else r[2] = make_uint4(0u, 0u, 0u, 0u);
+        if (m >= p.M) r[0] = r[1] = r[2] = make_uint4(0u, 0u, 0u, 0u);
+    };
+    auto stash = [&](const uint4 (&r)[3], int buf) __attribute__((always_inline)) {
+        unsigned char* d = smem + buf * WG_BUF + srow * WG_PITCH + spiece * 16;
+#pragma unroll
+        for (int q = 0; q < (DUAL ? 3 : 2); ++q) *reinterpret_cast<uint4*>(d + q * WG_TENSOR) = r[q];
+    };
+
+    f32x4_t a1[CT], a2[CT];
+#pragma unroll
+    for (int ct = 0; ct < CT; ++ct) a1[ct] = a2[ct] = f32x4_t{0.f, 0.f, 0.f, 0.f};
+    float dbs = 0.f;
+    float tsum = 0.f;
+
+    uint4 nx[3];
+    int tile = pair;
+    fetch(nx, tile);
+    stash(nx, 0);
+    __syncthreads();
+    int buf = 0;
+    for (; tile < ntile; tile += p.pairs) {
+        const int nt = tile + p.pairs;
+        fetch(nx, nt < ntile ? nt : tile);
+        const unsigned char* tb = smem + buf * WG_BUF;
+#pragma unroll
+        for (int r0 = 0; r0 < WG_ROWS; r0 += 32) {
+            f32x4_t h[2], da[2];
+#pragma unroll
+            for (int mt = 0; mt < 2; ++mt) {
+                const unsigned char* row = tb + (r0 + 16 * mt + s) * WG_PITCH + 16 * g;
+                h[mt] = da[mt] = f32x4_t{0.f, 0.f, 0.f, 0.f};
+#pragma unroll
+                for (int ks = 0; ks < NK; ++ks) {
+                    const uint4 xf = *reinterpret_cast<const uint4*>(row + ks * 64);
+                    const uint4 zf = *reinterpret_cast<const uint4*>(row + WG_TENSOR + ks * 64);
+                    h[mt] = wg_mfma(xf, w1f[ks], h[mt]);
+                    da[mt] = wg_mfma(zf, w2f[ks], da[mt]);
+                }
+            }
+            gelu4_bias_grad_n<2>(h, bv, da);
+            const uint4 pa = wg_pack8(h[0], h[1]), pd = wg_pack8(da[0], da[1]);
+            dbs += wg_sum8(pd);
+            const unsigned char* trb = tb + (r0 + 4 * g + (s >> 2)) * WG_PITCH + (s & 3) * 8;
+#pragma unroll
+            for (int ct = 0; ct < CT; ++ct) {
+                const wg_s16x4 xl = __builtin_amdgcn_ds_read_tr16_b64_v4i16((__attribute__((address_space(3))) wg_s16x4*)(trb + ct * 32));
+                const wg_s16x4 xh = __builtin_amdgcn_ds_read_tr16_b64_v4i16((__attribute__((address_space(3))) wg_s16x4*)(trb + ct * 32 + 16 * WG_PITCH));
+                const wg_s16x4 zl = __builtin_amdgcn_ds_read_tr16_b64_v4i16((__attribute__((address_space(3))) wg_s16x4*)(trb + ZW * WG_TENSOR + ct * 32));
+                const wg_s16x4 zh = __builtin_amdgcn_ds_read_tr16_b64_v4i16((__attribute__((address_space(3))) wg_s16x4*)(trb + ZW * WG_TENSOR + ct * 32 + 16 * WG_PITCH));
+                const uint2 xl2 = __builtin_bit_cast(uint2, xl), xh2 = __builtin_bit_cast(uint2, xh);
+                const uint2 zl2 = __builtin_bit_cast(uint2, zl), zh2 = __builtin_bit_cast(uint2, zh);
+                const uint4 xb = make_uint4(xl2.x, xl2.y, xh2.x, xh2.y), zb = make_uint4(zl2.x, zl2.y, zh2.x, zh2.y);
+                a1[ct] = wg_mfma(pd, xb, a1[ct]);
+                a2[ct] = wg_mfma(pa, zb, a2[ct]);
+                if (wave == ct) tsum += wg_sum8(zb);
+            }
+        }
+        stash(nx, buf ^ 1);
+        __syncthreads();
+        buf ^= 1;
+    }
+
+    float* slab = p.ws + (size_t)(2 * pair + half) * WG_SLAB;
+#pragma unroll
+    for (int ct = 0; ct < CT; ++ct) {
+#pragma unroll
+        for (int r = 0; r < 4; ++r) slab[(nl0 + 4 * g + r) * C + ct * 16 + s] = a1[ct][r];
+        *reinterpret_cast<float4*>(slab + WG_HID * C + (ct * 16 + s) * WG_HID + nl0 + 4 * g) = make_float4(a2[ct][0], a2[ct][1], a2[ct][2], a2[ct][3]);
+    }
+    dbs += __shfl_xor(dbs, 16, 64);
+    dbs += __shfl_xor(dbs, 32, 64);
+    tsum += __shfl_xor(tsum, 16, 64);
+    tsum += __shfl_xor(tsum, 32, 64);
+    if (g == 0) {
+        slab[2 * WG_HID * C + nl0 + s] = dbs;
+        if (wave < CT) slab[2 * WG_HID * C + WG_HID + wave * 16 + s] = tsum;
+    }
+}
+
+struct WgR {
+    const float* ws;
+    float* dw1;
+    float* db1;
+    float* dw2;
+    float* db2;
+    int64_t lddw1, lddw2;
+    int pairs;
+};
+__global__ __launch_bounds__(256) void convmlp_wgrad_reduce_kernel(const WgR p) {
+    constexpr int C = WG_C, HID = 4 * WG_C, HALF = WG_HID * WG_C;
+    const int e = (int)blockIdx.x * 256 + (int)threadIdx.x;
+    if (e >= 2 * HID * C + HID + C) return;
+    int half, off;
+    float* dst;
+    if (e < HID * C) {
+        const int n = e / C, c = e - n * C;
+        half = n / WG_HID;
+        off = (n - half * WG_HID) * C + c;
+        dst = p.dw1 + (int64_t)n * p.lddw1 + c;
+    } else if (e < 2 * HID * C) {
+        const int f = e - HID * C, c = f / HID, n = f - c * HID;
+        half = n / WG_HID;
+        off = HALF + c * WG_HID + (n - half * WG_HID);
+        dst = p.dw2 + (int64_t)c * p.lddw2 + n;
+    } else if (e < 2 * HID * C + HID) {
+        const int n = e - 2 * HID * C;
+        half = n / WG_HID;
+        off = 2 * HALF + (n - half * WG_HID);
+        dst = p.db1 + n;
+    } else {
+        const int c = e - 2 * HID * C - HID;
+        half = 0;
+        off = 2 * HALF + WG_HID + c;
+        dst = p.db2 + c;
+    }
+    const float* src = p.ws + (size_t)half * WG_SLAB + off;
+    const size_t step = 2 * (size_t)WG_SLAB;
+    float part[8] = {0.f, 0.f, 0.f, 0.f, 0.f, 0.f, 0.f, 0.f};
+    int pr = 0;
+    for (; pr + 8 <= p.pairs; pr += 8) {
+        float v[8];
+#pragma unroll
+        for (int j = 0; j < 8; ++j) v[j] = src[(size_t)(pr + j) * step];
+#pragma unroll
+        for (int j = 0; j < 8; ++j) part[j] += v[j];
+    }
+    for (; pr < p.pairs; ++pr) part[0] += src[(size_t)pr * step];
+    *dst += ((part[0] + part[4]) + (part[2] + part[6])) + ((part[1] + part[5]) + (part[3] + part[7]));
+}
+
+int wgrad_pairs(int M) {
+    const int cus = device_cus();
+    int room = persistent_cus(cus > 0 ? cus : 256);
+    if (room > 256) room = 256;
+    int pairs = room >= 16 ? (room / 16) * 8 : (room >= 2 ? room / 2 : 1);
+    const int ntile = cdiv(M, WG_ROWS);
+    if (pairs > ntile) pairs = ntile;
+    return pairs;
+}
+
+}
+
+extern "C" int lnx_convmlp_wgrad_supported(int dtype, int C) { return dtype == LNX_BF16 && C == WG_C; }
+
+extern "C" int lnx_convmlp_wgrad_query(int C, int M, lnx_convmlp_wgrad_launch* out) {
+    LNX_CHECK(out, "lnx_convmlp_wgrad_query: null output");
+    LNX_CHECK(lnx_convmlp_wgrad_supported(LNX_BF16, C) && M > 0, "lnx_convmlp_wgrad_query: unsupported C %d (96) or empty M %d", C, M);
+    const int pairs = wgrad_pairs(M);
+    out->grid = 2 * pairs;
+    out->pairs = pairs;
+    out->rows_per_tile = WG_ROWS;
+    out->ws_floats = (int64_t)2 * pairs * WG_SLAB;
+    return 0;
+}
+
+extern "C" int lnx_convmlp_wgrad(const lnx_convmlp_wgrad_args* a, void* stream) {
+    LNX_CHECK(a && a->ln && a->dz && a->w1 && a->b1 && a->w2t && a->dw1 && a->db1 && a->dw2 && a->db2 && a->ws, "lnx_convmlp_wgrad: null operand (only dz_w may be NULL)");
+    LNX_CHECK(lnx_convmlp_wgrad_supported(a->dtype, a->C), "lnx_convmlp_wgrad: unsupported dtype %d / C %d (bf16, C = 96)", a->dtype, a->C);
+    LNX_CHECK(a->M > 0, "lnx_convmlp_wgrad: empty");
+    LNX_CHECK(a->lddw1 >= a->C && a->lddw2 >= 4 * a->C, "lnx_convmlp_wgrad: lddw1 %lld / lddw2 %lld shorter than a row (C, 4C)", (long long)a->lddw1, (long long)a->lddw2);
+    LNX_CHECK(((uintptr_t)a->ws & 15) == 0 && ((uintptr_t)a->ln & 15) == 0 && ((uintptr_t)a->dz & 15) == 0 && ((uintptr_t)a->dz_w & 15) == 0 &&
+                  ((uintptr_t)a->w1 & 15) == 0 && ((uintptr_t)a->w2t & 15) == 0,
+              "lnx_convmlp_wgrad: ws, ln, dz, dz_w, w1 and w2t must be 16-byte aligned");
+    const int pairs = wgrad_pairs(a->M);
+    LNX_CHECK(a->ws_floats >= (int64_t)2 * pairs * WG_SLAB, "lnx_convmlp_wgrad: ws too small (%lld floats, lnx_convmlp_wgrad_query reports %lld)",
+              (long long)a->ws_floats, (long long)2 * pairs * WG_SLAB);
+    WgP p;
+    p.ln = (const unsigned char*)a->ln; p.dz = (const unsigned char*)a->dz; p.dzw = (const unsigned char*)(a->dz_w ? a->dz_w : a->dz);
+    p.w1 = (const unsigned char*)a->w1; p.w2t = (const unsigned char*)a->w2t; p.b1 = a->b1; p.ws = a->ws; p.M = a->M; p.pairs = pairs;
+    hipStream_t st = (hipStream_t)stream;
+    const int rc = a->dz_w && a->dz_w != a->dz ? launch_with_lds<convmlp_wgrad_kernel<3, true>>(2 * pairs, 64 * WG_NW, 2 * WG_BUF, st, p)
+                                               : launch_with_lds<convmlp_wgrad_kernel<3, false>>(2 * pairs, 64 * WG_NW, 2 * WG_BUF, st, p);
+    if (rc != 0) return rc;
+    WgR r;
+    r.ws = a->ws; r.dw1 = a->dw1; r.db1 = a->db1; r.dw2 = a->dw2; r.db2 = a->db2; r.lddw1 = a->lddw1; r.lddw2 = a->lddw2; r.pairs = pairs;
+    constexpr int work = 2 * 4 * WG_C * WG_C + 4 * WG_C + WG_C;
+    hipLaunchKernelGGL(convmlp_wgrad_reduce_kernel, dim3(cdiv(work, 256)), dim3(256), 0, st, r);
+    LNX_LAUNCH_CHECK();
+    return 0;
+}
diff --git a/linnaeus_amd/csrc/plan.cpp b/linnaeus_amd/csrc/plan.cpp
--- a/linnaeus_amd/csrc/plan.cpp
+++ b/linnaeus_amd/csrc/plan.cpp
@@ -50,6 +50,7 @@
     bool fused = false;
     bool fused_ln = false;
     bool keep_z = true;
+    bool wgrad_recompute = false;
     int gamma, dww, dwb, lnw, lnb, b1, b2;
     OpW w1, w2;
     int64_t w49;
@@ -520,14 +521,14 @@
     p->o_stem_pre = cv.take(M0 * D[0] * esz);
     p->o_stem_mean = cv.take(M0 * 4);
     p->o_stem_rstd = cv.take(M0 * 4);
-    int64_t maxMC = 0, maxM4C = 0;
-    bool any_fused = false;
+    int64_t maxMC = 0, needA = 0, needB = 0;
+    constexpr bool WRC_DEFAULT = true;
+    const bool wrc_on = getenv("LNX_CONV_WGRAD_RECOMPUTE") ? atoi(getenv("LNX_CONV_WGRAD_RECOMPUTE")) != 0 : WRC_DEFAULT;
     const bool inf = c.inference != 0;
     const bool ck = !inf && c.recompute != 0;
     for (int s = 0; s < 2; ++s) {
         const int64_t M = (int64_t)B * p->HW[s], C = D[s];
         if (M * C > maxMC) maxMC = M * C;
-        if (M * 4 * C > maxM4C) maxM4C = M * 4 * C;
         int64_t pp[2] = {0, 0};
         if (inf) {
             pp[0] = cv.take(M * C * 4);
@@ -545,7 +546,6 @@
             k.rstd = share ? f.rstd : cv.take(M * 4);
             k.fused = lnx_convmlp_supported(c.dtype, (int)C) != 0 && getenv("LNX_NO_FUSED_MLP") == nullptr &&
                       (getenv("LNX_FUSED_MLP_MAXC") == nullptr || C <= atoi(getenv("LNX_FUSED_MLP_MAXC")));
-            any_fused = any_fused || k.fused;
             {
                 const int64_t lnws = (int64_t)2048 * 2 * (D[3] > D[0] ? D[3] : D[0]);
                 k.fused_ln = k.fused && getenv("LNX_NO_FUSED_LN") == nullptr && lnx_convmlp_bwd_ws_floats((int)C, (int)M) <= lnws;
@@ -556,6 +556,10 @@
             }
             k.keep_z = !k.fused || getenv("LNX_CONV_Z") != nullptr;
             k.z = !k.keep_z ? 0 : (share ? f.z : cv.take(M * C * esz));
+            k.wgrad_recompute = k.fused && wrc_on && !inf && lnx_convmlp_wgrad_supported(c.dtype, (int)C) != 0;
+            const int64_t wantA = k.wgrad_recompute ? M * C : M * 4 * C, wantB = k.fused && !k.wgrad_recompute ? M * 4 * C : 0;
+            if (wantA > needA) needA = wantA;
+            if (wantB > needB) needB = wantB;
         }
         p->o_stage_out[s] = inf ? pp[nb & 1] : cv.take(M * C * 4);
         p->down[s].ln = cv.take(M * C * esz);
@@ -569,7 +573,7 @@
         const int heads = c.rope_heads[s];
         if (M * C > maxMC) maxMC = M * C;
         const int64_t wide = hid > 3 * C ? hid : 3 * C;
-        if (M * wide > maxM4C) maxM4C = M * wide;
+        if (M * wide > needA) needA = M * wide;
         p->o_tok[s] = cv.take(M * C * 4);
         int64_t pp[2] = {0, 0};
         if (inf) {
@@ -684,8 +688,9 @@
             p->lsws_floats = cmax * 4 * cmax + cmax;
             p->o_lsws = cv.take(p->lsws_floats * 4);
         }
-        p->o_sA = cv.take(maxM4C * esz);
-        if (any_fused) p->o_sB = cv.take(maxM4C * esz);
+        if (maxMC > needA) needA = maxMC;
+        p->o_sA = cv.take(needA * esz);
+        if (needB > 0) p->o_sB = cv.take(needB * esz);
         p->o_sC = cv.take(maxMC * esz);
         p->o_sD = cv.take(maxMC * esz);
     }
@@ -1616,8 +1621,13 @@
         f.g = g; f.ln = c.at<void>(k.ln); f.z = k.keep_z ? c.at<void>(k.z) : nullptr; f.w1 = c.wptr(k.w1); f.b1 = p->P[k.b1];
         f.w2t = c.wtptr(k.w2); f.w1t = c.wtptr(k.w1); f.gamma = p->P[k.gamma];
         f.rowscale = p->drop_ptr(p->drop_conv[s][i]); f.rows_per_sample = H * W;
-        f.act = sB; f.dh = sA; f.dz = sC; f.dln = sD; f.dgamma = p->G[k.gamma];
+        f.dz = sC; f.dln = sD; f.dgamma = p->G[k.gamma];
         f.dz_plain = k.keep_z ? 0 : 1;
+        if (!k.wgrad_recompute) {
+            f.act = sB; f.dh = sA;
+        } else if (!k.keep_z) {
+            f.dz_gamma = sA;
+        }
         if (k.fused_ln) {
             f.y = c.at<void>(k.y); f.ln_w = p->P[k.lnw]; f.mean = c.at<float>(k.mean); f.rstd = c.at<float>(k.rstd);
             f.d_ln_w = p->G[k.lnw]; f.d_ln_b = p->G[k.lnb];
@@ -1634,13 +1644,37 @@
             }
         }
         {
-            Timed t(c, 7, 2.0 * M * C * 4 * C * 3);
+            const double e = p->esz, mc = (double)M * C;
+            Timed t(c, 7, 2.0 * M * C * 4 * C * 3, mc * (4.0 + e * ((k.fused_ln ? 2.0 : 1.0) + (k.keep_z ? 1.0 : 0.0) + 2.0 + (f.act ? 8.0 : 0.0) + (f.dz_gamma ? 1.0 : 0.0))));
             RUN(lnx_convmlp_bwd(&f, c.st));
         }
         const Ctx cw = wg_ctx(c);
         RUN(wg_fork(c, 0));
         forked = true;
-        if (k.keep_z) {
+        if (k.wgrad_recompute) {
+            static_assert(LNX_CONVMLP_WGRAD_WS_FLOATS <= 2 * (int64_t)LNX_TN_WS_FLOATS && TN_WS_SLOTS >= 2, "the recompute kernel's slabs live in two split-K regions");
+            lnx_convmlp_wgrad_args w;
+            memset(&w, 0, sizeof w);
+            w.dtype = c.dt; w.M = M; w.C = C;
+            w.ln = c.at<void>(k.ln); w.w1 = c.wptr(k.w1); w.b1 = p->P[k.b1]; w.w2t = c.wtptr(k.w2);
+            w.dw1 = p->G[k.w1.param]; w.lddw1 = C; w.db1 = p->G[k.b1];
+            w.ws = c.at<float>(p->o_tnws); w.ws_floats = 2 * (int64_t)LNX_TN_WS_FLOATS;
+            float* S = c.at<float>(p->o_lsws);
+            float* T = S + (int64_t)C * 4 * C;
+            if (k.keep_z) {
+                w.dz = sC; w.dw2 = p->G[k.w2.param]; w.db2 = p->G[k.b2];
+            } else {
+                w.dz = sA; w.dz_w = sC; w.dw2 = S; w.db2 = T;
+                HIPRUN(hipMemsetAsync(S, 0, ((size_t)C * 4 * C + C) * 4, (hipStream_t)cw.st));
+            }
+            w.lddw2 = 4 * C;
+            {
+                Timed t(cw, 1, 2.0 * 2.0 * M * 4 * C * C, (double)p->esz * (k.keep_z ? 2.0 : 3.0) * M * C + 8.0 * 2.0 * 4 * C * C);
+                RUN(lnx_convmlp_wgrad(&w, cw.st));
+            }
+            if (!k.keep_z)
+                RUN(lnx_layerscale_apply_wgrad(S, T, 4 * C, p->P[k.w2.param], p->P[k.b2], 4 * C, p->P[k.gamma], p->G[k.w2.param], p->G[k.b2], 4 * C, p->G[k.gamma], C, 4 * C, cw.st));
+        } else if (k.keep_z) {
             RUN(wgrad(cw, M, C, 4 * C, sC, C, sB, 4 * C, k.w2.param, k.b2, 4 * C, 0, 0));
             RUN(wgrad(cw, M, 4 * C, C, sA, 4 * C, c.at<void>(k.ln), C, k.w1.param, k.b1, C, 0, 1));
             RUN(lnx_gemm_tn_flush(cw.st));
diff --git a/linnaeus_amd/ops.py b/linnaeus_amd/ops.py
--- a/linnaeus_amd/ops.py
+++ b/linnaeus_amd/ops.py
@@ -382,7 +382,7 @@
 
 
 def convmlp_bwd(g, ln, z, w1, b1, w2t, w1t, gamma, act, dh, dz, dln, dgamma, *, rowscale=None, rows_per_sample=0, y=None, ln_w=None, mean=None,
-                rstd=None, d_ln_w=None, d_ln_b=None, ws=None, dz_plain=False):
+                rstd=None, d_ln_w=None, d_ln_b=None, ws=None, dz_plain=False, dz_gamma=None):
     a = L.ConvMlpBwdArgs()
     a.dtype, a.M, a.C = code_of(ln), ln.shape[0], ln.shape[1]
     a.g, a.ln, a.z, a.w1, a.b1, a.w2t, a.w1t, a.gamma = _p(g), _p(ln), _p(z), _p(w1), _p(b1), _p(w2t), _p(w1t), _p(gamma)
@@ -390,8 +390,23 @@
     a.act, a.dh, a.dz, a.dln, a.dgamma = _p(act), _p(dh), _p(dz), _p(dln), _p(dgamma)
     a.y, a.ln_w, a.mean, a.rstd, a.d_ln_w, a.d_ln_b = _p(y), _p(ln_w), _p(mean), _p(rstd), _p(d_ln_w), _p(d_ln_b)
     a.ws, a.ws_floats = _p(ws), (ws.numel() if ws is not None else 0)
-    a.dz_plain = int(dz_plain)
+    a.dz_plain, a.dz_gamma = int(dz_plain), _p(dz_gamma)
     L.check(L.lib().lnx_convmlp_bwd(C.byref(a), _stream()), "lnx_convmlp_bwd")
+
+
+def convmlp_wgrad_query(Cc, M):
+    q = L.ConvMlpWgradLaunch()
+    L.check(L.lib().lnx_convmlp_wgrad_query(Cc, M, C.byref(q)), "lnx_convmlp_wgrad_query")
+    return q.grid, q.pairs, q.rows_per_tile, q.ws_floats
+
+
+def convmlp_wgrad(ln, dz, w1, b1, w2t, dw1, db1, dw2, db2, ws, *, dz_w=None):
+    a = L.ConvMlpWgradArgs()
+    a.dtype, a.M, a.C = code_of(ln), ln.shape[0], ln.shape[1]
+    a.ln, a.dz, a.dz_w, a.w1, a.b1, a.w2t = _p(ln), _p(dz), _p(dz_w), _p(w1), _p(b1), _p(w2t)
+    a.dw1, a.lddw1, a.db1, a.dw2, a.lddw2, a.db2 = _p(dw1), dw1.stride(0), _p(db1), _p(dw2), dw2.stride(0), _p(db2)
+    a.ws, a.ws_floats = _p(ws), ws.numel()
+    L.check(L.lib().lnx_convmlp_wgrad(C.byref(a), _stream()), "lnx_convmlp_wgrad")
 
 
 def _meta_head_buffers(B, C_, dev):
```

Result: faster. 13490 images/sec, median of 6 (+1.7%).
